# MuellerNico/DD2360-RayTracing

Hardware: AMD Instinct MI355X
Metric: Msamples/s (W*H*spp/render_time) at 1200x800, 10000 spheres (higher is better)
Workload: dtype f32

## Files before the change

### dd2360-raytracing_amd/csrc/rt_api.hip

```cpp
#include <hip/hip_runtime.h>
#include <atomic>
#include <vector>
#include <string>
#include <cstdio>
#include <cstring>
#include <new>
#include <limits>
#include <cmath>
#include <algorithm>
#include <mutex>
#include <cstdlib>
#include "rt_handles.h"
#include "rt_octgeom.h"
#include "../host/rt_image.hpp"

namespace rt {
hipError_t launch_render_init(rt_rand_state* rs, int max_x, int max_y, int part, int nparts, long long begin, long long end, hipStream_t st);
hipError_t launch_zero_counters(unsigned int* p, int n, hipStream_t st);
hipError_t launch_keep_counters(const unsigned int* queue, unsigned int* kept, hipStream_t st);
hipError_t launch_restore_counters(unsigned int* queue, const unsigned int* kept, hipStream_t st);
hipError_t launch_pilot(const RenderArgs& A, bool tree, int* cost, unsigned char* pilot, int* work, hipStream_t st);
hipError_t launch_pilot_h(const RenderArgs& A, bool tree, int* cost, hipStream_t st);
hipError_t launch_assemble_split(void* full, const void* parts, int max_x, int max_y, int nparts, const long long* starts, long long part_stride_px, bool half, hipStream_t st);
hipError_t launch_render(const RenderArgs& A, bool tree, int mode, hipStream_t st);
namespace fmac { hipError_t launch_render(const RenderArgs& A, bool tree, int mode, hipStream_t st); }
hipError_t launch_tile_order(const RenderArgs& A, bool tree, int* cost, unsigned int* order, unsigned char* flags, unsigned int* long_list, hipStream_t st);
hipError_t launch_render_h(const RenderArgs& A, bool tree, int mode, hipStream_t st);
hipError_t launch_tile_order_h(const RenderArgs& A, bool tree, int* cost, unsigned int* order, unsigned char* flags, unsigned int* long_list, hipStream_t st);
hipError_t launch_trace_h(const DevScene& S, const DevTree& T, bool tree, const float* rays, long long n, rt_hit_record* out, hipStream_t st);
hipError_t launch_assemble_h(void* full, const void* parts, int max_x, int max_y, int nparts, hipStream_t st);
hipError_t launch_trace(const DevScene& S, const DevTree& T, bool tree, const float* rays, long long n, rt_hit_record* out, hipStream_t st);
hipError_t launch_guides(const DevScene& S, const DevTree& T, bool tree, int max_x, int max_y, rt_hit_record* out, hipStream_t st);
hipError_t launch_denoise(float* fb_out, const float* fb_in, int max_x, int max_y, const rt_hit_record* hits, const rt_denoise_params& P,
                          float4* work, hipStream_t st);
hipError_t launch_denoise_var(float* fb_out, const float* fb_in, int max_x, int max_y, const rt_hit_record* hits, const void* state,
                              const rt_denoise_var_params& P, float4* work, hipStream_t st);
hipError_t launch_temporal_accumulate(void* hist_out, const void* hist_in, const rt_hit_record* hits, const rt_hit_record* hits_prev,
                                      const rt_camera* cam_prev, const void* state, const int32_t* kind, int n_kind, int max_x, int max_y,
                                      const rt_temporal_params& P, hipStream_t st);
hipError_t launch_denoise_hist(float* fb_out, const float* fb_in, int max_x, int max_y, const rt_hit_record* hits, const void* hist,
                               const rt_denoise_var_params& P, float4* work, hipStream_t st);
hipError_t launch_world_set_geometry(float4* geom, float4* shade, float4* list_hot, const int32_t* list_id, const float4* src, int n, int n_list,
                                     bool half, hipStream_t st);
hipError_t launch_temporal_accumulate_moving(void* hist_out, const void* hist_in, const rt_hit_record* hits, const rt_hit_record* hits_prev,
                                             const rt_camera* cam_prev, const float4* geom, const float4* geom_prev, const void* state,
                                             const int32_t* kind, int n_kind, int max_x, int max_y, const rt_temporal_params& P,
                                             hipStream_t st);
hipError_t launch_assemble(float* full, const float* parts, int max_x, int max_y, int nparts, hipStream_t st);
hipError_t launch_render_adaptive(const RenderArgs& A, bool tree, hipStream_t st);
hipError_t launch_adapt_check(float* fb, const float* sl, const float* q, const unsigned int* list_in, const unsigned int* count_in, long long n_all,
                              unsigned int* list_out, unsigned int* count_out, int32_t* spp, int k, bool last, float rel_error, float floor_lum,
                              const AdaptFrame& fr, hipStream_t st);
hipError_t launch_adapt_zero(unsigned int* p, int n, hipStream_t st);
hipError_t launch_adapt_check_keep(float* fb, const AdaptState& s, const unsigned int* list_in, const unsigned int* count_in, long long n_all,
                                   unsigned int* list_out, unsigned int* count_out, int32_t* spp, int k, bool last, float rel_error, float floor_lum,
                                   const AdaptFrame& fr, hipStream_t st);
hipError_t launch_adapt_refine_seed(float* fb, const AdaptState& s, long long n_all, unsigned int* list_out, unsigned int* count_out, int32_t* spp,
                                    int max_spp, float rel_error, float floor_lum, const AdaptFrame& fr, hipStream_t st);
hipError_t launch_adapt_refine_check(float* fb, const AdaptState& s, const unsigned int* list_in, const unsigned int* count_in, long long n_all,
                                     unsigned int* list_out, unsigned int* count_out, int32_t* spp, int batch, int max_spp, float rel_error, float floor_lum,
                                     hipStream_t st);
size_t budget_ws_bytes(long long n, bool filtered);
hipError_t launch_budget_select_filtered(const AdaptState& s, const rt_hit_record* hits, int max_x, int max_y, const rt_denoise_var_params& P, int batch,
                                         int max_spp, float floor_lum, unsigned int K, unsigned int* keys, float* keys_out, unsigned int* ws,
                                         unsigned int* list, unsigned int* count, hipStream_t st);
hipError_t launch_budget_select_temporal(const void* state, const void* hist_in, const rt_hit_record* hits, const rt_hit_record* hits_prev,
                                         const rt_camera* cam_prev, const int32_t* kind, int n_kind, int max_x, int max_y, const rt_temporal_params& P,
                                         int batch, int max_spp, float floor_lum, unsigned int K, unsigned int* keys, float* keys_out, unsigned int* ws,
                                         unsigned int* list, unsigned int* count, hipStream_t st);
hipError_t launch_budget_select(const AdaptState& s, long long n, const AdaptFrame& fr, int batch, int max_spp, float floor_lum, unsigned int K,
                                unsigned int* keys, unsigned int* ws, unsigned int* list, unsigned int* count, hipStream_t st);
hipError_t launch_budget_seed(float* fb, const AdaptState& s, const unsigned int* list, const unsigned int* count, unsigned int cap, hipStream_t st);
hipError_t launch_budget_final(float* fb, const AdaptState& s, const unsigned int* list, const unsigned int* count, unsigned int cap, int32_t* spp, int batch,
                               uint32_t* picked, hipStream_t st);
const char* render_kernel_name(bool tree, int mode, const DevAccel& acc);
namespace gpubuild { int build(rt_octree* O, const float4* d_geom, const int32_t* d_kind, int n, int spl, hipStream_t st); }
const char* render_kernel_name_h(bool tree, int mode);
#ifdef RT_H16_STATS
hipError_t read_h16_stats(unsigned long long* out, int reset);
#endif
#ifdef RT_STATS
hipError_t read_stats(unsigned long long* out, int reset);
hipError_t read_wp_classes(unsigned long long* out, int reset);
hipError_t read_wave_dbg(unsigned long long* out);
hipError_t read_pilot_dbg(int* out, int n);
#endif
}

using namespace rt;

#define RT_TRY(expr) do { const int e_ = (int)(expr); if (e_) return e_; } while (0)

static int world_host_geometry(const rt_world* W) {
    rt_world::Lazy& Z = *W->z;
    if (!Z.host_stale) return 0;
    rt_world* M = const_cast<rt_world*>(W);
    RT_TRY(hipDeviceSynchronize());
    RT_TRY(hipMemcpy(M->h_geom.data(), Z.d_geom, M->h_geom.size() * sizeof(float4), hipMemcpyDeviceToHost));
    if (!M->h_hot.empty()) RT_TRY(hipMemcpy(M->h_hot.data(), Z.d_list_hot, M->h_hot.size() * sizeof(float4), hipMemcpyDeviceToHost));
    Z.host_stale = false;
    return 0;
}

static rt_octree* build_list_tree(const rt_world* W) {
    rt_octree* O = new rt_octree();
    O->z = new rt_octree::Lazy();
    O->precision = RT_PRECISION_FP32;
    DevNode d; memset(&d, 0, sizeof(d));
    const float inf = std::numeric_limits<float>::infinity();
    d.lo[0] = d.lo[1] = d.lo[2] = -inf; d.hix = d.hiy = d.hiz = inf;
    d.skip = 1; d.first = 0; d.ref_index = 0;
    for (int i = 1; i < W->n; ++i) {
        if (W->h_kind[i] == RT_MAT_NONE) continue;
        const float4 g = W->h_geom[i];
        O->h_ent_hot.push_back(make_float4(g.x, g.y, g.z, g.w * g.w));
        O->h_ent_id.push_back(i);
    }
    d.count = (int32_t)O->h_ent_id.size();
    O->h_nodes.push_back(d);
    O->n_nodes = 1; O->n_entries = d.count;
    if (d.count > 0) build_accel(O->accel, O->h_nodes, O->h_ent_id, O->h_ent_hot, W->n, true);
    if (d.count < 64 || !O->accel.p.enabled || O->accel.p.n_large > 64) { delete O->z; delete O; return nullptr; }
    return O;
}
static rt_octree* ensure_list_tree(const rt_world* W) {
    rt_world::Lazy& Z = *W->z;
    if (!Z.list_tree_tried && W->precision == RT_PRECISION_FP32) {
        if (world_host_geometry(W)) return nullptr;
        Z.list_tree_tried = true;
        try { Z.list_tree = build_list_tree(W); } catch (const std::bad_alloc&) { Z.list_tree = nullptr; }
    }
    return Z.list_tree;
}

static bool valid_partition(rt_partition p) {
    if (!(p.nparts >= 1 && p.part >= 0 && p.part < p.nparts)) return false;
    if (p.tile_begin == 0 && p.tile_end == 0) return true;
    return p.tile_begin >= 0 && p.tile_end > p.tile_begin;
}
bool adaptive_params_ok(const rt_adaptive* P) {
    if (!P || P->min_spp < 2 || P->batch < 1 || P->max_spp < P->min_spp || (P->max_spp - P->min_spp) % P->batch != 0) return false;
    return P->rel_error >= 0.f && P->floor >= 0.f;
}
static bool adaptive_refines(const rt_adaptive* from, const rt_adaptive* to) {
    if (!adaptive_params_ok(from) || !adaptive_params_ok(to)) return false;
    if (to->min_spp != from->min_spp || to->batch != from->batch || to->max_spp < from->max_spp || !(to->floor <= from->floor)) return false;
    if (!(to->rel_error == 0.f || (to->rel_error > 0.f && to->rel_error <= from->rel_error))) return false;
    const float t = from->rel_error * from->rel_error;
    const float tn = t * ((float)from->max_spp - 1.f);
    if (!std::isfinite(tn)) return false;
    if (from->rel_error > 0.f && t == 0.f && to->rel_error > 0.f && to->floor != from->floor) return false;
    return true;
}
static const rt_partition kWhole = {0, 1, 0, 0};
static bool range_in_frame(rt_partition p, int64_t tiles) { return p.tile_end <= p.tile_begin || p.tile_end <= tiles; }
static int64_t local_tiles_of(int64_t tiles, rt_partition p) { return part_local_tiles(tiles, p.part, p.nparts, p.tile_begin, p.tile_end); }
static bool hittable(const rt_sphere& s) { return s.material != RT_MAT_NONE; }
static float radius_squared(const rt_sphere& s, int precision) {
    if (precision == RT_PRECISION_FP16) { const half_t r(s.radius); return (r * r).f(); }
    return s.radius * s.radius;
}

template <class R> static int create_world_impl(rt_sphere* list, int num_spheres, float sphere_radius, rt_camera* cam, int nx, int ny, rt_rand_state* st, int* num_created) {
    const int created = create_world_pods<R>(list, num_spheres, sphere_radius, cam, nx, ny, st);
    if (num_created) *num_created = created;
    return 0;
}

// ... 22 lines not shown
    switch (code) {
        case 0: return "ok";
        case RT_EINVAL: return "invalid argument";
        case RT_ENOMEM: return "out of host memory";
        case RT_EIO: return "i/o error";
        case RT_ENOTSUP: return "not supported";
        case RT_ECOMM: return "multi-GPU exchange failed";
        default: return code > 0 ? hipGetErrorString((hipError_t)code) : "unknown error";
    }
}

int rt_rand_init(rt_rand_state* rand_state) {
    if (!rand_state) return RT_EINVAL;
    xorwow::init(*rand_state, 1984ull);
    return 0;
}

int rt_create_world(rt_sphere* list, int num_spheres, float sphere_radius, rt_camera* cam, int nx, int ny, rt_rand_state* rand_state, int precision, int* num_created) {
    if (!list || !cam || !rand_state || num_spheres < 5 || nx <= 0 || ny <= 0) return RT_EINVAL;
    try {
        if (precision == RT_PRECISION_FP16) return create_world_impl<half_t>(list, num_spheres, sphere_radius, cam, nx, ny, rand_state, num_created);
        if (precision == RT_PRECISION_FP32) return create_world_impl<float>(list, num_spheres, sphere_radius, cam, nx, ny, rand_state, num_created);
    } catch (const std::bad_alloc&) { return RT_ENOMEM; }
    return RT_EINVAL;
}

int rt_camera_init(rt_camera* cam, const float lookfrom[3], const float lookat[3], const float vup[3], float vfov, float aspect, float aperture, float focus_dist, int precision) {
    if (!cam || !lookfrom || !lookat || !vup) return RT_EINVAL;
    if (precision == RT_PRECISION_FP16) camera_impl<half_t>(cam, lookfrom, lookat, vup, vfov, aspect, aperture, focus_dist);
    else if (precision == RT_PRECISION_FP32) camera_impl<float>(cam, lookfrom, lookat, vup, vfov, aspect, aperture, focus_dist);
    else return RT_EINVAL;
    return 0;
}

int rt_world_create(const rt_sphere* list, int num_spheres, const rt_camera* cam, int precision, rt_world** out) {
    if (!list || !cam || !out || num_spheres <= 0) return RT_EINVAL;
    if (precision != RT_PRECISION_FP32 && precision != RT_PRECISION_FP16) return RT_EINVAL;
    *out = nullptr;
    rt_world* W = new (std::nothrow) rt_world();
    if (!W) return RT_ENOMEM;
    W->z = new (std::nothrow) rt_world::Lazy();
    if (!W->z) { delete W; return RT_ENOMEM; }
    W->precision = precision; W->n = num_spheres;
    std::vector<float4>& hot = W->h_hot; std::vector<float4>& geom = W->h_geom; std::vector<float4>& mat = W->h_mat;
    std::vector<int32_t>& ids = W->h_ids; std::vector<int32_t>& kind = W->h_kind;
    geom.resize(num_spheres); mat.resize(num_spheres); kind.resize(num_spheres);
    for (int i = 0; i < num_spheres; ++i) {
        const rt_sphere& s = list[i];
        geom[i] = make_float4(s.center[0], s.center[1], s.center[2], s.radius);
        mat[i] = make_float4(s.albedo[0], s.albedo[1], s.albedo[2], s.param);
        kind[i] = s.material;
        if (hittable(s)) { hot.push_back(make_float4(s.center[0], s.center[1], s.center[2], radius_squared(s, precision))); ids.push_back(i); }
    }
    W->z->dev.n = num_spheres; W->z->dev.n_list = (int)hot.size();
    W->z->dev.ground_valid = hittable(list[0]) ? 1 : 0;
    W->z->dev.cam = *cam;
    *out = W;
    return 0;
}

int rt_world_set_list_traversal(rt_world* W, int mode) {
    if (!W || (mode != RT_TRAVERSAL_REFERENCE && mode != RT_TRAVERSAL_FAST)) return RT_EINVAL;
    W->list_traversal = mode;
    return 0;
}

int rt_world_set_arith(rt_world* W, int mode) {
    if (!W || (mode != RT_ARITH_IEEE && mode != RT_ARITH_CONTRACT)) return RT_EINVAL;
    if (mode == RT_ARITH_CONTRACT && W->precision == RT_PRECISION_FP16) return RT_ENOTSUP;
    W->arith = mode;
    return 0;
}
int rt_world_list_accel_info(const rt_world* W, int* enabled, int* grid_dim, float* cell_size, int* grid_entries, int* large_spheres) {
    if (!W) return RT_EINVAL;
    rt_octree* LT = ensure_list_tree(W);
    if (enabled) *enabled = LT != nullptr;
    if (!LT) { if (grid_dim) *grid_dim = 0; if (cell_size) *cell_size = 0.f; if (grid_entries) *grid_entries = 0; if (large_spheres) *large_spheres = 0; return 0; }
    return rt_octree_accel_info(LT, grid_dim, cell_size, grid_entries, large_spheres);
}

static DevGroup queue_group(rt_render_ctx& C) { return DevGroup().add(&C.d_queue, (kQueueSlots + 1) * kQueueStride * sizeof(unsigned int)); }
static DevGroup sched_group(rt_render_ctx& C, size_t tiles) {
    return DevGroup().add(&C.d_cost, sizeof(int) * tiles).add(&C.d_order, sizeof(unsigned int) * tiles).add(&C.d_flags, tiles * 96)
                     .add(&C.d_long, sizeof(unsigned int) * (tiles * 128 + 512)).add(&C.d_work, sizeof(int) * tiles * 2);
}
static DevGroup progressive_group(rt_render_ctx& C, size_t tiles) { return DevGroup().add(&C.p_cost, sizeof(int) * tiles).add(&C.p_order, sizeof(unsigned int) * tiles); }
static DevGroup adaptive_group(rt_render_ctx& C, size_t pixels) {
    return DevGroup().add(&C.a_sl, sizeof(float) * pixels).add(&C.a_q, sizeof(float) * pixels).add(&C.a_list, sizeof(unsigned int) * pixels * 2);
}
static DevGroup rounds_group(rt_render_ctx& C, size_t rounds) { return DevGroup().add(&C.a_count, sizeof(unsigned int) * rounds); }
static DevGroup budget_group(rt_render_ctx& C, size_t bytes) { return DevGroup().add(&C.b_ws, bytes); }

static int ctx_prepare(rt_render_ctx& C) {
    if (!C.d_queue) {
        RT_TRY(group_regrow(queue_group(C)));
        const hipError_t e = hipMemset(C.d_queue, 0, (kQueueSlots + 1) * kQueueStride * sizeof(unsigned int));
        if (e != hipSuccess) { (void)group_free(queue_group(C)); return (int)e; }
        C.d_kept = C.d_queue + (size_t)kQueueSlots * kQueueStride;
        sched_keep_drop(C.keep);
    }
    if (!C.ev_ready) {
        for (int k = 0; k < 64; ++k) {
            if (!C.ev0[k]) RT_TRY(hipEventCreate(&C.ev0[k]));
            if (!C.ev1[k]) RT_TRY(hipEventCreate(&C.ev1[k]));
        }
        if (!C.done) RT_TRY(hipEventCreateWithFlags(&C.done, hipEventDisableTiming));
        C.ev_ready = true;
    }
    return 0;
}
static int ctx_reserve(rt_render_ctx& C, int64_t tiles) {
    if (C.sched_tiles < tiles) sched_keep_drop(C.keep);
    return group_reserve(C.sched_tiles, tiles, sched_group(C, tiles));
}
static int ctx_reserve_progressive(rt_render_ctx& C, int64_t tiles) {
    if (C.p_tiles >= tiles) return 0;
    if (C.p_pinned) return RT_EINVAL;
    C.p_valid = false;
    return group_reserve(C.p_tiles, tiles, progressive_group(C, tiles));
}
static int ctx_reserve_adaptive(rt_render_ctx& C, int64_t pixels, int rounds) {
    RT_TRY(group_reserve(C.a_pixels, pixels, adaptive_group(C, pixels)));
    return group_reserve(C.a_rounds, rounds, rounds_group(C, rounds));
}
static int ctx_reserve_budget(rt_render_ctx& C, int64_t pixels, bool filtered = false) {
    const size_t bytes = budget_ws_bytes(pixels, filtered);
    return group_reserve(C.b_bytes, (int64_t)bytes, budget_group(C, bytes));
}
static int ctx_release(rt_render_ctx& C) {
    sched_keep_drop(C.keep); C.d_kept = nullptr;
    C.a_pixels = 0; C.a_rounds = 0; C.b_bytes = 0; C.sched_tiles = 0; C.p_tiles = 0; C.p_valid = false;
    int rc = 0;
    for (const DevGroup& g : {adaptive_group(C, 0), rounds_group(C, 0), budget_group(C, 0), queue_group(C), sched_group(C, 0), progressive_group(C, 0)}) {
        const int r = group_free(g);
        if (!rc) rc = r;
    }
    for (int k = 0; k < 64; ++k) { if (C.ev0[k]) (void)hipEventDestroy(C.ev0[k]); if (C.ev1[k]) (void)hipEventDestroy(C.ev1[k]); C.ev0[k] = nullptr; C.ev1[k] = nullptr; }
    if (C.done) (void)hipEventDestroy(C.done);
    C.done = nullptr; C.ev_ready = false; C.has_done = false; C.ev_count = 0;
    return rc;
}

int rt_render_ctx_create(rt_render_ctx** out) {
    if (!out) return RT_EINVAL;
    *out = nullptr;
    rt_render_ctx* C = new (std::nothrow) rt_render_ctx();
    if (!C) return RT_ENOMEM;
    const int rc = ctx_prepare(*C);
    if (rc) { (void)ctx_release(*C); delete C; return rc; }
    *out = C;
    return 0;
}
int rt_render_ctx_reserve(rt_render_ctx* C, int max_x, int max_y, rt_partition part) {
    if (!C || max_x <= 0 || max_y <= 0 || !valid_partition(part)) return RT_EINVAL;
    const int64_t tiles = (int64_t)((max_x + 7) / 8) * ((max_y + 7) / 8);
    const int rc = ctx_prepare(*C);
    if (!range_in_frame(part, tiles)) return RT_EINVAL;
    return rc ? rc : ctx_reserve(*C, local_tiles_of(tiles, part));
}
int rt_render_ctx_destroy(rt_render_ctx* C) {
    if (!C) return 0;
    const int rc = ctx_release(*C);
    delete C;
    return rc;
}

static DevGroup world_group(const rt_world* W, const std::vector<float4>* shade = nullptr, const std::vector<uint8_t>* kind8 = nullptr) {
// ... 352 lines not shown
        if (rc != RT_ENOTSUP) return rc;
    }
    RT_TRY(world_host_geometry(world));
    std::vector<rt_sphere> list;
    try {
        list.resize((size_t)world->n);
        for (int i = 0; i < world->n; ++i) {
            rt_sphere& s = list[i];
            const float4 g = world->h_geom[i], m = world->h_mat[i];
            s.center[0] = g.x; s.center[1] = g.y; s.center[2] = g.z; s.radius = g.w;
            s.material = world->h_kind[i]; s.albedo[0] = m.x; s.albedo[1] = m.y; s.albedo[2] = m.z; s.param = m.w;
        }
    } catch (const std::bad_alloc&) { return RT_ENOMEM; }
    return rt_build_octree(list.data(), world->n, spheres_per_leaf, world->precision, out);
}

int64_t rt_part_pixels(int max_x, int max_y, rt_partition part) {
    if (max_x <= 0 || max_y <= 0 || !valid_partition(part)) return RT_EINVAL;
    if (part_whole(part.nparts, part.tile_begin, part.tile_end)) return (int64_t)max_x * max_y;
    const int64_t tiles = (int64_t)((max_x + 7) / 8) * ((max_y + 7) / 8);
    if (!range_in_frame(part, tiles)) return RT_EINVAL;
    return local_tiles_of(tiles, part) * 64;
}

int rt_render_init(int max_x, int max_y, rt_rand_state* d_rand_state, rt_partition part, void* stream) {
    if (max_x <= 0 || max_y <= 0 || !valid_partition(part)) return RT_EINVAL;
    const int64_t npx = rt_part_pixels(max_x, max_y, part);
    if (npx < 0) return RT_EINVAL;
    if (npx == 0) return 0;
    if (!d_rand_state) return RT_EINVAL;
    return (int)launch_render_init(d_rand_state, max_x, max_y, part.part, part.nparts, part.tile_begin, part.tile_end, (hipStream_t)stream);
}

static const rt_octree* list_tree_of(const rt_world* world) {
    if (world->list_traversal != RT_TRAVERSAL_FAST) return nullptr;
    return ensure_list_tree(world);
}

static int ensure_on_device(const rt_world* world, const rt_octree*& d_octree) {
    if (!d_octree) d_octree = list_tree_of(world);
    int rc = world_upload(world);
    if (!rc && d_octree) rc = octree_upload(d_octree);
    return rc;
}
static DevTree tree_args(const rt_octree* d_octree) {
    DevTree T;
    if (d_octree) { T = d_octree->z->dev; T.acc.enabled = T.acc.enabled && d_octree->traversal == RT_TRAVERSAL_FAST; }
    else memset(&T, 0, sizeof(T));
    return T;
}
static float tune_value(const char* env, float dflt) {
    static std::mutex mu;
    static std::vector<std::pair<std::string, float>> seen;
    std::lock_guard<std::mutex> lock(mu);
    for (const auto& kv : seen) if (kv.first == env) return kv.second;
    float v = dflt;
    if (const char* e = getenv(env)) { char* end = nullptr; const float x = strtof(e, &end); if (end != e) v = x; }
    seen.emplace_back(env, v);
    return v;
}
static bool capturing(hipStream_t st) {
    hipStreamCaptureStatus cs = hipStreamCaptureStatusNone;
    if (hipStreamIsCapturing(st, &cs) != hipSuccess) { (void)hipGetLastError(); return false; }
    return cs != hipStreamCaptureStatusNone;
}

static void clear_schedule(RenderArgs& A) {
    A.order = nullptr; A.long_flag = nullptr; A.long_list = nullptr;
    A.tail_list = nullptr; A.tail_ws = nullptr; A.f_tail = 0.f; A.head_sum = 0; A.head_sum_dense = 0; A.head_min_load = 0.f;
    A.n_lanes = 0;
}
static RenderArgs frame_args(void* fb, int max_x, int max_y, int ns, const rt_world* world, rt_rand_state* d_rand_state, const rt_octree* d_octree, rt_partition part) {
    RenderArgs A;
    A.fb = fb; A.rand_state = d_rand_state; A.max_x = max_x; A.max_y = max_y; A.ns = ns;
    A.tiles_x = (max_x + 7) / 8; A.tiles_y = (max_y + 7) / 8;
    A.part = part.part; A.nparts = part.nparts; A.tile_begin = part.tile_begin; A.tile_end = part.tile_end;
    const int64_t tiles = (int64_t)A.tiles_x * A.tiles_y;
    A.n_local_tiles = local_tiles_of(tiles, part);
    A.scene = world->z->dev;
    A.tree = tree_args(d_octree);
    clear_schedule(A);
    A.f_inflight = tune_value("RT_F_INFLIGHT", RT_F_INFLIGHT); A.f_inflight_dense = tune_value("RT_F_INFLIGHT_DENSE", RT_F_INFLIGHT_DENSE); A.f_static = tune_value("RT_F_STATIC", RT_F_STATIC);
    A.ad_list = nullptr; A.ad_count = nullptr; A.ad_sl = nullptr; A.ad_q = nullptr;
    return A;
}

static int ctx_wait_previous(rt_render_ctx& C, hipStream_t st) {
    if (C.has_done && C.last_stream != st) RT_TRY(hipStreamWaitEvent(st, C.done, 0));
    return 0;
}
static int ctx_mark_done(rt_render_ctx& C, hipStream_t st) {
    RT_TRY(hipEventRecord(C.done, st));
    C.has_done = true; C.last_stream = st;
    return 0;
}
static unsigned int* next_slot(rt_render_ctx& C) { return C.d_queue + (size_t)(C.launches++ % kQueueSlots) * kQueueStride; }
static int ctx_timed_begin(rt_render_ctx& C, hipStream_t st) { return (int)hipEventRecord(C.ev0[C.ev_head % 64u], st); }
static int ctx_timed_end(rt_render_ctx& C, hipStream_t st) {
    RT_TRY(hipEventRecord(C.ev1[C.ev_head % 64u], st));
    C.ev_head++; if (C.ev_count < 64) C.ev_count++;
    return 0;
}
static int resumed_round(rt_render_ctx& C, RenderArgs& A, bool tree, hipStream_t st) {
    A.queue = next_slot(C);
    RT_TRY(launch_zero_counters(A.queue, (int)kQueueStride, st));
    return (int)launch_render_adaptive(A, tree, st);
}

static SchedKey frame_key(const rt_world* world, const rt_octree* d_octree, int max_x, int max_y, rt_partition part) {
    SchedKey key;
    key.world = world->serial; key.tree = d_octree ? d_octree->serial : 0;
    key.max_x = max_x; key.max_y = max_y;
    key.part = part.part; key.nparts = part.nparts; key.tile_begin = part.tile_begin; key.tile_end = part.tile_end;
    key.traversal = d_octree ? d_octree->traversal : 0;
    key.half = world->precision == RT_PRECISION_FP16 ? 1 : 0;
    return key;
}
static int schedule_decide(rt_render_ctx& C, const RenderArgs& A, const rt_world* world, const rt_octree* d_octree, int ns, bool cap, SchedKey& key, SchedAction& act) {
    int dev = 0;
    RT_TRY(hipGetDevice(&dev));
    key = frame_key(world, d_octree, A.max_x, A.max_y, rt_partition{A.part, A.nparts, A.tile_begin, A.tile_end});
    key.ns = ns; key.device = dev;
    act = sched_keep_decide(C.keep, key, tune_value("RT_SCHED_CACHE", (float)RT_SCHED_CACHE) != 0.f, cap);
    return 0;
}
static int begin_counters(rt_render_ctx& C, const RenderArgs& A, SchedAction act, hipStream_t st) {
    if (act == kSchedReuse) RT_TRY(launch_restore_counters(A.queue, C.d_kept, st));
    else RT_TRY(launch_zero_counters(A.queue, (int)kQueueStride, st));
    return 0;
}
static int schedule_frame(rt_render_ctx& C, RenderArgs& A, const rt_world* world, const rt_octree* d_octree, int ns, hipStream_t st, SchedAction act, const SchedKey& key) {
    const bool classify = ns >= 16;
    if (classify && world->precision != RT_PRECISION_FP16) { A.tail_list = C.d_long + (size_t)A.n_local_tiles * 64; A.tail_ws = C.d_long + (size_t)C.sched_tiles * 128; A.f_tail = tune_value("RT_F_TAIL", RT_F_TAIL); A.head_sum = (int)tune_value("RT_HEAD_SUM_SPARSE", (float)RT_HEAD_SUM_SPARSE); A.head_sum_dense = (int)tune_value("RT_HEAD_SUM_DENSE", (float)RT_HEAD_SUM_DENSE); A.head_min_load = tune_value("RT_HEAD_LOAD_DENSE", (float)RT_HEAD_LOAD_DENSE); }
    if (act != kSchedReuse) {
        if (world->precision == RT_PRECISION_FP16) RT_TRY(launch_tile_order_h(A, d_octree != nullptr, C.d_cost, C.d_order, classify ? C.d_flags : nullptr, classify ? C.d_long : nullptr, st));
        else RT_TRY(launch_tile_order(A, d_octree != nullptr, C.d_cost, C.d_order, classify ? C.d_flags : nullptr, classify ? C.d_long : nullptr, st));
        if (act == kSchedCompute) {
            RT_TRY(launch_keep_counters(A.queue, C.d_kept, st));
            sched_keep_commit(C.keep, key);
        }
    }
    A.order = C.d_order;
    if (classify) { A.long_flag = C.d_flags; A.long_list = C.d_long; }
    return 0;
}
static int scheduled_round(rt_render_ctx& C, RenderArgs& A, const rt_world* world, const rt_octree* d_octree, int ns, bool sched, bool cap, hipStream_t st) {
    A.queue = next_slot(C);
    SchedKey key; SchedAction act = kSchedBypass;
    if (sched) RT_TRY(schedule_decide(C, A, world, d_octree, ns, cap, key, act));
    RT_TRY(begin_counters(C, A, act, st));
    if (sched) RT_TRY(schedule_frame(C, A, world, d_octree, ns, st, act, key));
    return 0;
}

static int render_common(rt_render_ctx* ctx, void* fb, int max_x, int max_y, int ns, const rt_world* world, rt_rand_state* d_rand_state, const rt_octree* d_octree, rt_partition part, void* stream, int mode) {
    if (!world || max_x <= 0 || max_y <= 0 || ns <= 0 || !valid_partition(part)) return RT_EINVAL;
    if (d_octree && d_octree->precision != world->precision) return RT_EINVAL;
    { const int64_t npx = rt_part_pixels(max_x, max_y, part); if (npx < 0) return RT_EINVAL; if (npx == 0) return 0; }
    if (!fb || !d_rand_state) return RT_EINVAL;
    const hipStream_t st = (hipStream_t)stream;
    const bool cap = capturing(st);
    int rc = ensure_on_device(world, d_octree);
    rt_render_ctx& C = ctx ? *ctx : world->z->ctx;
    if (!rc && !cap) rc = ctx_prepare(C);
    if (rc) return rc;
    if (!C.d_queue) return RT_EINVAL;
    const SchedKey pkey = frame_key(world, d_octree, max_x, max_y, part);
    if (mode == 1 && ns == 1 && !cap && C.p_pinned && !sched_key_equal(C.p_key, pkey)) return RT_EINVAL;
    RenderArgs A = frame_args(fb, max_x, max_y, ns, world, d_rand_state, d_octree, part);
    const bool sched = mode == 0 && ns >= 4, tree = d_octree != nullptr;
    if (sched && C.sched_tiles < A.n_local_tiles) {
        if (cap) return RT_EINVAL;
        RT_TRY(ctx_reserve(C, A.n_local_tiles));
    }
    if (!cap) RT_TRY(ctx_wait_previous(C, st));
    RT_TRY(scheduled_round(C, A, world, d_octree, ns, sched, cap, st));
    C.last_queue = A.queue;
    if (mode == 1) {
        if (ns == 1 && !cap) {
            C.p_valid = false;
            RT_TRY(ctx_reserve_progressive(C, A.n_local_tiles));
            if (world->precision == RT_PRECISION_FP16) RT_TRY(launch_tile_order_h(A, tree, C.p_cost, C.p_order, nullptr, nullptr, st));
            else RT_TRY(launch_tile_order(A, tree, C.p_cost, C.p_order, nullptr, nullptr, st));
            C.p_key = pkey; C.p_valid = true;
        }
        if (C.p_valid && sched_key_equal(C.p_key, pkey) && C.p_tiles >= A.n_local_tiles) { A.order = C.p_order; if (cap) C.p_pinned = true; }
    }
    if (!cap) RT_TRY(ctx_timed_begin(C, st));
    if (world->precision == RT_PRECISION_FP16) RT_TRY(launch_render_h(A, tree, mode, st));
    else if (world->arith == RT_ARITH_CONTRACT) RT_TRY(fmac::launch_render(A, tree, mode, st));
    else RT_TRY(launch_render(A, tree, mode, st));
    if (cap) return 0;
    RT_TRY(ctx_timed_end(C, st));
    return ctx_mark_done(C, st);
}

static int ctx_times(rt_render_ctx& C, float* ms_out, int max, int* count) {
    int n = 0;
    const unsigned have = C.ev_count;
    for (unsigned k = 0; k < have && n < max; ++k) {
        const unsigned slot = (C.ev_head - have + k) % 64u;
        RT_TRY(hipEventSynchronize(C.ev1[slot]));
        float ms = 0.f;
        RT_TRY(hipEventElapsedTime(&ms, C.ev0[slot], C.ev1[slot]));
        ms_out[n++] = ms;
    }
    *count = n;
    C.ev_count = 0;
    return 0;
}
static int ctx_counters(rt_render_ctx& C, uint32_t* out4) {
    if (!C.last_queue) { out4[0] = out4[1] = out4[2] = out4[3] = 0u; return 0; }
    if (C.has_done) RT_TRY(hipEventSynchronize(C.done));
    uint32_t q[6];
    RT_TRY(hipMemcpy(q, C.last_queue, sizeof(q), hipMemcpyDeviceToHost));
    out4[0] = q[0]; out4[1] = q[1]; out4[2] = q[2] + q[4]; out4[3] = q[3] + q[5];
    return 0;
}
int rt_world_render_counters(rt_world* W, uint32_t* out4) {
    if (!W || !out4) return RT_EINVAL;
    return ctx_counters(W->z->ctx, out4);
}
int rt_render_ctx_counters(rt_render_ctx* C, uint32_t* out4) {
    if (!C || !out4) return RT_EINVAL;
    return ctx_counters(*C, out4);
}
static int ctx_schedule(rt_render_ctx& C, uint32_t* out, int n) {
    if (n > RT_SCHEDULE_WORDS) n = RT_SCHEDULE_WORDS;
    uint32_t w[RT_SCHEDULE_WORDS] = {0, 0, 0, 0, 0, 0, 0, 0};
    if (C.last_queue) {
        if (C.has_done) RT_TRY(hipEventSynchronize(C.done));
        uint32_t q[kQueueThr + 6];
        RT_TRY(hipMemcpy(q, C.last_queue, sizeof(q), hipMemcpyDeviceToHost));
        for (int k = 0; k < 6; ++k) w[k] = q[kQueueThr + k];
        w[6] = q[2]; w[7] = q[4];
    }
    for (int k = 0; k < n; ++k) out[k] = w[k];
    return 0;
}
int rt_world_render_schedule(rt_world* W, uint32_t* out, int n) {
    if (!W || n < 0 || (n > 0 && !out)) return RT_EINVAL;
    return ctx_schedule(W->z->ctx, out, n);
}
int rt_render_ctx_schedule(rt_render_ctx* C, uint32_t* out, int n) {
    if (!C || n < 0 || (n > 0 && !out)) return RT_EINVAL;
    return ctx_schedule(*C, out, n);
}
int rt_render_ctx_schedule_reuse(rt_render_ctx* C, uint64_t* reused, uint64_t* computed) {
    if (!C || !reused || !computed) return RT_EINVAL;
    *reused = C->keep.reused; *computed = C->keep.computed;
    return 0;
}
int rt_world_render_schedule_reuse(rt_world* W, uint64_t* reused, uint64_t* computed) {
    if (!W) return RT_EINVAL;
    return rt_render_ctx_schedule_reuse(&W->z->ctx, reused, computed);
}
int rt_world_render_times(rt_world* W, float* ms_out, int max, int* count) {
    if (!W || !ms_out || !count || max < 0) return RT_EINVAL;
    return ctx_times(W->z->ctx, ms_out, max, count);
}
int rt_render_ctx_times(rt_render_ctx* C, float* ms_out, int max, int* count) {
    if (!C || !ms_out || !count || max < 0) return RT_EINVAL;
    return ctx_times(*C, ms_out, max, count);
}

int rt_render(void* fb, int max_x, int max_y, int ns, const rt_world* world, rt_rand_state* d_rand_state, const rt_octree* d_octree, rt_partition part, void* stream) {
    return render_common(nullptr, fb, max_x, max_y, ns, world, d_rand_state, d_octree, part, stream, 0);
}
int rt_render_progressive(void* fb, int max_x, int max_y, int current_sample, const rt_world* world, rt_rand_state* d_rand_state, const rt_octree* d_octree, rt_partition part, void* stream) {
    return render_common(nullptr, fb, max_x, max_y, current_sample, world, d_rand_state, d_octree, part, stream, 1);
}
int rt_render_on(rt_render_ctx* ctx, void* fb, int max_x, int max_y, int ns, const rt_world* world, rt_rand_state* d_rand_state, const rt_octree* d_octree, rt_partition part, void* stream) {
    if (!ctx) return RT_EINVAL;
    return render_common(ctx, fb, max_x, max_y, ns, world, d_rand_state, d_octree, part, stream, 0);
}
int rt_render_progressive_on(rt_render_ctx* ctx, void* fb, int max_x, int max_y, int current_sample, const rt_world* world, rt_rand_state* d_rand_state, const rt_octree* d_octree, rt_partition part, void* stream) {
    if (!ctx) return RT_EINVAL;
    return render_common(ctx, fb, max_x, max_y, current_sample, world, d_rand_state, d_octree, part, stream, 1);
}

struct FrameCall {
    hipStream_t st = nullptr; rt_render_ctx* C = nullptr;
    int64_t npx = 0;
    bool tree = false;
    AdaptFrame fr{};
};
static int frame_begin(FrameCall& F, rt_render_ctx* ctx, bool params_ok, bool pointers_ok, int max_x, int max_y, rt_partition part,
                       const rt_world* world, const rt_octree*& d_octree, void* stream, const rt_world* kinds = nullptr) {
    if (!params_ok || max_x <= 0 || max_y <= 0 || !valid_partition(part)) return RT_EINVAL;
    const int64_t npx = rt_part_pixels(max_x, max_y, part);
    if (npx < 0 || npx > (int64_t)0xffffffffll) return RT_EINVAL;
    if (npx == 0) return 0;
    if (!pointers_ok) return RT_EINVAL;
    if (world && d_octree && d_octree->precision != world->precision) return RT_EINVAL;
    if (world && (world->precision == RT_PRECISION_FP16 || world->arith == RT_ARITH_CONTRACT)) return RT_ENOTSUP;
    if (kinds && kinds->precision == RT_PRECISION_FP16) return RT_ENOTSUP;
    F.st = (hipStream_t)stream;
    if (capturing(F.st)) return RT_EINVAL;
    int rc = world ? ensure_on_device(world, d_octree) : 0;
    if (!rc && kinds) rc = world_upload(kinds);
    F.C = ctx ? ctx : &world->z->ctx;
    if (!rc) rc = ctx_prepare(*F.C);
    if (rc) return rc;
    F.npx = npx; F.tree = d_octree != nullptr;
    F.fr = AdaptFrame{max_x, max_y, (max_x + 7) / 8, part.part, part.nparts, part.tile_begin, part.tile_end};
    return 0;
}

static int render_adaptive_common(rt_render_ctx* ctx, void* fb, int max_x, int max_y, const rt_adaptive* P, const rt_world* world,
                                  rt_rand_state* d_rand_state, const rt_octree* d_octree, int32_t* d_spp, rt_partition part, void* stream,
                                  void* d_state = nullptr, bool need_state = false) {
    FrameCall F;
    const int rc = frame_begin(F, ctx, adaptive_params_ok(P) && world, fb && d_rand_state && (d_state || !need_state), max_x, max_y, part, world, d_octree, stream);
    if (rc || !F.npx) return rc;
    rt_render_ctx& C = *F.C; const hipStream_t st = F.st; const int64_t npx = F.npx;
    const AdaptState keep = adapt_state(d_state, npx);
    const int rounds = (P->max_spp - P->min_spp) / P->batch;
    RenderArgs A = frame_args(fb, max_x, max_y, P->min_spp, world, d_rand_state, d_octree, part);
    const bool sched = P->min_spp >= 4;
    if (sched) RT_TRY(ctx_reserve(C, A.n_local_tiles));
    RT_TRY(ctx_reserve_adaptive(C, npx, rounds + 1));
    RT_TRY(ctx_wait_previous(C, st));
    unsigned int* lists[2] = {C.a_list, C.a_list + npx};
    A.ad_sl = d_state ? keep.sl : C.a_sl; A.ad_q = d_state ? keep.q : C.a_q;
    RT_TRY(launch_adapt_zero(C.a_count, rounds + 1, st));
    RT_TRY(scheduled_round(C, A, world, d_octree, P->min_spp, sched, false, st));
    RT_TRY(ctx_timed_begin(C, st));
    RT_TRY(launch_render_adaptive(A, F.tree, st));
    auto check = [&](const unsigned int* list_in, const unsigned int* count_in, unsigned int* list_out, unsigned int* count_out, int k, bool last) {
        return d_state ? launch_adapt_check_keep((float*)fb, keep, list_in, count_in, npx, list_out, count_out, d_spp, k, last, P->rel_error, P->floor, F.fr, st)
                       : launch_adapt_check((float*)fb, C.a_sl, C.a_q, list_in, count_in, npx, list_out, count_out, d_spp, k, last, P->rel_error, P->floor, F.fr, st);
    };
    RT_TRY(check(nullptr, nullptr, lists[0], C.a_count, P->min_spp, rounds == 0));
    A.ns = P->batch;
    clear_schedule(A);
    for (int r = 1; r <= rounds; ++r) {
        A.ad_list = lists[(r - 1) & 1]; A.ad_count = C.a_count + (r - 1);
        RT_TRY(resumed_round(C, A, F.tree, st));
// ... 348 lines not shown
    if (P.normal_pow_log2 < -1 || P.normal_pow_log2 > 10) return RT_EINVAL;
    if (P.prefilter != 0 && P.prefilter != 1) return RT_EINVAL;
    if (!denoise_sigma_ok(P.sigma_position, 1.0f)) return RT_EINVAL;
    if (!(P.sigma_variance >= 0.0f) || !std::isfinite(P.sigma_variance * P.sigma_variance)) return RT_EINVAL;
    return 0;
}

int rt_denoise_adaptive(void* fb_out, const void* fb_in, int max_x, int max_y, const rt_hit_record* d_hits, const void* d_state,
                        const rt_denoise_var_params* params, void* d_work, void* stream) {
    if (!fb_out || !fb_in || !d_hits || !d_state || !d_work) return RT_EINVAL;
    if (((uintptr_t)d_hits & 15) || ((uintptr_t)d_work & 15)) return RT_EINVAL;
    const int rc = rt_denoise_adaptive_check(max_x, max_y, params);
    if (rc) return rc;
    return (int)launch_denoise_var((float*)fb_out, (const float*)fb_in, max_x, max_y, d_hits, d_state, *params, (float4*)d_work, (hipStream_t)stream);
}

int rt_temporal_check(int max_x, int max_y, const rt_temporal_params* params) {
    if (!params || max_x <= 0 || max_y <= 0 || (long long)max_x * max_y > RT_DENOISE_MAX_PIXELS) return RT_EINVAL;
    const rt_temporal_params& P = *params;
    if (P.max_history < 0) return RT_EINVAL;
    if (P.reuse_specular != 0 && P.reuse_specular != 1) return RT_EINVAL;
    if (!(P.position_tolerance > 0.0f) || !std::isfinite(P.position_tolerance) || !std::isfinite(P.position_tolerance * P.position_tolerance)) return RT_EINVAL;
    if (!(P.normal_min_dot >= -1.0f && P.normal_min_dot <= 1.0f)) return RT_EINVAL;
    return 0;
}

int rt_temporal_accumulate(void* d_hist_out, const void* d_hist_in, const rt_hit_record* d_hits, const rt_hit_record* d_hits_prev,
                           const rt_camera* cam_prev, const void* d_state, const rt_world* world, int max_x, int max_y,
                           const rt_temporal_params* params, void* stream) {
    if (!d_hist_out || !d_hits || !d_state || !world) return RT_EINVAL;
    if (d_hist_in && (!d_hits_prev || !cam_prev)) return RT_EINVAL;
    if (((uintptr_t)d_hist_out & 15) || ((uintptr_t)d_hist_in & 15) || ((uintptr_t)d_hits & 15) || (d_hist_in && ((uintptr_t)d_hits_prev & 15))) return RT_EINVAL;
    const int rc = rt_temporal_check(max_x, max_y, params);
    if (rc) return rc;
    if (d_hist_in) {
        const uintptr_t a = (uintptr_t)d_hist_out, b = (uintptr_t)d_hist_in, bytes = (uintptr_t)RT_TEMPORAL_HISTORY_BYTES * (uintptr_t)max_x * (uintptr_t)max_y;
        if ((a > b ? a - b : b - a) < bytes) return RT_EINVAL;
    }
    if (world->precision == RT_PRECISION_FP16) return RT_ENOTSUP;
    const int up = world_upload(world);
    if (up) return up;
    return (int)launch_temporal_accumulate(d_hist_out, d_hist_in, d_hits, d_hits_prev, cam_prev, d_state, world->z->dev.kind, world->n, max_x, max_y,
                                           *params, (hipStream_t)stream);
}

int rt_temporal_accumulate_moving(void* d_hist_out, const void* d_hist_in, const rt_hit_record* d_hits, const rt_hit_record* d_hits_prev,
                                  const rt_camera* cam_prev, const float* d_geom_prev, const void* d_state, const rt_world* world,
                                  int max_x, int max_y, const rt_temporal_params* params, void* stream) {
    if (!d_hist_out || !d_hits || !d_state || !world) return RT_EINVAL;
    if (d_hist_in && (!d_hits_prev || !cam_prev || !d_geom_prev)) return RT_EINVAL;
    if (((uintptr_t)d_hist_out & 15) || ((uintptr_t)d_hist_in & 15) || ((uintptr_t)d_hits & 15) || (d_hist_in && ((uintptr_t)d_hits_prev & 15))) return RT_EINVAL;
    if (d_hist_in && ((uintptr_t)d_geom_prev & 15)) return RT_EINVAL;
    const int rc = rt_temporal_check(max_x, max_y, params);
    if (rc) return rc;
    if (d_hist_in) {
        const uintptr_t a = (uintptr_t)d_hist_out, b = (uintptr_t)d_hist_in, bytes = (uintptr_t)RT_TEMPORAL_HISTORY_BYTES * (uintptr_t)max_x * (uintptr_t)max_y;
        if ((a > b ? a - b : b - a) < bytes) return RT_EINVAL;
    }
    if (world->precision == RT_PRECISION_FP16) return RT_ENOTSUP;
    const int up = world_upload(world);
    if (up) return up;
    return (int)launch_temporal_accumulate_moving(d_hist_out, d_hist_in, d_hits, d_hits_prev, cam_prev, world->z->dev.geom,
                                                  d_hist_in ? (const float4*)d_geom_prev : nullptr, d_state, world->z->dev.kind, world->n,
                                                  max_x, max_y, *params, (hipStream_t)stream);
}

int rt_denoise_history(void* fb_out, const void* fb_in, int max_x, int max_y, const rt_hit_record* d_hits, const void* d_hist,
                       const rt_denoise_var_params* params, void* d_work, void* stream) {
    if (!fb_out || !fb_in || !d_hits || !d_hist || !d_work) return RT_EINVAL;
    if (((uintptr_t)d_hits & 15) || ((uintptr_t)d_hist & 15) || ((uintptr_t)d_work & 15)) return RT_EINVAL;
    const int rc = rt_denoise_adaptive_check(max_x, max_y, params);
    if (rc) return rc;
    return (int)launch_denoise_hist((float*)fb_out, (const float*)fb_in, max_x, max_y, d_hits, d_hist, *params, (float4*)d_work, (hipStream_t)stream);
}

#ifdef RT_H16_STATS
int rt_debug_h16(unsigned long long* out8, int reset) { return (int)rt::read_h16_stats(out8, reset); }
#endif
#ifdef RT_STATS
int rt_debug_stats(unsigned long long* out16, int reset) { return (int)read_stats(out16, reset); }
int rt_debug_wp_classes(unsigned long long* out96, int reset) { return (int)read_wp_classes(out96, reset); }
int rt_debug_waves(unsigned long long* out) { return (int)read_wave_dbg(out); }
int rt_debug_pilot(int* out, int n) { return (int)read_pilot_dbg(out, n); }
#endif

using rt::ppm_text;

int64_t rt_format_ppm(int nx, int ny, const void* fb, int precision, char* out, int64_t cap) {
    if (nx <= 0 || ny <= 0 || !fb) return RT_EINVAL;
    std::string s;
    try { ppm_text(nx, ny, fb, precision, s); } catch (const std::bad_alloc&) { return RT_ENOMEM; }
    if (out && (int64_t)s.size() <= cap) memcpy(out, s.data(), s.size());
    return (int64_t)s.size();
}

int rt_write_ppm(const char* path, int nx, int ny, const void* fb, int precision) {
    if (nx <= 0 || ny <= 0 || !fb) return RT_EINVAL;
    std::string s;
    try { ppm_text(nx, ny, fb, precision, s); } catch (const std::bad_alloc&) { return RT_ENOMEM; }
    FILE* f = path ? fopen(path, "wb") : stdout;
    if (!f) return RT_EIO;
    const size_t w = fwrite(s.data(), 1, s.size(), f);
    if (path) { if (fclose(f) != 0) return RT_EIO; } else fflush(f);
    return w == s.size() ? 0 : RT_EIO;
}

int rt_write_image(const char* path, int nx, int ny, const void* fb, int precision, int format) {
    if (!path || nx <= 0 || ny <= 0 || !fb) return RT_EINVAL;
    if (precision != RT_PRECISION_FP32 && precision != RT_PRECISION_FP16) return RT_EINVAL;
    if (format == RT_IMAGE_P3) return rt_write_ppm(path, nx, ny, fb, precision);
    if (format != RT_IMAGE_P6 && format != RT_IMAGE_PFM) return RT_EINVAL;
    FILE* f = fopen(path, "wb");
    if (!f) return RT_EIO;
    bool ok = true;
    try {
        ok = rt::write_binary_image(f, nx, ny, fb, precision, format);
    } catch (const std::bad_alloc&) { fclose(f); return RT_ENOMEM; }
    if (fclose(f) != 0) ok = false;
    return ok ? 0 : RT_EIO;
}

}
```

### dd2360-raytracing_amd/csrc/rt_device.h

```cpp
#pragma once
#include <hip/hip_runtime.h>
#include <stdint.h>
#include "../../include/rt_amd.h"

namespace rt {

constexpr double kRootHalfXZ = 11.0;
constexpr double kCellXZ = 2.0 * kRootHalfXZ / 8.0, kCellY = 0.25;
constexpr float kRootHalfXZf = (float)kRootHalfXZ, kInvCellXZf = 1.0f / 2.75f, kInvCellYf = 4.0f;
static_assert(kCellXZ == 2.75 && 1.0 / kCellY == 4.0, "level-3 cells of the reference's root box");


#ifndef RT_PART_RUN_BUILD
#define RT_PART_RUN_BUILD RT_PART_RUN
#endif
constexpr long long kPartRun = RT_PART_RUN_BUILD;
__host__ __device__ inline bool part_whole(int nparts, long long begin, long long end) { return nparts == 1 && end <= begin; }
__host__ __device__ inline long long part_tile(long long local_tile, int part, int nparts, long long begin = 0, long long end = 0) {
    if (end > begin) return begin + local_tile;
    if (nparts == 1) return local_tile;
    return ((local_tile / kPartRun) * nparts + part) * kPartRun + local_tile % kPartRun;
}
__host__ __device__ inline long long part_local_tiles(long long tiles, int part, int nparts, long long begin = 0, long long end = 0) {
    if (end > begin) return end - begin;
// ... 59 lines not shown
    float hiy, hiz;
    int32_t skip;
    int32_t first;
    int32_t count;
    int32_t ref_index;
    int32_t pad[2];
};
static_assert(sizeof(DevNode) == 48, "DevNode is 3 x float4");

struct DevScene {
    const float4* list_hot;
    const int32_t* list_id;
    const float4* geom;
    const float4* mat;
    const int32_t* kind;
    const float4* shade;
    const uint8_t* kind8;
    int32_t n, n_list;
    int32_t ground_valid;
    rt_camera cam;
};

struct DevAccel {
    const float4* large_hot;
    const float4* large_brick;
    const int32_t* cs;
    const float4* hot;
    const float4* brick;
    int32_t zoff;
    const int32_t* memb_start;
    const int32_t* memb_cell;
    const int32_t* bits_index;
    const uint32_t* cellbits;
    const int32_t* cellnode;
    int32_t n_large, G;
    int32_t F, Gf;
    float rq_c;
    float g0, h, inv_h;
    float ylo, yhi;
    float rmax;
    float zone2;
    int32_t enabled;
    int32_t coop_groups;
    int32_t solo_chains;
};

struct DevTree {
    const float4* nodes4;
    const float4* ent_hot;
    const int32_t* ent_id;
    int32_t n_nodes, n_entries;
    const float* h16_planes;
    int32_t h16_np[3];
    DevAccel acc;
};

constexpr int kQueueThr = 32;
struct RenderArgs {
    void* fb;
    rt_rand_state* rand_state;
    int32_t max_x, max_y, ns;
    int32_t tiles_x, tiles_y;
    int32_t part, nparts;
    int64_t tile_begin, tile_end;
    int64_t n_local_tiles;
    unsigned int* queue;
    int32_t n_lanes;
    const unsigned int* tail_list;
    unsigned int* tail_ws;
    float head_min_load;
    int32_t head_sum, head_sum_dense;
    float f_tail;
    float f_inflight_dense;
    float f_inflight, f_static;
    const unsigned int* order;
    const unsigned char* long_flag;
    const unsigned int* long_list;
    DevScene scene;
    DevTree tree;
    const unsigned int* ad_list;
    const unsigned int* ad_count;
    float* ad_sl;
    float* ad_q;
};

}
```

### dd2360-raytracing_amd/csrc/rt_handles.h

```cpp
#pragma once
#include <hip/hip_runtime.h>
#include <cassert>
#include <vector>
#include "rt_device.h"
#include "../host/rt_scene.hpp"
#include "rt_accel.h"
#include "rt_sched_keep.h"

using rt::DevScene; using rt::DevTree; using rt::DevNode; using rt::DevAccel; using rt::AccelHost; using rt::Octree;

struct rt_octree;

struct DevBuf { void** at; size_t bytes; const void* src; size_t src_bytes; };
struct DevGroup {
    int n = 0; DevBuf b[16];
    DevGroup& add(void* at, size_t bytes) { assert(n < 16); b[n++] = DevBuf{(void**)at, bytes, nullptr, 0}; return *this; }
    template <class V> DevGroup& add_copy(void* at, const V& v) {
        const size_t sz = sizeof(typename V::value_type);
        assert(n < 16);
        b[n++] = DevBuf{(void**)at, (v.empty() ? 1 : v.size()) * sz, v.empty() ? nullptr : v.data(), v.size() * sz};
        return *this;
    }
};
inline int group_free(const DevGroup& g) {
    int rc = 0;
    for (int k = 0; k < g.n; ++k) {
        void*& p = *g.b[k].at;
        if (p) { const hipError_t e = hipFree(p); if (e != hipSuccess && !rc) rc = (int)e; p = nullptr; }
    }
    return rc;
}
inline int group_regrow(const DevGroup& g) {
    int rc = group_free(g);
    for (int k = 0; k < g.n && !rc; ++k) {
        const DevBuf& b = g.b[k];
        if (!b.bytes) continue;
        rc = (int)hipMalloc(b.at, b.bytes);
        if (!rc && b.src) rc = (int)hipMemcpy(*b.at, b.src, b.src_bytes, hipMemcpyHostToDevice);
        if (rc) (void)group_free(g);
    }
    return rc;
}
inline int group_reserve(int64_t& have, int64_t need, const DevGroup& g) {
    if (have >= need) return 0;
    have = 0;
    const int rc = group_regrow(g);
    if (!rc) have = need;
    return rc;
}

struct rt_render_ctx {
    unsigned int* d_queue = nullptr; unsigned launches = 0;
    int* d_cost = nullptr; unsigned int* d_order = nullptr; unsigned char* d_flags = nullptr; unsigned int* d_long = nullptr; int* d_work = nullptr; int64_t sched_tiles = 0;
    unsigned int* last_queue = nullptr;
    rt::SchedKeep keep; unsigned int* d_kept = nullptr;
    int* p_cost = nullptr; unsigned int* p_order = nullptr; int64_t p_tiles = 0; bool p_valid = false; rt::SchedKey p_key;
    bool p_pinned = false;
    float* a_sl = nullptr; float* a_q = nullptr; unsigned int* a_list = nullptr; int64_t a_pixels = 0; unsigned int* a_count = nullptr; int64_t a_rounds = 0;
    unsigned int* b_ws = nullptr; int64_t b_bytes = 0;
    hipEvent_t ev0[64] = {}, ev1[64] = {}; unsigned ev_head = 0, ev_count = 0; bool ev_ready = false;
    hipEvent_t done = nullptr; hipStream_t last_stream = nullptr; bool has_done = false;
};
static const unsigned kQueueSlots = 64, kQueueStride = 64;

uint64_t rt_next_serial();

struct rt_world {
    uint64_t serial = rt_next_serial();
    int precision = RT_PRECISION_FP32;
    int n = 0;
    std::vector<float4> h_hot, h_geom, h_mat;
    std::vector<int32_t> h_ids, h_kind;
    int list_traversal = RT_TRAVERSAL_FAST;
    int arith = RT_ARITH_IEEE;
    struct Lazy {
        bool uploaded = false;
        DevScene dev{};
        void* d_list_hot = nullptr; void* d_list_id = nullptr; void* d_geom = nullptr; void* d_mat = nullptr; void* d_kind = nullptr;
        void* d_shade = nullptr; void* d_kind8 = nullptr;
        rt_octree* list_tree = nullptr; bool list_tree_tried = false;
        rt_render_ctx ctx;
        bool host_stale = false;
    };
    Lazy* z = nullptr;
};

struct rt_octree {
    uint64_t serial = rt_next_serial();
    int precision = RT_PRECISION_FP32;
    Octree* host = nullptr;
    std::vector<DevNode> h_nodes; std::vector<float4> h_ent_hot; std::vector<int32_t> h_ent_id;
    AccelHost accel;
    int traversal = RT_TRAVERSAL_FAST;
    struct Lazy {
        bool uploaded = false;
        DevTree dev{};
        void* d_nodes = nullptr; void* d_ent_hot = nullptr; void* d_ent_id = nullptr;
        void* d_acc[12] = {nullptr, nullptr, nullptr, nullptr, nullptr, nullptr, nullptr, nullptr, nullptr, nullptr, nullptr, nullptr};
        void* d_arena = nullptr;
        const rt_octnode* d_ref_nodes = nullptr; const int32_t* d_leaf_count = nullptr; const int32_t* d_leaf_indices = nullptr;
        int ref_node_count = 0, ref_leaf_count = 0, ref_dropped_full = 0, ref_dropped_outside = 0, ref_spl = 0;
        Octree* host_view = nullptr;
    };
    Lazy* z = nullptr;
    int n_nodes = 0, n_entries = 0;
    int n_world = 0, bit_rows = 1;
};


bool adaptive_params_ok(const rt_adaptive* P);
```

### dd2360-raytracing_amd/csrc/rt_kernels.hip

```cpp
#include <hip/hip_runtime.h>
#include <float.h>
#include "rt_device.h"
#include "rt_tuning.h"
#include "rt_sampling.h"
#include "rt_sched_keep.h"

#ifdef RT_TU_CONTRACT
#pragma clang fp contract(fast)
#else
#pragma clang fp contract(off)
#endif

namespace rt {
#ifdef RT_TU_CONTRACT
namespace fmac {
#endif

#define RT_DEV static __device__ __forceinline__

#include "rt_stats.h"

struct Rng { uint32_t d, v0, v1, v2, v3, v4; };

RT_DEV float rng_uniform(Rng& s) {
// ... 1009 lines not shown
    const float dt = dot3(uv, on);
    const float disc = 1.0f - ni * ni * (1.0f - dt * dt);
    float fx = 0.0f, fy = 0.0f, fz = 0.0f, reflect_prob;
    if (disc > 0.0f) {
        const float sq = sqrtf(disc);
        fx = ni * (uv.x - dt * on.x) - sq * on.x;
        fy = ni * (uv.y - dt * on.y) - sq * on.y;
        fz = ni * (uv.z - dt * on.z) - sq * on.z;
        const float r0 = r0sq;
        reflect_prob = r0 + (1.0f - r0) * pow5(1.0f - cosine);
    } else {
        reflect_prob = 1.0f;
    }
    r.o = p;
    if (rng_uniform(s) < reflect_prob) { r.d.x = rx; r.d.y = ry; r.d.z = rz; }
    else { r.d.x = fx; r.d.y = fy; r.d.z = fz; }
    return true;
}

RT_DEV V3 sky(const RayF& r, const V3& att) {
    WPASS(WP_SKY);
    const float len = sqrtf(r.d.x * r.d.x + r.d.y * r.d.y + r.d.z * r.d.z);
    const float uy = r.d.y / len;
    const float t = 0.5f * (uy + 1.0f);
    const float omt = 1.0f - t;
    V3 c;
    c.x = att.x * (omt + t * 0.5f);
    c.y = att.y * (omt + t * 0.7f);
    c.z = att.z * (omt + t * 1.0f);
    return c;
}

#ifndef RT_TU_LIST
__global__ __launch_bounds__(256) void k_render_init(rt_rand_state* rand_state, int max_x, int max_y, int tiles_x, int part, int nparts, long long begin, long long end, long long n_local_tiles) {
    const int lane = threadIdx.x & 63;
    const long long local_tile = (long long)blockIdx.x * 4 + (threadIdx.x >> 6);
    if (local_tile >= n_local_tiles) return;
    const long long tile = part_tile(local_tile, part, nparts, begin, end);
    const int tx = (int)(tile % tiles_x), ty = (int)(tile / tiles_x);
    const int i = tx * 8 + (lane & 7), j = ty * 8 + (lane >> 3);
    const bool inside = (i < max_x) && (j < max_y);
    const bool whole = part_whole(nparts, begin, end);
    if (whole && !inside) return;
    const long long idx = whole ? (long long)j * max_x + i : local_tile * 64 + lane;
    const int pixel_index = j * max_x + i;
    Rng s; rng_seed(s, 1984ull + (unsigned long long)(long long)pixel_index);
    rt_rand_state out;
    out.d = s.d; out.v[0] = s.v0; out.v[1] = s.v1; out.v[2] = s.v2; out.v[3] = s.v3; out.v[4] = s.v4;
    out.boxmuller_flag = 0; out.boxmuller_flag_double = 0; out.boxmuller_extra = 0.f; out.pad_ = 0; out.boxmuller_extra_double = 0.0;
    rand_state[idx] = out;
}
#endif

template <bool TREE, int MODE, int COOPG>
__global__ __launch_bounds__(256, RT_RENDER_WAVES) void k_render(RenderArgs A) {
    extern __shared__ float4 s_nodes[];
    if (TREE) stage_tree_fp32<COOPG != 1>(A.scene, A.tree, s_nodes);
    const int lane = threadIdx.x & 63;
    const long long n_slots = (MODE == 2 && A.ad_list) ? (long long)*A.ad_count : A.n_local_tiles * 64;
    const int ns = (MODE != 1) ? A.ns : 1;

    const long long n_waves = (long long)gridDim.x * 4;
    long long slot = 0;
    int i = 0, j = 0; long long idx = 0;
    unsigned int iters = 0;
    bool is_long = false;
    bool is_med = false;
    bool retired = false;
    bool thin = false;
    bool thin_counted = false;
    bool long_done = false;
    const unsigned int n_long_raw = A.long_list ? A.queue[2] : 0u, n_solo_raw = A.long_list ? A.queue[4] : 0u;
    const bool use_long = (n_long_raw + n_solo_raw) != 0u && (long long)(n_long_raw + n_solo_raw) * 64 <= n_slots;
    const unsigned int n_long = use_long ? n_long_raw : 0u, n_solo = use_long ? n_solo_raw : 0u;
    bool solo = false, solo_done = false;
    Rng s = {0, 0, 0, 0, 0, 0};
    V3 col = {0.0f, 0.0f, 0.0f};
    V3 att = {1.0f, 1.0f, 1.0f};
    float sum_l = 0.0f, sum_q = 0.0f;
    RayF r; r.o = {0.f, 0.f, 0.f}; r.d = {0.f, 1.f, 0.f};
    int sample = 0, depth = 0;
    bool live = false;
    RT_STATS_ONLY(
    unsigned int pix_iters = 0;
    unsigned long long pix_t0 = 0;
    )

    constexpr bool kChunked = MODE == 1;
    constexpr long long kProgOwn = RT_PROG_OWN;
    const long long first_free = (kChunked && kProgOwn > 0 && n_waves * kProgOwn <= n_slots) ? n_waves * kProgOwn : 0;
    long long pool_next = 0, pool_end = 0;
    if (kChunked && first_free > 0) { pool_next = ((long long)blockIdx.x * 4 + (threadIdx.x >> 6)) * kProgOwn; pool_end = pool_next + kProgOwn; }
    auto take_slot = [&]() -> long long {
        return first_free + (long long)atomicAdd(cold_args()->queue, 1u);
    };
    auto begin_pixel = [&]() {
        live = false;
        const RenderArgs& A = *cold_args();
#ifdef RT_ONLY_LANE
        if (lane != RT_ONLY_LANE) return;
#endif
        iters = 0; is_long = false; is_med = false;
        while (slot < n_slots) {
            if constexpr (MODE == 2) {
                if (A.ad_list) {
                    const unsigned int pid = A.ad_list[slot];
                    idx = (long long)pid;
                    if (part_whole(A.nparts, A.tile_begin, A.tile_end)) { i = (int)(pid % (unsigned int)A.max_x); j = (int)(pid / (unsigned int)A.max_x); }
                    else {
                        const long long tile = part_tile((long long)(pid >> 6), A.part, A.nparts, A.tile_begin, A.tile_end);
                        const int tx = (int)(tile % A.tiles_x), ty = (int)(tile / A.tiles_x);
                        i = tx * 8 + (int)(pid & 7u); j = ty * 8 + (int)((pid >> 3) & 7u);
                    }
                    live = true;
                    break;
                }
            }
            long long local_tile; int l;
            const long long tail0 = (MODE != 1 && A.tail_list) ? (long long)A.queue[kQueueThr + 2] : 0;
            const long long head = tail0 > 0 ? (long long)A.queue[kQueueThr + 3] : 0;
            if (tail0 > 0 && (slot < head || slot >= tail0 - 1 + head)) {
                const bool from_end = A.queue[kQueueThr + 5] != 0u;
                const long long n_tail = n_slots - (tail0 - 1);
                const long long k = slot < head ? (from_end ? n_tail - head + slot : slot) : (from_end ? slot - (tail0 - 1) - head : slot - (tail0 - 1));
                const unsigned int pid = A.tail_list[k];
                local_tile = (long long)(pid >> 6); l = (int)(pid & 63u);
            } else {
                constexpr int kIl = COOPG == 2 ? RT_INTERLEAVE_DENSE : (COOPG == 5 ? RT_INTERLEAVE_SOLO : RT_INTERLEAVE);
                static_assert(kIl > 0 && 64 % kIl == 0, "RT_INTERLEAVE, RT_INTERLEAVE_DENSE and RT_INTERLEAVE_SOLO must divide 64 (the tail starts on a multiple of 64 tiles)");
                const long long ms = slot - head;
                const long long blk = ms / (64 * kIl);
                const long long tiles_in_blk = (A.n_local_tiles - blk * kIl) < kIl ? (A.n_local_tiles - blk * kIl) : kIl;
                const long long within = ms % (64 * kIl);
                const long long rank = blk * kIl + within % tiles_in_blk;
                l = (int)(within / tiles_in_blk);
                local_tile = A.order ? (long long)A.order[rank] : rank;
            }
            const long long tile = part_tile(local_tile, A.part, A.nparts, A.tile_begin, A.tile_end);
            const int tx = (int)(tile % A.tiles_x), ty = (int)(tile / A.tiles_x);
            i = tx * 8 + (l & 7); j = ty * 8 + (l >> 3);
            const bool taken = use_long && A.long_flag[local_tile * 64 + l];
            if (i < A.max_x && j < A.max_y && !taken) {
                idx = part_whole(A.nparts, A.tile_begin, A.tile_end) ? (long long)j * A.max_x + i : local_tile * 64 + l;
                live = true;
                RT_STATS_ONLY(
                pix_t0 = __builtin_amdgcn_s_memrealtime();
                )
                break;
            }
            slot = take_slot();
        }
        if (!live) retired = true;
        if (live) {
            const rt_rand_state* st = A.rand_state + idx;
            s.d = st->d; s.v0 = st->v[0]; s.v1 = st->v[1]; s.v2 = st->v[2]; s.v3 = st->v[3]; s.v4 = st->v[4];
            col = {0.0f, 0.0f, 0.0f}; att = {1.0f, 1.0f, 1.0f}; sample = 0; depth = 0;
            if constexpr (MODE == 2) {
                sum_l = 0.0f; sum_q = 0.0f;
                if (A.ad_list) {
                    const float* f = (const float*)A.fb + idx * 3;
                    col.x = f[0]; col.y = f[1]; col.z = f[2]; sum_l = A.ad_sl[idx]; sum_q = A.ad_q[idx];
                }
            }
            r = primary_ray(A.scene.cam, i, j, A.max_x, A.max_y, s);
        }
    };
    auto begin_long_pixel = [&](bool from_solo) -> bool {
        if (!use_long || (from_solo ? solo_done : long_done)) return false;
        const RenderArgs& A = *cold_args();
        long long pid;
        if (from_solo) {
            const unsigned int h = atomicAdd(A.queue + 5, 1u);
            if (h >= n_solo) { solo_done = true; return false; }
            pid = (long long)A.long_list[n_slots - 1 - (long long)h];
        } else {
            const unsigned int h = atomicAdd(A.queue + 3, 1u);
            if (h >= n_long) { long_done = true; return false; }
            const unsigned int stride = n_long % 257u ? 257u : (n_long % 263u ? 263u : 269u);
            pid = (long long)A.long_list[(unsigned int)(((unsigned long long)h * stride) % n_long)];
        }
        const long long local_tile = pid >> 6;
        const int l = (int)(pid & 63);
        const long long tile = part_tile(local_tile, A.part, A.nparts, A.tile_begin, A.tile_end);
        const int tx = (int)(tile % A.tiles_x), ty = (int)(tile / A.tiles_x);
        i = tx * 8 + (l & 7); j = ty * 8 + (l >> 3);
        idx = part_whole(A.nparts, A.tile_begin, A.tile_end) ? (long long)j * A.max_x + i : pid;
        live = true; iters = 0; is_long = true;
        RT_STATS_ONLY(
        pix_t0 = __builtin_amdgcn_s_memrealtime();
        )
        const rt_rand_state* st = A.rand_state + idx;
        s.d = st->d; s.v0 = st->v[0]; s.v1 = st->v[1]; s.v2 = st->v[2]; s.v3 = st->v[3]; s.v4 = st->v[4];
        col = {0.0f, 0.0f, 0.0f}; att = {1.0f, 1.0f, 1.0f}; sample = 0; depth = 0;
        if constexpr (MODE == 2) { sum_l = 0.0f; sum_q = 0.0f; }
        r = primary_ray(A.scene.cam, i, j, A.max_x, A.max_y, s);
        return true;
    };
    auto end_pixel = [&]() {
        const RenderArgs& A = *cold_args();
        rt_rand_state* st_out = A.rand_state + idx;
        st_out->d = s.d; st_out->v[0] = s.v0; st_out->v[1] = s.v1; st_out->v[2] = s.v2; st_out->v[3] = s.v3; st_out->v[4] = s.v4;
        float* fb = (float*)A.fb + idx * 3;
        if constexpr (MODE == 2) {
            fb[0] = col.x; fb[1] = col.y; fb[2] = col.z;
            A.ad_sl[idx] = sum_l; A.ad_q[idx] = sum_q;
        } else if (MODE == 0) {
            const float k = (float)(1.0 / (double)(float)A.ns);
            col.x *= k; col.y *= k; col.z *= k;
            fb[0] = sqrtf(col.x); fb[1] = sqrtf(col.y); fb[2] = sqrtf(col.z);
            RT_STATS_ONLY(
            fb[0] = (float)pix_iters; fb[1] = (float)((__builtin_amdgcn_s_memrealtime() >> 4) & 0xffffffull); fb[2] = (float)((pix_t0 >> 4) & 0xffffffull);
            )
        } else {
            if (A.ns == 1) { fb[0] = col.x; fb[1] = col.y; fb[2] = col.z; }
            else { fb[0] += col.x; fb[1] += col.y; fb[2] += col.z; }
        }
    };
    RT_STATS_ONLY(
    Stats st; for (int q = 0; q < ST_N; ++q) st.c[q] = 0;
    for (int q = 0; q < 8; ++q) st.cyc[q] = 0;
    const unsigned long long tK0 = TICK(), rK0 = __builtin_amdgcn_s_memrealtime();
    unsigned int dbg_thin_iters = 0, dbg_long = 0;
    unsigned long long th[4] = {0, 0, 0, 0};
    unsigned long long dbg_thin_cyc = 0, dbg_thin_closest = 0, dbg_thin1_cyc = 0; unsigned int dbg_thin1_iters = 0; unsigned long long dbg_t_prev = TICK();
    )
    constexpr bool kSolo = TREE && COOPG == 5;
    if (kSolo && lane == 0 && begin_long_pixel(true)) solo = true;
    if (__ballot(live) == 0ull && lane < RT_LONG_PER_WAVE) begin_long_pixel(false);
    if (__ballot(live) != 0ull) { thin = true; __builtin_amdgcn_s_setprio(3); }

    const unsigned int thin_cap = (unsigned int)(n_waves / RT_THIN_CAP_DEN);
    float closest = FLT_MAX; int best = -1;
    TreeState ts; tree_state_init(ts);
    while (true) {
        const unsigned long long m_live = __ballot(live);
        const unsigned long long m_long = __ballot(live && is_long);
        if (!thin && m_long != 0ull) {
            unsigned int prev = 0;
            if (lane == 0) prev = atomicAdd(cold_args()->queue + 1, 1u);
            prev = __builtin_amdgcn_readfirstlane(prev);
            if (prev < thin_cap) { thin = true; thin_counted = true; __builtin_amdgcn_s_setprio(3); }
            else { if (lane == 0) atomicSub(cold_args()->queue + 1, 1u); is_long = false; }
        } else if (thin && m_long == 0ull) {
            thin = false; __builtin_amdgcn_s_setprio(0);
            if (thin_counted && lane == 0) atomicSub(A.queue + 1, 1u);
            thin_counted = false;
        }
        if (RT_MED_RATE > 0 && !thin) { if (__ballot(live && is_med) != 0ull) __builtin_amdgcn_s_setprio(1); else __builtin_amdgcn_s_setprio(0); }
        if (!thin) {
            if (kChunked) {
                const bool need = !live && !retired;
                const unsigned long long mneed = __ballot(need);
                if (mneed != 0ull) {
                    const long long n = (long long)__popcll(mneed);
                    const long long left = pool_end - pool_next;
                    const long long rank = (long long)__builtin_amdgcn_mbcnt_hi((unsigned)(mneed >> 32), __builtin_amdgcn_mbcnt_lo((unsigned)mneed, 0u));
                    long long fresh = 0;
                    if (n > left) {
                        unsigned int b = 0;
                        if (lane == 0) b = atomicAdd(cold_args()->queue, 64u);
                        fresh = first_free + (long long)__builtin_amdgcn_readfirstlane(b);
                    }
                    if (need) slot = rank < left ? pool_next + rank : fresh + (rank - left);
                    if (n > left) { pool_next = fresh + (n - left); pool_end = fresh + 64; } else pool_next += n;
                    if (need) begin_pixel();
                }
            } else if (!live && !retired) { slot = take_slot(); begin_pixel(); }
        }
        if (__ballot(live) == 0ull) break;
        (void)m_live;
        STAT(st, ST_LOOP_ITERS_WAVE, 1);
        RT_STATS_ONLY(
        { const unsigned long long now = TICK(); const int nl2 = __popcll(__ballot(live));
          if (thin) { ++dbg_thin_iters; dbg_thin_cyc += now - dbg_t_prev; if (nl2 <= 2) { ++dbg_thin1_iters; dbg_thin1_cyc += now - dbg_t_prev; } }
          dbg_t_prev = now; }
        )
        RT_STATS_ONLY(
        { const int nl = __popcll(__ballot(live)); STAT(st, nl >= 56 ? ST_LIVE_GE56 : nl >= 32 ? ST_LIVE_32 : nl >= 8 ? ST_LIVE_8 : ST_LIVE_LT8, 1);
          WPASS_CLASS(nl >= 56 ? 0 : nl >= 32 ? 1 : nl >= 8 ? 2 : 3); }
        )
        const float a = dot3(r.d, r.d);
        if (!TREE) { closest = FLT_MAX; best = -1; }
        RT_STATS_ONLY(
        const unsigned long long tC0 = TICK();
        const unsigned long long c4_ = st.cyc[4], c5_ = st.cyc[5], c1_ = st.cyc[1], c3_ = st.cyc[3];
        const bool thin12 = thin && __popcll(__ballot(live)) <= 2;
        )
        if (TREE) closest_tree<COOPG>(A.scene, A.tree, s_nodes, r, a, live, closest, best, ts STAT_PASS);
        else closest_list(A.scene, r, a, live, closest, best);
        RT_STATS_ONLY(
        const unsigned long long tC1 = TICK(); st.cyc[0] += tC1 - tC0; st.cyc[2] += tC0; if (thin) dbg_thin_closest += tC1 - tC0;
        if (TREE && thin12) { th[0] += (st.cyc[4] - c4_) - tC0; th[1] += st.cyc[5] - c5_; th[2] += (st.cyc[1] - c1_) - (st.cyc[5] - c5_); th[3] += st.cyc[3] - c3_; }
        if (live) { ++pix_iters; }
        )
        if (live && !(TREE && ts.pending)) {
            ++iters;
            bool done;
            float lum = 0.0f;
            if (best >= 0) {
                const bool cont = scatter(cold_args()->scene, best, closest, r, att, s);
                ++depth;
                done = !cont || depth >= 50;
            } else {
                const V3 c = sky(r, att);
                col.x += c.x; col.y += c.y; col.z += c.z;
                if constexpr (MODE == 2) lum = (c.x + c.y) + c.z;
                done = true;
            }
            if (done) {
                if constexpr (MODE == 2) { sum_l += lum; sum_q += lum * lum; }
                (void)lum;
                ++sample; depth = 0; att = {1.0f, 1.0f, 1.0f};
                if (sample < ns) {
                    { const RenderArgs& C = *cold_args(); r = primary_ray(C.scene.cam, i, j, C.max_x, C.max_y, s); }
                    bool now_long = false;
                    if ((sample & (RT_LONG_CHECK - 1)) == 0 && sample + 8 <= ns) {
                        const unsigned int long_thr = MODE != 1 ? cold_args()->queue[kQueueThr] : 0u;
                        now_long = iters >= (unsigned int)((COOPG == 2 ? RT_LONG_RATE_DENSE : RT_LONG_RATE) * sample) ||
                                   (long_thr != 0u && (unsigned long long)iters * (unsigned int)ns >= (unsigned long long)long_thr * (unsigned int)sample);
                    }
                    if (now_long) {
                        RT_STATS_ONLY(
                        if (!is_long) ++dbg_long;
                        )
                        is_long = true;
                    }
                    else if (RT_MED_RATE > 0 && (sample & 7) == 0 && iters >= (unsigned int)(RT_MED_RATE * sample)) is_med = true;
                } else {
                    WPASS(WP_ENDPIX);
                    end_pixel();
                    RT_STATS_ONLY(
                    pix_iters = 0;
                    )
                    STAT(st, ST_SWITCHES, 1);
                    live = false; is_long = false; is_med = false;
                    if (kSolo && solo && begin_long_pixel(true)) {  }
                    else if (lane < RT_LONG_PER_WAVE && begin_long_pixel(false)) { solo = false;  }
                }
            }
        }
    }

    RT_STATS_ONLY(
    for (int q = 0; q < ST_N; ++q) {
        const bool wave_level = (q == ST_LOOP_ITERS_WAVE || (q >= ST_LIVE_GE56 && q <= ST_LIVE_LT8));
        const bool lane_max = (q == ST_A_ITERS_WAVE || q == ST_B_ROUNDS_WAVE);
        if (lane_max) { int m = (int)st.c[q]; for (int off = 32; off > 0; off >>= 1) m = max(m, __shfl_xor(m, off)); if (lane == 0) atomicAdd(&g_stats[q], (unsigned long long)m); }
        else if (st.c[q] && (!wave_level || lane == 0)) atomicAdd(&g_stats[q], (unsigned long long)st.c[q]);
    }
    { int nl = (int)dbg_long; for (int off = 32; off > 0; off >>= 1) nl += __shfl_xor(nl, off); dbg_long = (unsigned int)nl; }
    if (lane == 0) {
        const long long wv = (long long)blockIdx.x * 4 + (threadIdx.x >> 6);
        if (wv < 8192) {
            g_wave_dbg[wv * 4 + 0] = __builtin_amdgcn_s_memrealtime();
            g_wave_dbg[wv * 4 + 1] = st.c[ST_LOOP_ITERS_WAVE]; g_wave_dbg[wv * 4 + 2] = dbg_thin_iters; g_wave_dbg[wv * 4 + 3] = dbg_long;
            atomicAdd(&g_stats[TH_GROUND], th[0]); atomicAdd(&g_stats[TH_LARGE_SETUP], th[1]); atomicAdd(&g_stats[TH_WALK], th[2]); atomicAdd(&g_stats[TH_SCAN], th[3]);
            atomicAdd(&g_stats[ST_SPARE0], dbg_thin_cyc); atomicAdd(&g_stats[ST_SPARE1], dbg_thin_closest); atomicAdd(&g_stats[ST_SPARE2], dbg_thin1_cyc); atomicAdd(&g_stats[ST_SPARE3], (unsigned long long)dbg_thin1_iters); atomicAdd(&g_stats[ST_SPARE4], (unsigned long long)dbg_thin_iters);
        }
        atomicAdd(&g_stats[ST_SAMPLES], 1ull);
        const unsigned long long tot = TICK() - tK0;
        atomicAdd(&g_stats[ST_CYC_TOTAL], tot);
        atomicAdd(&g_stats[ST_CYC_CLOSEST], st.cyc[0]); atomicAdd(&g_stats[ST_CYC_WALK_A], st.cyc[1]); atomicAdd(&g_stats[ST_CYC_WALK_B], st.cyc[4] - st.cyc[2]);
        atomicAdd(&g_stats[ST_CYC_SCAN], st.cyc[3]); atomicAdd(&g_stats[ST_CYC_SHADE], tot - st.cyc[0]); atomicAdd(&g_stats[ST_SPARE4 + 1], st.cyc[5]); atomicAdd(&g_stats[ST_SPARE4 + 2], st.cyc[6]);
        atomicAdd(&g_stats[ST_REALTIME], __builtin_amdgcn_s_memrealtime() - rK0);
    }
    )
}

#if !defined(RT_TU_LIST) && !defined(RT_TU_CONTRACT)
__device__ __forceinline__ bool adapt_rule(float S, float Q, int k, float rel_error, float floor_lum) {
    const float nk = (float)k;
    const float d = nk * Q - S * S;
    const float nf = nk * floor_lum;
    const float m = S > nf ? S : nf;
    const float tt = rel_error * rel_error;
    return rel_error > 0.f && d <= (tt * (nk - 1.f)) * (m * m);
}
__device__ __forceinline__ bool adapt_in_frame(long long t, const AdaptFrame& fr) {
    const long long tile = part_tile(t >> 6, fr.part, fr.nparts, fr.tile_begin, fr.tile_end);
    const int tx = (int)(tile % fr.tiles_x), ty = (int)(tile / fr.tiles_x);
    return tx * 8 + (int)(t & 7) < fr.max_x && ty * 8 + (int)((t >> 3) & 7) < fr.max_y;
}
__device__ __forceinline__ void adapt_append(bool active, unsigned int pid, unsigned int* list_out, unsigned int* count_out) {
    const unsigned long long mask = __ballot(active);
    if (mask != 0ull) {
        unsigned int base = 0;
        if ((threadIdx.x & 63) == 0) base = atomicAdd(count_out, (unsigned int)__popcll(mask));
        base = __shfl(base, 0);
        const unsigned int rank = __builtin_amdgcn_mbcnt_hi((unsigned)(mask >> 32), __builtin_amdgcn_mbcnt_lo((unsigned)mask, 0u));
        if (active) list_out[base + rank] = pid;
    }
}
template <bool KEEP>
__device__ __forceinline__ void adapt_check(float* __restrict__ fb, const float* __restrict__ sl, const float* __restrict__ q,
                                            const unsigned int* __restrict__ list_in, const unsigned int* __restrict__ count_in, long long n_all,
                                            unsigned int* __restrict__ list_out, unsigned int* __restrict__ count_out, int32_t* __restrict__ spp,
                                            int k, int last, float rel_error, float floor_lum, const AdaptFrame& fr, const AdaptState& keep) {
    const long long t = (long long)blockIdx.x * 256 + threadIdx.x;
    const long long n = count_in ? (long long)*count_in : n_all;
    bool active = false;
    unsigned int pid = 0;
    bool inside = true;
    if (!list_in && t < n && !part_whole(fr.nparts, fr.tile_begin, fr.tile_end)) {
        const long long tile = part_tile(t >> 6, fr.part, fr.nparts, fr.tile_begin, fr.tile_end);
        const int tx = (int)(tile % fr.tiles_x), ty = (int)(tile / fr.tiles_x);
        inside = tx * 8 + (int)(t & 7) < fr.max_x && ty * 8 + (int)((t >> 3) & 7) < fr.max_y;
    }
    if (t < n && inside) {
        pid = list_in ? list_in[t] : (unsigned int)t;
        bool stop = last != 0;
        if (!stop) stop = adapt_rule(sl[pid], q[pid], k, rel_error, floor_lum);
        if (stop) {
            float* f = fb + (size_t)pid * 3;
            const float kk = (float)(1.0 / (double)(float)k);
            if constexpr (KEEP) {
// ... 56 lines not shown
        s.k[pid] = k;
        if (k >= max_spp || adapt_rule(s.sl[pid], s.q[pid], k, rel_error, floor_lum)) {
            float* f = fb + (size_t)pid * 3;
            float* S = s.rgb + (size_t)pid * 3;
            const float kk = (float)(1.0 / (double)(float)k);
            S[0] = f[0]; S[1] = f[1]; S[2] = f[2];
            f[0] = sqrtf(f[0] * kk); f[1] = sqrtf(f[1] * kk); f[2] = sqrtf(f[2] * kk);
            if (spp) spp[pid] = k;
        } else {
            active = true;
        }
    }
    adapt_append(active, pid, list_out, count_out);
}
__global__ __launch_bounds__(256) void k_adapt_zero(unsigned int* p, int n) {
    const int t = blockIdx.x * 256 + threadIdx.x;
    if (t < n) p[t] = 0u;
}
#endif

template <bool TREE, int COOPG = 1>
__global__ __launch_bounds__(256) void k_tile_cost(RenderArgs A, int* __restrict__ cost, unsigned char* __restrict__ pilot, int* __restrict__ work) {
    extern __shared__ float4 s_nodes[];
    if (TREE) stage_tree_fp32<COOPG != 1>(A.scene, A.tree, s_nodes);
    const int lane = threadIdx.x & 63;
    constexpr int kPerTile = 16 * RT_PILOT_SAMPLES, kTilesPerWave = 64 / kPerTile;
    static_assert(RT_PILOT_SAMPLES == 1 || RT_PILOT_SAMPLES == 2 || RT_PILOT_SAMPLES == 4, "pilot samples per pixel");
    const long long local_tile = ((long long)blockIdx.x * 4 + (threadIdx.x >> 6)) * kTilesPerWave + lane / kPerTile;
    const bool tile_ok = local_tile < A.n_local_tiles;
    const long long tile = part_tile(tile_ok ? local_tile : 0, A.part, A.nparts, A.tile_begin, A.tile_end);
    const int tx = (int)(tile % A.tiles_x), ty = (int)(tile / A.tiles_x);
    const int sub = (lane % kPerTile) / RT_PILOT_SAMPLES, smp = lane % RT_PILOT_SAMPLES;
    const int lx = 2 * (sub & 3), ly = 2 * (sub >> 2);
    const int i = tx * 8 + lx, j = ty * 8 + ly;
    const bool inside = tile_ok && (i < A.max_x) && (j < A.max_y);
    Rng ps; rng_seed(ps, 0x5deece66dull + (unsigned long long)((long long)j * A.max_x + i) + (unsigned long long)smp * 0x9e3779b97f4a7c15ull);
    RayF r; r.o = {0.f, 0.f, 0.f}; r.d = {0.f, 1.f, 0.f};
    V3 att = {1.0f, 1.0f, 1.0f};
    bool live = inside;
    if (live) r = primary_ray(A.scene.cam, i, j, A.max_x, A.max_y, ps);
    int bounces = 0;
    RT_STATS_ONLY(
    Stats st; for (int q = 0; q < ST_N; ++q) st.c[q] = 0;
    for (int q = 0; q < 8; ++q) st.cyc[q] = 0;
    )
    float closest = FLT_MAX; int best = -1;
    TreeState ts; tree_state_init(ts);
    int lane_iters = 0;
    while (__ballot(live) != 0ull) {
        const float a = dot3(r.d, r.d);
        if (!TREE) { closest = FLT_MAX; best = -1; }
        if (TREE) closest_tree<COOPG>(A.scene, A.tree, s_nodes, r, a, live, closest, best, ts STAT_PASS);
        else closest_list(A.scene, r, a, live, closest, best);
        if (live) ++lane_iters;
        if (live && !(TREE && ts.pending)) {
            ++bounces;
            bool done = true;
            if (best >= 0) { const bool cont = scatter(A.scene, best, closest, r, att, ps); done = !cont || bounces >= RT_PILOT_CAP; }
            if (done) live = false;
        }
    }
    int pix = inside ? bounces : 0;
    for (int off = RT_PILOT_SAMPLES / 2; off > 0; off >>= 1) pix += __shfl_xor(pix, off);
    RT_STATS_ONLY(
    if (tile_ok && smp == 0 && local_tile * 16 + sub < (1 << 20)) g_pilot_dbg[local_tile * 16 + sub] = inside ? pix : -1;
    )
    if (pilot && tile_ok && smp == 0) pilot[local_tile * 16 + sub] = (unsigned char)(pix < 255 ? pix : 255);
    int w = inside ? bounces : 0;
    for (int off = kPerTile / 2; off > 0; off >>= 1) w += __shfl_xor(w, off);
    if (lane % kPerTile == 0 && tile_ok) cost[local_tile] = w * 4;
    if (work) {
        int tw = inside ? (int)ts.work : 0;
        for (int off = kPerTile / 2; off > 0; off >>= 1) tw += __shfl_xor(tw, off);
        int tc = inside ? lane_iters : 0;
        for (int off = kPerTile / 2; off > 0; off >>= 1) tc += __shfl_xor(tc, off);
        if (lane % kPerTile == 0 && tile_ok) { work[local_tile] = tw; work[A.n_local_tiles + local_tile] = tc; }
        (void)ts.cols;
    }
}

RT_DEV int cost_class(int w) { const int c = (w - 64) / 64; return c < 0 ? 0 : (c > 7 ? 7 : c); }

#ifndef RT_TU_LIST
__global__ __launch_bounds__(256) void k_long_select(RenderArgs A, const unsigned char* __restrict__ pilot, unsigned char* __restrict__ long_flag,
                                                    unsigned int* __restrict__ long_list, int long_sum, int solo_sum, unsigned char* __restrict__ sum8) {
    const long long g = (long long)blockIdx.x * 256 + threadIdx.x;
    if (g >= A.n_local_tiles * 16) return;
    const long long local_tile = g >> 4;
    const int sub = (int)(g & 15);
    const long long tile = part_tile(local_tile, A.part, A.nparts, A.tile_begin, A.tile_end);
    const int tx = (int)(tile % A.tiles_x), ty = (int)(tile / A.tiles_x);
    const int bx = tx * 4 + (sub & 3), by = ty * 4 + (sub >> 2);
    const int own = pilot[g];
    int sum = 0;
#pragma unroll
    for (int dy = -1; dy <= 1; ++dy)
#pragma unroll
        for (int dx = -1; dx <= 1; ++dx) {
            const int nx_ = bx + dx, ny_ = by + dy;
            int v = own;
            if (nx_ >= 0 && ny_ >= 0 && nx_ < A.tiles_x * 4 && ny_ < A.tiles_y * 4) {
                long long nl;
                if (part_has((long long)(ny_ >> 2) * A.tiles_x + (nx_ >> 2), A.part, A.nparts, A.tile_begin, A.tile_end, nl)) v = pilot[nl * 16 + (ny_ & 3) * 4 + (nx_ & 3)];
            }
            sum += v;
        }
    if (sum8) sum8[g] = (unsigned char)(sum < 255 ? sum : 255);
    const int abs_sum = (int)A.queue[kQueueThr + 1];
    const bool is_long = sum >= (abs_sum > 0 && abs_sum < long_sum ? abs_sum : long_sum);
    const int lx = 2 * (sub & 3), ly = 2 * (sub >> 2);
#pragma unroll
    for (int q = 0; q < 4; ++q) {
        const int px = lx + (q & 1), py = ly + (q >> 1);
        const bool in_img = (tx * 8 + px < A.max_x) && (ty * 8 + py < A.max_y);
        const long long pid = local_tile * 64 + py * 8 + px;
        long_flag[pid] = (is_long && in_img) ? 1 : 0;
        if (is_long && in_img) {
            if (sum >= solo_sum) { const unsigned int pos = atomicAdd(A.queue + 4, 1u); long_list[A.n_local_tiles * 64 - 1 - pos] = (unsigned int)pid; }
            else { const unsigned int pos = atomicAdd(A.queue + 2, 1u); long_list[pos] = (unsigned int)pid; }
        }
    }
}

__global__ __launch_bounds__(1024) void k_tile_order(const int* __restrict__ cost, unsigned int* __restrict__ order, long long n, unsigned int* __restrict__ queue,
                                                    int ns, int n_lanes, float f_inflight, float f_static, float f_tail, long long tail_cap_tiles, unsigned int* __restrict__ tail_ws, int head_sum, float head_min_load) {
    if (tail_ws && threadIdx.x < 512) tail_ws[threadIdx.x] = 0u;
    __shared__ int s_cnt[16][8];
    __shared__ long long s_sum[16];
    __shared__ long long s_ccost[16][8];
    const int lane = threadIdx.x & 63, wave = threadIdx.x >> 6;
    const long long per = ((n + 15) / 16 + 63) / 64 * 64;
    const long long lo = wave * per, hi = (lo + per < n) ? lo + per : n;
    int cnt[8] = {0, 0, 0, 0, 0, 0, 0, 0};
    long long csum = 0;
    long long ccost[8] = {0, 0, 0, 0, 0, 0, 0, 0};
    for (long long t0 = lo + lane; t0 < hi; t0 += 512) {
        int wv[8];
#pragma unroll
        for (int u = 0; u < 8; ++u) wv[u] = (t0 + 64 * u < hi) ? cost[t0 + 64 * u] : -1;
#pragma unroll
        for (int u = 0; u < 8; ++u) {
            const int w = wv[u] < 0 ? 0 : wv[u];
            const int c = wv[u] < 0 ? -1 : cost_class(w);
            csum += w;
#pragma unroll
            for (int k = 0; k < 8; ++k) { cnt[k] += (c == k) ? 1 : 0; ccost[k] += (c == k) ? w : 0; }
        }
    }
#pragma unroll
    for (int k = 0; k < 8; ++k) {
        for (int off = 32; off > 0; off >>= 1) ccost[k] += __shfl_xor(ccost[k], off);
        if (lane == 0) s_ccost[wave][k] = ccost[k];
    }
#pragma unroll
    for (int k = 0; k < 8; ++k) {
        for (int off = 32; off > 0; off >>= 1) cnt[k] += __shfl_xor(cnt[k], off);
        if (lane == 0) s_cnt[wave][k] = cnt[k];
    }
    for (int off = 32; off > 0; off >>= 1) csum += __shfl_xor(csum, off);
    if (lane == 0) s_sum[wave] = csum;
    __syncthreads();
    if (threadIdx.x == 0 && queue && n_lanes > 0 && ns > 0) {
        long long tot = 0;
        for (int w = 0; w < 16; ++w) tot += s_sum[w];
        const double load = (double)tot * 0.5 * (double)ns / (double)n_lanes;
        double ti = (double)f_inflight * load, tsum = 18.0 * (double)f_static * load / (double)ns;
        if (ti < (double)RT_LONG_RATE_MIN * ns) ti = (double)RT_LONG_RATE_MIN * ns;
        if (tsum < (double)RT_PILOT_LONG_SUM_MIN) tsum = (double)RT_PILOT_LONG_SUM_MIN;
        unsigned int tail_mark = 0u;
        if (f_tail > 0.f && tot > 0) {
            const double want = (1.0 - (double)f_tail) * (double)tot;
            double cum = 0.0; long long r0 = n;
            long long start = 0;
#pragma unroll 1
            for (int k = 7; k >= 0; --k) {
                long long nk = 0, ck = 0;
#pragma unroll 1
                for (int w = 0; w < 16; ++w) { nk += s_cnt[w][k]; ck += s_ccost[w][k]; }
                if (nk > 0 && cum + (double)ck >= want) { r0 = start + (long long)((want - cum) / ((double)ck / (double)nk)); break; }
                cum += (double)ck; start += nk;
            }
            r0 = (r0 / 64) * 64;
            if (r0 < n && (n - r0) <= tail_cap_tiles) tail_mark = (unsigned int)(r0 * 64 + 1);
        }
        queue[kQueueThr + 2] = tail_mark;
        if (load < (double)head_min_load) head_sum = 0;
        queue[kQueueThr + 4] = (tail_mark != 0u && head_sum > 0) ? (unsigned int)(head_sum > 255 ? 255 : head_sum) : (tail_mark != 0u && head_sum < 0) ? (unsigned int)(-head_sum >= 254 ? 255 : -head_sum + 1) : 0u;
        queue[kQueueThr + 5] = (tail_mark != 0u && head_sum < 0) ? 1u : 0u;
        queue[kQueueThr] = f_inflight > 0.f ? (unsigned int)(ti < 1.0 ? 1.0 : (ti > 4.0e9 ? 4.0e9 : ti)) : 0u;
        queue[kQueueThr + 1] = f_static > 0.f ? (unsigned int)(tsum < 1.0 ? 1.0 : (tsum > 1.0e9 ? 1.0e9 : tsum)) : 0u;
    }
    __shared__ int s_tot[8];
    __shared__ int s_base[16][8];
    if (threadIdx.x < 8) {
        int all = 0;
#pragma unroll 1
        for (int w = 0; w < 16; ++w) all += s_cnt[w][threadIdx.x];
        s_tot[threadIdx.x] = all;
    }
    __syncthreads();
    if (threadIdx.x < 128) {
        const int w0 = threadIdx.x >> 3, k0 = threadIdx.x & 7;
// ... 232 lines not shown
    return hipGetLastError();
}

hipError_t launch_render_init(rt_rand_state* rs, int max_x, int max_y, int part, int nparts, long long begin, long long end, hipStream_t st) {
    const int tiles_x = (max_x + 7) / 8, tiles_y = (max_y + 7) / 8;
    const long long tiles = (long long)tiles_x * tiles_y;
    const long long local = part_local_tiles(tiles, part, nparts, begin, end);
    if (local <= 0) return hipSuccess;
    const unsigned blocks = (unsigned)((local + 3) / 4);
    hipLaunchKernelGGL(k_render_init, dim3(blocks), dim3(256), 0, st, rs, max_x, max_y, tiles_x, part, nparts, begin, end, local);
    return hipGetLastError();
}
#endif

static size_t tree_lds_bytes(int n_nodes, bool pool = false) { return (size_t)n_nodes * sizeof(DevNode) + (pool ? 4 * sizeof(WalkLds) + kHotSlots * sizeof(float4) : 0); }

template <class K> static unsigned resident_blocks(K kernel, size_t lds) {
    int dev = 0, cus = 0, per_cu = 0;
    if (hipGetDevice(&dev) != hipSuccess) return 1024u;
    if (hipDeviceGetAttribute(&cus, hipDeviceAttributeMultiprocessorCount, dev) != hipSuccess || cus <= 0) return 1024u;
    if (hipOccupancyMaxActiveBlocksPerMultiprocessor(&per_cu, kernel, 256, lds) != hipSuccess || per_cu <= 0) per_cu = 4;
    return (unsigned)(cus * per_cu);
}

#if defined(RT_TU_LIST) || !defined(RT_SPLIT_LIST)
#ifdef RT_TU_LIST
#define RT_LIST_FN(name) name##_list
#else
#define RT_LIST_FN(name) static name##_list
#endif
hipError_t RT_LIST_FN(launch_tile_cost)(const RenderArgs& A, unsigned blocks, int* cost, unsigned char* pilot, hipStream_t st) {
    hipLaunchKernelGGL((k_tile_cost<false>), dim3(blocks), dim3(256), 0, st, A, cost, pilot, (int*)nullptr);
    return hipGetLastError();
}
hipError_t RT_LIST_FN(launch_render)(const RenderArgs& A, int mode, hipStream_t st) {
    const unsigned need = (unsigned)((A.n_local_tiles + 3) / 4);
    const unsigned cap = mode == 0 ? resident_blocks(k_render<false, 0, 1>, 0) : resident_blocks(k_render<false, 1, 1>, 0);
    const unsigned blocks = need < cap ? need : cap;
    if (mode == 0) hipLaunchKernelGGL((k_render<false, 0, 1>), dim3(blocks), dim3(256), 0, st, A);
    else hipLaunchKernelGGL((k_render<false, 1, 1>), dim3(blocks), dim3(256), 0, st, A);
    return hipGetLastError();
}
hipError_t RT_LIST_FN(launch_trace)(const RenderArgs& A, unsigned blocks, const float* rays, long long n, rt_hit_record* out, hipStream_t st) {
    hipLaunchKernelGGL((k_trace<false>), dim3(blocks), dim3(256), 0, st, A, rays, n, out);
    return hipGetLastError();
}
#ifndef RT_TU_CONTRACT
hipError_t RT_LIST_FN(launch_guides)(const RenderArgs& A, unsigned blocks, long long n, rt_hit_record* out, hipStream_t st) {
    hipLaunchKernelGGL((k_guides<false>), dim3(blocks), dim3(256), 0, st, A, n, out);
    return hipGetLastError();
}
hipError_t RT_LIST_FN(launch_render_adaptive)(const RenderArgs& A, hipStream_t st) {
    const unsigned need = (unsigned)((A.n_local_tiles + 3) / 4);
    const unsigned cap = resident_blocks(k_render<false, 2, 1>, 0);
    hipLaunchKernelGGL((k_render<false, 2, 1>), dim3(need < cap ? need : cap), dim3(256), 0, st, A);
    return hipGetLastError();
}
#endif
#else
hipError_t launch_tile_cost_list(const RenderArgs& A, unsigned blocks, int* cost, unsigned char* pilot, hipStream_t st);
hipError_t launch_render_list(const RenderArgs& A, int mode, hipStream_t st);
hipError_t launch_trace_list(const RenderArgs& A, unsigned blocks, const float* rays, long long n, rt_hit_record* out, hipStream_t st);
hipError_t launch_guides_list(const RenderArgs& A, unsigned blocks, long long n, rt_hit_record* out, hipStream_t st);
hipError_t launch_render_adaptive_list(const RenderArgs& A, hipStream_t st);
#endif

#ifndef RT_TU_LIST
static int render_variant(bool tree, int mode, const DevAccel& acc) {
    (void)mode;
    if (!tree) return 0;
    if (acc.enabled) return acc.coop_groups >= 4 ? (acc.solo_chains ? 5 : 4) : 2;
    return 1;
}
const char* render_kernel_name(bool tree, int mode, const DevAccel& acc) {
    switch (render_variant(tree, mode, acc)) {
        case 0: return mode == 0 ? "k_render<false,0,1>" : "k_render<false,1,1>";
        case 4: return mode == 0 ? "k_render<true,0,4>" : "k_render<true,1,4>";
        case 5: return mode == 0 ? "k_render<true,0,5>" : "k_render<true,1,5>";
        case 2: return mode == 0 ? "k_render<true,0,2>" : "k_render<true,1,2>";
        default: return mode == 0 ? "k_render<true,0,1>" : "k_render<true,1,1>";
    }
}

hipError_t launch_select_and_order(const RenderArgs& A, int* cost, unsigned int* order, unsigned char* flags, unsigned int* long_list, hipStream_t st, int long_sum, int solo_sum) {
    const bool tail = flags && A.tail_list && A.tail_ws && A.f_tail > 0.f;
    hipLaunchKernelGGL(k_tile_order, dim3(1), dim3(1024), 0, st, (const int*)cost, order, (long long)A.n_local_tiles, A.queue, (int)A.ns, (int)A.n_lanes, A.f_inflight, A.f_static,
                       tail ? A.f_tail : 0.f, (long long)A.n_local_tiles, tail ? A.tail_ws : (unsigned int*)nullptr, tail ? A.head_sum : 0, A.head_min_load);
    if (flags) {
        const unsigned char* pilot = flags + (size_t)A.n_local_tiles * 64;
        unsigned char* sum8 = flags + (size_t)A.n_local_tiles * 80;
        hipLaunchKernelGGL(k_long_select, dim3((unsigned)((A.n_local_tiles * 16 + 255) / 256)), dim3(256), 0, st, A, pilot, flags, long_list, long_sum > 0 ? long_sum : RT_PILOT_LONG_SUM, solo_sum, sum8);
        if (tail) {
            const unsigned nb = (unsigned)((A.n_local_tiles * 16 + kTailChunk - 1) / kTailChunk);
            hipLaunchKernelGGL(k_tail_hist, dim3(nb), dim3(256), 0, st, (const unsigned int*)order, (const unsigned char*)sum8, (long long)A.n_local_tiles, (const unsigned int*)A.queue, A.tail_ws);
            hipLaunchKernelGGL(k_tail_scatter, dim3(nb), dim3(256), 0, st, (const unsigned int*)order, (const unsigned char*)sum8, (unsigned int*)A.tail_list, (long long)A.n_local_tiles, A.queue, A.tail_ws);
        }
    }
    return hipGetLastError();
}

static unsigned render_grid_blocks(const RenderArgs& A, int variant, int mode);
hipError_t launch_pilot(const RenderArgs& A, bool tree, int* cost, unsigned char* pilot, int* work, hipStream_t st) {
    if (A.n_local_tiles <= 0) return hipSuccess;
    const long long per_block = 4 * (64 / (16 * RT_PILOT_SAMPLES));
    const unsigned blocks = (unsigned)((A.n_local_tiles + per_block - 1) / per_block);
    const int variant = render_variant(tree, 0, A.tree.acc);
    if (variant == 5) hipLaunchKernelGGL((k_tile_cost<true, 5>), dim3(blocks), dim3(256), tree_lds_bytes(A.tree.n_nodes, true), st, A, cost, pilot, work);
    else if (variant == 4) hipLaunchKernelGGL((k_tile_cost<true, 4>), dim3(blocks), dim3(256), tree_lds_bytes(A.tree.n_nodes, true), st, A, cost, pilot, work);
    else if (variant == 2) hipLaunchKernelGGL((k_tile_cost<true, 2>), dim3(blocks), dim3(256), tree_lds_bytes(A.tree.n_nodes, true), st, A, cost, pilot, work);
    else if (tree) hipLaunchKernelGGL((k_tile_cost<true, 1>), dim3(blocks), dim3(256), tree_lds_bytes(A.tree.n_nodes), st, A, cost, pilot, work);
    else return launch_tile_cost_list(A, blocks, cost, pilot, st);
    return hipGetLastError();
}

hipError_t launch_tile_order(const RenderArgs& A, bool tree, int* cost, unsigned int* order, unsigned char* flags, unsigned int* long_list, hipStream_t st) {
    if (A.n_local_tiles <= 0) return hipSuccess;
    unsigned char* pilot = flags ? flags + (size_t)A.n_local_tiles * 64 : nullptr;
    const int variant = render_variant(tree, 0, A.tree.acc);
    RenderArgs B = A;
    B.n_lanes = tree ? (int)render_grid_blocks(A, variant, 0) * 256 : 0;
    if (variant == 2 && A.f_inflight_dense > 0.f) B.f_inflight = A.f_inflight_dense;
    B.head_sum = variant == 2 ? A.head_sum_dense : A.head_sum;
    B.head_min_load = variant == 2 ? A.head_min_load : 0.f;
    { const hipError_t e = launch_pilot(A, tree, cost, pilot, nullptr, st); if (e != hipSuccess) return e; }
    return launch_select_and_order(B, cost, order, flags, long_list, st, 0, variant == 5 ? RT_PILOT_SOLO_SUM : 0x7fffffff);
}

template <int MODE, int COOPG>
static unsigned tree_grid_blocks(const RenderArgs& A, size_t lds) {
    const unsigned need = (unsigned)((A.n_local_tiles + 3) / 4);
    thread_local int c_dev = -1; thread_local size_t c_lds = 0; thread_local unsigned c_cap = 0;
    int dev = 0;
    if (hipGetDevice(&dev) != hipSuccess) dev = -2;
    if (dev != c_dev || lds != c_lds || c_cap == 0) { c_cap = resident_blocks(k_render<true, MODE, COOPG>, lds); c_dev = dev; c_lds = lds; }
    const unsigned cap = c_cap;
    return need < cap ? need : cap;
}
template <int MODE, int COOPG>
static hipError_t launch_render_tree(const RenderArgs& A, size_t lds, hipStream_t st) {
    hipLaunchKernelGGL((k_render<true, MODE, COOPG>), dim3(tree_grid_blocks<MODE, COOPG>(A, lds)), dim3(256), lds, st, A);
    return hipGetLastError();
}
static unsigned render_grid_blocks(const RenderArgs& A, int variant, int mode) {
    const size_t lds = tree_lds_bytes(A.tree.n_nodes, variant != 1);
    if (variant == 5) return mode == 0 ? tree_grid_blocks<0, 5>(A, lds) : tree_grid_blocks<1, 5>(A, lds);
    if (variant == 4) return mode == 0 ? tree_grid_blocks<0, 4>(A, lds) : tree_grid_blocks<1, 4>(A, lds);
    if (variant == 2) return mode == 0 ? tree_grid_blocks<0, 2>(A, lds) : tree_grid_blocks<1, 2>(A, lds);
    return mode == 0 ? tree_grid_blocks<0, 1>(A, lds) : tree_grid_blocks<1, 1>(A, lds);
}

hipError_t launch_render(const RenderArgs& A, bool tree, int mode, hipStream_t st) {
    if (A.n_local_tiles <= 0) return hipSuccess;
    const int variant = render_variant(tree, mode, A.tree.acc);
    if (variant == 0) return launch_render_list(A, mode, st);
    const size_t lds = tree_lds_bytes(A.tree.n_nodes, variant != 1);
    if (variant == 5) return mode == 0 ? launch_render_tree<0, 5>(A, lds, st) : launch_render_tree<1, 5>(A, lds, st);
    if (variant == 4) return mode == 0 ? launch_render_tree<0, 4>(A, lds, st) : launch_render_tree<1, 4>(A, lds, st);
    if (variant == 2) return mode == 0 ? launch_render_tree<0, 2>(A, lds, st) : launch_render_tree<1, 2>(A, lds, st);
    return mode == 0 ? launch_render_tree<0, 1>(A, lds, st) : launch_render_tree<1, 1>(A, lds, st);
}

#ifndef RT_TU_CONTRACT
hipError_t launch_render_adaptive(const RenderArgs& A, bool tree, hipStream_t st) {
    if (A.n_local_tiles <= 0) return hipSuccess;
    const int variant = render_variant(tree, 0, A.tree.acc);
    if (variant == 0) return launch_render_adaptive_list(A, st);
    const size_t lds = tree_lds_bytes(A.tree.n_nodes, variant != 1);
    if (variant == 5) return launch_render_tree<2, 5>(A, lds, st);
    if (variant == 4) return launch_render_tree<2, 4>(A, lds, st);
    if (variant == 2) return launch_render_tree<2, 2>(A, lds, st);
    return launch_render_tree<2, 1>(A, lds, st);
}
hipError_t launch_adapt_check(float* fb, const float* sl, const float* q, const unsigned int* list_in, const unsigned int* count_in, long long n_all,
                              unsigned int* list_out, unsigned int* count_out, int32_t* spp, int k, bool last, float rel_error, float floor_lum,
                              const AdaptFrame& fr, hipStream_t st) {
    if (n_all <= 0) return hipSuccess;
    hipLaunchKernelGGL(k_adapt_check, dim3((unsigned)((n_all + 255) / 256)), dim3(256), 0, st, fb, sl, q, list_in, count_in, n_all, list_out, count_out, spp,
                       k, last ? 1 : 0, rel_error, floor_lum, fr);
    return hipGetLastError();
}
hipError_t launch_adapt_check_keep(float* fb, const AdaptState& s, const unsigned int* list_in, const unsigned int* count_in, long long n_all,
                                   unsigned int* list_out, unsigned int* count_out, int32_t* spp, int k, bool last, float rel_error, float floor_lum,
                                   const AdaptFrame& fr, hipStream_t st) {
    if (n_all <= 0) return hipSuccess;
    hipLaunchKernelGGL(k_adapt_check_keep, dim3((unsigned)((n_all + 255) / 256)), dim3(256), 0, st, fb, s, list_in, count_in, n_all, list_out, count_out, spp,
                       k, last ? 1 : 0, rel_error, floor_lum, fr);
    return hipGetLastError();
}
hipError_t launch_adapt_refine_seed(float* fb, const AdaptState& s, long long n_all, unsigned int* list_out, unsigned int* count_out, int32_t* spp,
                                    int max_spp, float rel_error, float floor_lum, const AdaptFrame& fr, hipStream_t st) {
    if (n_all <= 0) return hipSuccess;
    hipLaunchKernelGGL(k_adapt_refine_seed, dim3((unsigned)((n_all + 255) / 256)), dim3(256), 0, st, fb, s, n_all, list_out, count_out, spp,
                       max_spp, rel_error, floor_lum, fr);
    return hipGetLastError();
}
hipError_t launch_adapt_refine_check(float* fb, const AdaptState& s, const unsigned int* list_in, const unsigned int* count_in, long long n_all,
                                     unsigned int* list_out, unsigned int* count_out, int32_t* spp, int batch, int max_spp, float rel_error, float floor_lum,
                                     hipStream_t st) {
    if (n_all <= 0) return hipSuccess;
    hipLaunchKernelGGL(k_adapt_refine_check, dim3((unsigned)((n_all + 255) / 256)), dim3(256), 0, st, fb, s, list_in, count_in, list_out, count_out, spp,
                       batch, max_spp, rel_error, floor_lum);
    return hipGetLastError();
}
hipError_t launch_adapt_zero(unsigned int* p, int n, hipStream_t st) {
    if (n <= 0) return hipSuccess;
    hipLaunchKernelGGL(k_adapt_zero, dim3((unsigned)((n + 255) / 256)), dim3(256), 0, st, p, n);
    return hipGetLastError();
}
// ... 57 lines not shown
```

### dd2360-raytracing_amd/csrc/rt_sched_keep.h

```cpp
#pragma once
#include <cstdint>

namespace rt {

struct SchedKey {
    uint64_t world = 0, tree = 0;
    int32_t max_x = 0, max_y = 0;
    int32_t part = 0, nparts = 0;
    int64_t tile_begin = 0, tile_end = 0;
    int32_t traversal = 0;
    int32_t ns = 0;
    int32_t half = 0;
    int32_t device = 0;
};
inline bool sched_key_equal(const SchedKey& a, const SchedKey& b) {
    return a.world == b.world && a.tree == b.tree && a.max_x == b.max_x && a.max_y == b.max_y && a.part == b.part && a.nparts == b.nparts &&
           a.tile_begin == b.tile_begin && a.tile_end == b.tile_end && a.traversal == b.traversal && a.ns == b.ns && a.half == b.half &&
           a.device == b.device;
}

constexpr int kSchedKeptWords = 8;

enum SchedAction {
    kSchedBypass = 0,
    kSchedCompute = 1,
    kSchedReuse = 2,
};

struct SchedKeep {
    bool valid = false;
    bool captured = false;
    SchedKey key;
    uint64_t reused = 0, computed = 0;
};

inline SchedAction sched_keep_decide(SchedKeep& K, const SchedKey& key, bool enabled, bool capturing) {
    if (capturing) K.captured = true;
    if (capturing || K.captured || !enabled) { K.valid = false; ++K.computed; return kSchedBypass; }
    if (K.valid && sched_key_equal(K.key, key)) { ++K.reused; return kSchedReuse; }
    K.valid = false; ++K.computed;
    return kSchedCompute;
}
inline void sched_keep_commit(SchedKeep& K, const SchedKey& key) {
    if (K.captured) return;
    K.key = key; K.valid = true;
}
inline void sched_keep_drop(SchedKeep& K) { K.valid = false; }

}
```

### dd2360-raytracing_amd/csrc/rt_stats.h

```cpp
#pragma once
#ifdef RT_STATS
enum { ST_RAYS, ST_FAST, ST_SLOW, ST_TIE, ST_COLS, ST_TESTS, ST_DISCPOS, ST_OFFERS, ST_ELIG, ST_ELIG_NODES, ST_A_ITERS_WAVE, ST_B_ROUNDS_WAVE,
       ST_LOOP_ITERS_WAVE, ST_A_LANE_STEPS, ST_B_LANES, ST_SAMPLES, ST_LIVE_GE56, ST_LIVE_32, ST_LIVE_8, ST_LIVE_LT8, ST_SWITCHES,
       ST_CYC_TOTAL, ST_CYC_CLOSEST, ST_CYC_WALK_A, ST_CYC_WALK_B, ST_CYC_SCAN, ST_CYC_SHADE, ST_REALTIME,
       ST_SPARE0, ST_SPARE1, ST_SPARE2, ST_SPARE3, ST_SPARE4, ST_SPARE5, ST_SPARE6,
       WP_GROUND, WP_LARGE_K, WP_LARGE_EXACT, WP_OFFER_NODE, WP_OFFER_RAYBOX, WP_ELIG_FN, WP_ELIG_LIST, WP_SETUP, WP_A_COL, WP_A_BATCH, WP_A_HOLD,
       WP_B_OFFER, WP_B_CLIP, WP_COOP_CHUNK, WP_SCAN, WP_SC_ANY, WP_SC_LAMB, WP_SC_METAL, WP_SC_DIEL, WP_REJ_ITER, WP_PRIMARY, WP_DISK_ITER, WP_SKY, WP_ENDPIX,
       TH_GROUND, TH_LARGE_SETUP, TH_WALK, TH_SCAN,
       TR_ROUNDS, TR_SEG0, TR_SEG1, TR_SEG4, TR_SEG16, TR_SEGMORE, TR_LE64, ST_N };
#ifdef RT_STATS_LIGHT
#define TICK() 0ull
#else
#define TICK() ((unsigned long long)__builtin_amdgcn_s_memtime())
#endif
__device__ unsigned long long g_stats[ST_N];
__device__ int g_pilot_dbg[1 << 20];
__device__ unsigned long long g_wave_dbg[8192 * 4];
struct Stats { unsigned int c[ST_N]; unsigned long long cyc[8]; };
#ifdef RT_STATS_LIGHT
#define STAT(st, k, v) ((void)0)
#define TRSTAT_ROUND(lane, n_seg, total) ((void)0)
#else
#define STAT(st, k, v) ((st).c[k] += (v))
#define TRSTAT_ROUND(lane, n_seg, total) do { if ((lane) == 0) { atomicAdd(&g_stats[TR_ROUNDS], 1ull); \
    atomicAdd(&g_stats[(n_seg) == 0u ? TR_SEG0 : (n_seg) == 1u ? TR_SEG1 : (n_seg) <= 4u ? TR_SEG4 : (n_seg) <= 16u ? TR_SEG16 : TR_SEGMORE], 1ull); \
    if ((total) <= 64u) atomicAdd(&g_stats[TR_LE64], 1ull); } } while (0)
#endif
constexpr int kWpBlocks = WP_ENDPIX - WP_GROUND + 1;
__device__ unsigned long long g_wp_cls[4 * kWpBlocks];
#ifdef RT_STATS_WPASS
__shared__ int s_wp_cls[4];
#define WPASS(k) do { const int l_ = (int)(threadIdx.x & 63); if (__builtin_amdgcn_readfirstlane(l_) == l_) { atomicAdd(&g_stats[k], 1ull); \
    atomicAdd(&g_wp_cls[(s_wp_cls[(threadIdx.x >> 6) & 3] & 3) * kWpBlocks + ((k) - WP_GROUND)], 1ull); } } while (0)
#define WPASS_CLASS(c) do { const int l_ = (int)(threadIdx.x & 63); if (__builtin_amdgcn_readfirstlane(l_) == l_) s_wp_cls[(threadIdx.x >> 6) & 3] = (c); } while (0)
#else
#define WPASS(k) ((void)0)
#define WPASS_CLASS(c) ((void)0)
#endif
#define STAT_ARG , Stats& st
#define STAT_PASS , st
#define RT_STATS_ONLY(...) __VA_ARGS__
#define RT_STATS_READERS \
hipError_t read_pilot_dbg(int* out, int n) { return hipMemcpyFromSymbol(out, HIP_SYMBOL(g_pilot_dbg), sizeof(int) * (size_t)(n < (1 << 20) ? n : (1 << 20))); } \
hipError_t read_wave_dbg(unsigned long long* out) { return hipMemcpyFromSymbol(out, HIP_SYMBOL(g_wave_dbg), sizeof(unsigned long long) * 8192 * 4); } \
hipError_t read_wp_classes(unsigned long long* out, int reset) { \
    hipError_t e = hipMemcpyFromSymbol(out, HIP_SYMBOL(g_wp_cls), sizeof(unsigned long long) * 4 * kWpBlocks); \
    if (e != hipSuccess) return e; \
    if (reset) { unsigned long long z[4 * kWpBlocks] = {0}; e = hipMemcpyToSymbol(HIP_SYMBOL(g_wp_cls), z, sizeof(z)); } \
    return e; \
} \
hipError_t read_stats(unsigned long long* out, int reset) { \
    hipError_t e = hipMemcpyFromSymbol(out, HIP_SYMBOL(g_stats), sizeof(unsigned long long) * ST_N); \
    if (e != hipSuccess) return e; \
    if (reset) { unsigned long long z[ST_N] = {0}; e = hipMemcpyToSymbol(HIP_SYMBOL(g_stats), z, sizeof(z)); } \
    return e; \
}
#else
#define STAT(st, k, v) ((void)0)
#define WPASS(k) ((void)0)
#define WPASS_CLASS(c) ((void)0)
#define STAT_ARG
#define STAT_PASS
#define RT_STATS_ONLY(...)
#define RT_STATS_READERS
#endif
```

### dd2360-raytracing_amd/csrc/rt_tuning.h

```cpp
#pragma once

#ifndef RT_RENDER_WAVES
#define RT_RENDER_WAVES 4
#endif

#ifndef RT_LONG_RATE
#define RT_LONG_RATE 14
#endif
#ifndef RT_LONG_RATE_DENSE
#define RT_LONG_RATE_DENSE 20
#endif
#ifndef RT_LONG_CHECK
#define RT_LONG_CHECK 4
#endif
#ifndef RT_F_INFLIGHT
#define RT_F_INFLIGHT 1.35f
#endif
#ifndef RT_F_INFLIGHT_DENSE
#define RT_F_INFLIGHT_DENSE 1.1f
#endif

#ifndef RT_F_STATIC
#define RT_F_STATIC 1.07f
#endif
#ifndef RT_HEAD_SUM_SPARSE
#define RT_HEAD_SUM_SPARSE 1
#endif
#ifndef RT_HEAD_SUM_DENSE
#define RT_HEAD_SUM_DENSE -21
#endif
#ifndef RT_HEAD_LOAD_DENSE
#define RT_HEAD_LOAD_DENSE 3500
#endif
#ifndef RT_F_TAIL
#define RT_F_TAIL 0.15f
#endif
#ifndef RT_INTERLEAVE
#define RT_INTERLEAVE 64
#endif
#ifndef RT_INTERLEAVE_DENSE
#define RT_INTERLEAVE_DENSE 16
#endif
#ifndef RT_INTERLEAVE_SOLO
#define RT_INTERLEAVE_SOLO 1
#endif
#ifndef RT_LONG_RATE_MIN
#define RT_LONG_RATE_MIN 8
#endif
#ifndef RT_PILOT_LONG_SUM_MIN
#define RT_PILOT_LONG_SUM_MIN 120
#endif
#ifndef RT_MED_RATE
#define RT_MED_RATE 12
#endif
#ifndef RT_THIN_CAP_DEN
#define RT_THIN_CAP_DEN 4
#endif
#ifndef RT_LONG_PER_WAVE
#define RT_LONG_PER_WAVE 16
#endif
#ifndef RT_PILOT_SAMPLES
#define RT_PILOT_SAMPLES 2
#endif
#ifndef RT_PILOT_LONG_SUM
#define RT_PILOT_LONG_SUM 200
#endif
#ifndef RT_SOLO_DENSITY
#define RT_SOLO_DENSITY 1.0
#endif
#ifndef RT_PILOT_SOLO_SUM
#define RT_PILOT_SOLO_SUM 200
#endif
#ifndef RT_PILOT_CAP
#define RT_PILOT_CAP 35
#endif
#ifndef RT_SCHED_CACHE
#define RT_SCHED_CACHE 1
#endif
#ifndef RT_PROG_OWN
#define RT_PROG_OWN 64
#endif

#ifndef RT_SPLIT_WB
#define RT_SPLIT_WB 1000
#endif
#ifndef RT_SPLIT_WT
#define RT_SPLIT_WT 17
#endif
#ifndef RT_SPLIT_WC
#define RT_SPLIT_WC 0
#endif

#ifndef RT_ACCEL_FINE
#define RT_ACCEL_FINE 8
#endif
#ifndef RT_DENSE_CELL
#define RT_DENSE_CELL 0.7
#endif
#ifndef RT_SPARSE_CELL
#define RT_SPARSE_CELL 1.0
#endif

#ifndef RT_QUORUM_SPARSE
#define RT_QUORUM_SPARSE 4
#endif
#ifndef RT_QUORUM_DENSE
#define RT_QUORUM_DENSE 2
#endif
#ifndef RT_QUORUM_MIN
#define RT_QUORUM_MIN 16
#endif
#ifndef RT_POOL_COLS
#define RT_POOL_COLS 2
#endif
#ifndef RT_POOL_COLS_THIN
#define RT_POOL_COLS_THIN 4
#endif
#ifndef RT_POOL_THIN_ROUND
#define RT_POOL_THIN_ROUND 1
#endif
#ifndef RT_POOL_SPANS
#define RT_POOL_SPANS 1
#endif
#ifndef RT_POOL_DIRECT
#define RT_POOL_DIRECT 1
#endif
#ifndef RT_DENSE_PB
#define RT_DENSE_PB 4
#endif
#ifndef RT_DENSE_DRAIN
#define RT_DENSE_DRAIN 32
#endif

#ifndef RT_LIST_BATCH
#define RT_LIST_BATCH 8
#endif
#ifndef RT_LIST_COOP_COST
#define RT_LIST_COOP_COST 16
#endif

#ifndef RT_H16_MINWAVES
#define RT_H16_MINWAVES 4
#endif
#ifndef RT_H16_BIG
#define RT_H16_BIG 128
#endif
#ifndef RT_H16_SMALL
#define RT_H16_SMALL 256
#endif
#ifndef RT_H16_INTERLEAVE
#define RT_H16_INTERLEAVE 64
#endif
#ifndef RT_H16_TASKS
#define RT_H16_TASKS 384
#endif
#ifndef RT_H16_PP
#define RT_H16_PP 10
#endif
#ifndef RT_H16_LONG_PER_WAVE
#define RT_H16_LONG_PER_WAVE 16
// ... 17 lines not shown
```

### dd2360-raytracing_amd/rt_amd.py

```python
import ctypes as C
import os
import numpy as np

_HERE = os.path.dirname(os.path.abspath(__file__))
LIB_PATH = os.environ.get("RT_AMD_LIB", os.path.join(_HERE, "librt_amd.so"))

FP32, FP16 = 0, 1
MAT_NONE, MAT_LAMBERTIAN, MAT_METAL, MAT_DIELECTRIC = -1, 0, 1, 2
OCTREE_MAX_NODES = 585
TRAVERSAL_REFERENCE, TRAVERSAL_FAST = 0, 1
ARITH_IEEE, ARITH_CONTRACT = 0, 1
IMAGE_P3, IMAGE_P6, IMAGE_PFM = 0, 1, 2

rand_state_dtype = np.dtype([("d", "<u4"), ("v", "<u4", 5), ("boxmuller_flag", "<i4"), ("boxmuller_flag_double", "<i4"),
                             ("boxmuller_extra", "<f4"), ("pad_", "<u4"), ("boxmuller_extra_double", "<f8")])
sphere_dtype = np.dtype([("center", "<f4", 3), ("radius", "<f4"), ("material", "<i4"), ("albedo", "<f4", 3), ("param", "<f4")])
camera_dtype = np.dtype([("origin", "<f4", 3), ("lower_left_corner", "<f4", 3), ("horizontal", "<f4", 3), ("vertical", "<f4", 3),
                         ("u", "<f4", 3), ("v", "<f4", 3), ("w", "<f4", 3), ("lens_radius", "<f4")])
octnode_dtype = np.dtype([("level", "<i4"), ("aabb", "<f4", 6), ("children", "<i4", 8)])
hit_record_dtype = np.dtype([("t", "<f4"), ("p", "<f4", 3), ("normal", "<f4", 3), ("sphere", "<i4")])
assert rand_state_dtype.itemsize == 48 and sphere_dtype.itemsize == 36 and camera_dtype.itemsize == 88
assert octnode_dtype.itemsize == 60 and hit_record_dtype.itemsize == 32


class RtError(RuntimeError):
    pass


class Partition(C.Structure):
    _fields_ = [("part", C.c_int32), ("nparts", C.c_int32), ("tile_begin", C.c_int64), ("tile_end", C.c_int64)]


WHOLE = Partition(0, 1)
PART_RUN = 64
SCHEDULE_FIELDS = ("inflight_thr", "static_thr", "tail_mark", "head", "head_thr", "from_end", "long_raw", "solo_raw")

class Adaptive(C.Structure):
    _fields_ = [("min_spp", C.c_int32), ("max_spp", C.c_int32), ("batch", C.c_int32), ("rel_error", C.c_float), ("floor", C.c_float)]

ADAPTIVE_STATE_BYTES = 24


class Budget(C.Structure):
    _fields_ = [("samples", C.c_int64), ("rounds", C.c_int32), ("batch", C.c_int32), ("max_spp", C.c_int32), ("floor", C.c_float)]


class DenoiseParams(C.Structure):
    _fields_ = [("input", C.c_int32), ("samples", C.c_int32), ("levels", C.c_int32), ("normal_pow_log2", C.c_int32),
                ("sigma_position", C.c_float), ("sigma_color", C.c_float)]

DENOISE_INPUT_GAMMA, DENOISE_INPUT_SUM = 0, 1
DENOISE_MAX_LEVELS = 8
DENOISE_MAX_PIXELS = 1 << 30
DENOISE_WORK_BYTES = 32
DENOISE_DEFAULTS = dict(levels=2, normal_pow_log2=4, sigma_position=0.01, sigma_color=0.3)


def denoise_params(input=DENOISE_INPUT_GAMMA, samples=1, **kw):
    p = dict(DENOISE_DEFAULTS)
    p.update(kw)
    return DenoiseParams(input, samples, p["levels"], p["normal_pow_log2"], p["sigma_position"], p["sigma_color"])


class DenoiseVarParams(C.Structure):
    _fields_ = [("levels", C.c_int32), ("normal_pow_log2", C.c_int32), ("prefilter", C.c_int32), ("sigma_position", C.c_float),
                ("sigma_variance", C.c_float)]

DENOISE_VAR_EPS = 1e-8
DENOISE_VAR_DEFAULTS = dict(levels=1, normal_pow_log2=4, prefilter=1, sigma_position=0.01, sigma_variance=4.0)


def denoise_var_params(**kw):
    p = dict(DENOISE_VAR_DEFAULTS)
    p.update(kw)
    return DenoiseVarParams(p["levels"], p["normal_pow_log2"], p["prefilter"], p["sigma_position"], p["sigma_variance"])


class TemporalParams(C.Structure):
    _fields_ = [("max_history", C.c_int32), ("reuse_specular", C.c_int32), ("position_tolerance", C.c_float), ("normal_min_dot", C.c_float)]

TEMPORAL_HISTORY_BYTES = 20
TEMPORAL_DEFAULTS = dict(max_history=32, reuse_specular=0, position_tolerance=0.03, normal_min_dot=0.9)


def temporal_params(**kw):
    p = dict(TEMPORAL_DEFAULTS)
    p.update(kw)
    return TemporalParams(p["max_history"], p["reuse_specular"], p["position_tolerance"], p["normal_min_dot"])


class TemporalInputs(C.Structure):
    _fields_ = [("d_hist_in", C.c_void_p), ("d_hits", C.c_void_p), ("d_hits_prev", C.c_void_p), ("cam_prev", C.c_void_p)]


def temporal_inputs(d_hits, d_hist_in=None, d_hits_prev=None, cam_prev=None):
    ptr = lambda t: None if t is None else (t if isinstance(t, int) else t.data_ptr())
    t = TemporalInputs(ptr(d_hist_in), ptr(d_hits), ptr(d_hits_prev), None)
    t._keep = (d_hits, d_hist_in, d_hits_prev)
    if cam_prev is not None:
        t._cam = np.ascontiguousarray(cam_prev, camera_dtype).reshape(1).copy()
        t.cam_prev = t._cam.ctypes.data
    return t


class LevelsParams(C.Structure):
    _fields_ = [("input", C.c_int32), ("samples", C.c_int32), ("format", C.c_int32), ("top_first", C.c_int32)]

LEVELS_RGB8, LEVELS_RGBA8, LEVELS_GRAY8 = 0, 1, 2


class FrameMetrics(C.Structure):
    _fields_ = [("pixels", C.c_int64), ("gray_sse", C.c_int64), ("gray_differ", C.c_int64), ("windows", C.c_int64), ("ssim_sum", C.c_double),
                ("finite_pixels", C.c_int64), ("sq_err", C.c_double), ("reserved", C.c_int64)]

    @property
    def psnr(self):
        return lib().rt_frame_psnr(C.byref(self))

    @property
    def ssim(self):
        return lib().rt_frame_ssim(C.byref(self))

    @property
    def rmse(self):
        return lib().rt_frame_rmse(C.byref(self))

assert C.sizeof(FrameMetrics) == 64 and C.sizeof(LevelsParams) == 16

_vp, _i, _i64, _f = C.c_void_p, C.c_int, C.c_int64, C.c_float
SYMBOLS = {
    "rt_abi_version": (_i, []),
    "rt_device_check": (_i, [_vp]),
    "rt_error_string": (C.c_char_p, [_i]),
    "rt_rand_init": (_i, [_vp]),
    "rt_create_world": (_i, [_vp, _i, _f, _vp, _i, _i, _vp, _i, _vp]),
    "rt_camera_init": (_i, [_vp, _vp, _vp, _vp, _f, _f, _f, _f, _i]),
    "rt_world_create": (_i, [_vp, _i, _vp, _i, _vp]),
    "rt_world_upload": (_i, [_vp]),
    "rt_world_set_camera": (_i, [_vp, _vp]),
    "rt_world_camera": (_i, [_vp, _vp]),
    "rt_world_set_geometry": (_i, [_vp, _vp, _vp]),
    "rt_world_get_geometry": (_i, [_vp, _vp, _vp]),
    "rt_free_world": (_i, [_vp]),
    "rt_build_octree": (_i, [_vp, _i, _i, _i, _vp]),
    "rt_octree_upload": (_i, [_vp]),
    "rt_build_octree_gpu": (_i, [_vp, _i, _vp, _vp]),
    "rt_octree_debug_array": (_i, [_vp, _i, _vp, C.c_size_t, _vp]),
    "rt_free_octree": (_i, [_vp]),
    "rt_octree_info": (_i, [_vp, _vp, _vp, _vp, _vp, _vp]),
    "rt_octree_flat_info": (_i, [_vp, _vp, _vp]),
    "rt_octree_set_traversal": (_i, [_vp, _i]),
    "rt_world_set_list_traversal": (_i, [_vp, _i]),
    "rt_world_set_arith": (_i, [_vp, _i]),
    "rt_world_list_accel_info": (_i, [_vp, _vp, _vp, _vp, _vp, _vp]),
    "rt_octree_accel_info": (_i, [_vp, _vp, _vp, _vp, _vp]),
    "rt_octree_nodes": (_i, [_vp, _vp]),
    "rt_octree_leaves": (_i, [_vp, _vp, _vp]),
    "rt_part_pixels": (_i64, [_i, _i, Partition]),
    "rt_render_init": (_i, [_i, _i, _vp, Partition, _vp]),
    "rt_render": (_i, [_vp, _i, _i, _i, _vp, _vp, _vp, Partition, _vp]),
    "rt_render_progressive": (_i, [_vp, _i, _i, _i, _vp, _vp, _vp, Partition, _vp]),
    "rt_world_render_times": (_i, [_vp, _vp, _i, _vp]),
    "rt_render_ctx_create": (_i, [_vp]),
    "rt_render_ctx_reserve": (_i, [_vp, _i, _i, Partition]),
    "rt_render_ctx_destroy": (_i, [_vp]),
    "rt_render_on": (_i, [_vp, _vp, _i, _i, _i, _vp, _vp, _vp, Partition, _vp]),
    "rt_render_progressive_on": (_i, [_vp, _vp, _i, _i, _i, _vp, _vp, _vp, Partition, _vp]),
    "rt_render_adaptive": (_i, [_vp, _i, _i, C.POINTER(Adaptive), _vp, _vp, _vp, _vp, _vp]),
    "rt_render_adaptive_on": (_i, [_vp, _vp, _i, _i, C.POINTER(Adaptive), _vp, _vp, _vp, _vp, _vp]),
    "rt_render_adaptive_part": (_i, [_vp, _i, _i, C.POINTER(Adaptive), _vp, _vp, _vp, _vp, Partition, _vp]),
    "rt_render_adaptive_part_on": (_i, [_vp, _vp, _i, _i, C.POINTER(Adaptive), _vp, _vp, _vp, _vp, Partition, _vp]),
    "rt_render_adaptive_begin": (_i, [_vp, _i, _i, C.POINTER(Adaptive), _vp, _vp, _vp, _vp, _vp, Partition, _vp]),
    "rt_render_adaptive_begin_on": (_i, [_vp, _vp, _i, _i, C.POINTER(Adaptive), _vp, _vp, _vp, _vp, _vp, Partition, _vp]),
    "rt_render_adaptive_refine": (_i, [_vp, _i, _i, C.POINTER(Adaptive), C.POINTER(Adaptive), _vp, _vp, _vp, _vp, _vp, Partition, _vp]),
    "rt_render_adaptive_refine_on": (_i, [_vp, _vp, _i, _i, C.POINTER(Adaptive), C.POINTER(Adaptive), _vp, _vp, _vp, _vp, _vp, Partition, _vp]),
    "rt_adaptive_priority": (_f, [_f, _f, _i, _f]),
    "rt_adaptive_budget_check": (_i, [C.POINTER(Budget)]),
    "rt_adaptive_budget_picks": (_i, [C.POINTER(Budget), _i, _vp]),
    "rt_adaptive_budget_select": (_i, [_vp, _vp, _i, _i, Partition, C.POINTER(Budget), _i64, _vp, _vp, _vp]),
    "rt_render_adaptive_spend": (_i, [_vp, _i, _i, C.POINTER(Budget), _vp, _vp, _vp, _vp, _vp, Partition, _vp, _vp]),
    "rt_render_adaptive_spend_on": (_i, [_vp, _vp, _i, _i, C.POINTER(Budget), _vp, _vp, _vp, _vp, _vp, Partition, _vp, _vp]),
    "rt_render_ctx_times": (_i, [_vp, _vp, _i, _vp]),
    "rt_render_ctx_counters": (_i, [_vp, _vp]),
    "rt_world_render_counters": (_i, [_vp, _vp]),
    "rt_render_ctx_schedule": (_i, [_vp, _vp, _i]),
    "rt_world_render_schedule": (_i, [_vp, _vp, _i]),
    "rt_render_ctx_schedule_reuse": (_i, [_vp, _vp, _vp]),
    "rt_world_render_schedule_reuse": (_i, [_vp, _vp, _vp]),
    "rt_render_kernel_name": (_i, [_vp, _vp, _i, _vp, _i]),
    "rt_multi_unique_id": (_i, [_vp]),
    "rt_multi_init": (_i, [_vp, _i, _i, _vp]),
    "rt_multi_probe": (_i, []),
    "rt_multi_init_custom": (_i, [_vp, _i, _i, _vp, _vp]),
    "rt_multi_destroy": (_i, [_vp]),
    "rt_multi_reserve": (_i, [_vp, _i, _i, _i, _i]),
    "rt_multi_render": (_i, [_vp, _vp, _i, _i, _i, _vp, _vp, _i, _i, _vp]),
    "rt_multi_render_adaptive": (_i, [_vp, _vp, _i, _i, C.POINTER(Adaptive), _vp, _vp, _i, _i, _vp, _vp]),
    "rt_multi_last_render_ms": (_i, [_vp, _vp, _vp]),
    "rt_multi_selftest": (_i, [_vp, _vp, _vp, C.c_size_t, _vp]),
    "rt_assemble": (_i, [_vp, _vp, _i, _i, _i, _i, _vp]),
    "rt_assemble_split": (_i, [_vp, _vp, _i, _i, _i, _vp, _i64, _i, _vp]),
    "rt_split_balanced": (_i, [_vp, _vp, _vp, _i, _i, _i, _vp, _vp, _vp, _vp, _vp]),
    "rt_multi_set_split": (_i, [_vp, _i]),
    "rt_multi_last_split": (_i, [_vp, _vp]),
    "rt_trace_rays": (_i, [_vp, _vp, _vp, _i64, _vp, _vp]),
    "rt_render_guides": (_i, [_vp, _vp, _i, _i, _vp, _vp]),
    "rt_denoise": (_i, [_vp, _vp, _i, _i, _vp, C.POINTER(DenoiseParams), _vp, _vp]),
    "rt_denoise_check": (_i, [_i, _i, C.POINTER(DenoiseParams)]),
    "rt_denoise_adaptive": (_i, [_vp, _vp, _i, _i, _vp, _vp, C.POINTER(DenoiseVarParams), _vp, _vp]),
    "rt_denoise_adaptive_check": (_i, [_i, _i, C.POINTER(DenoiseVarParams)]),
    "rt_temporal_check": (_i, [_i, _i, C.POINTER(TemporalParams)]),
    "rt_temporal_accumulate": (_i, [_vp, _vp, _vp, _vp, _vp, _vp, _vp, _i, _i, C.POINTER(TemporalParams), _vp]),
    "rt_temporal_accumulate_moving": (_i, [_vp, _vp, _vp, _vp, _vp, _vp, _vp, _vp, _i, _i, C.POINTER(TemporalParams), _vp]),
    "rt_denoise_history": (_i, [_vp, _vp, _i, _i, _vp, _vp, C.POINTER(DenoiseVarParams), _vp, _vp]),
    "rt_adaptive_priority_filtered": (_f, [_f, _f, _f]),
    "rt_adaptive_budget_select_filtered": (_i, [_vp, _vp, _vp, _i, _i, C.POINTER(Budget), C.POINTER(DenoiseVarParams), _i64, _vp, _vp, _vp, _vp]),
    "rt_render_adaptive_spend_filtered": (_i, [_vp, _i, _i, C.POINTER(Budget), C.POINTER(DenoiseVarParams), _vp, _vp, _vp, _vp, _vp, _vp, _vp, _vp]),
    "rt_render_adaptive_spend_filtered_on": (_i, [_vp, _vp, _i, _i, C.POINTER(Budget), C.POINTER(DenoiseVarParams), _vp, _vp, _vp, _vp, _vp, _vp, _vp, _vp]),
    "rt_adaptive_budget_select_temporal": (_i, [_vp, _vp, _vp, _i, _i, C.POINTER(Budget), C.POINTER(TemporalInputs), C.POINTER(TemporalParams), _i64,
                                                _vp, _vp, _vp, _vp]),
    "rt_render_adaptive_spend_temporal": (_i, [_vp, _i, _i, C.POINTER(Budget), C.POINTER(TemporalInputs), C.POINTER(TemporalParams), _vp, _vp, _vp, _vp,
                                               _vp, _vp, _vp]),
    "rt_render_adaptive_spend_temporal_on": (_i, [_vp, _vp, _i, _i, C.POINTER(Budget), C.POINTER(TemporalInputs), C.POINTER(TemporalParams), _vp, _vp, _vp,
                                                  _vp, _vp, _vp, _vp]),
    "rt_frame_levels": (_i, [_vp, _vp, _i, _i, _i, C.POINTER(LevelsParams), _vp]),
    "rt_frame_levels_check": (_i, [_i, _i, _i, C.POINTER(LevelsParams)]),
    "rt_frame_levels_bytes": (_i64, [_i, _i, _i]),
    "rt_frame_compare_work_bytes": (_i64, [_i, _i]),
    "rt_frame_compare": (_i, [_vp, _i, _vp, _i, _i, _i, _vp, _vp, _vp, _vp]),
    "rt_frame_psnr": (C.c_double, [C.POINTER(FrameMetrics)]),
    "rt_frame_ssim": (C.c_double, [C.POINTER(FrameMetrics)]),
    "rt_frame_rmse": (C.c_double, [C.POINTER(FrameMetrics)]),
    "rt_write_ppm": (_i, [C.c_char_p, _i, _i, _vp, _i]),
    "rt_format_ppm": (_i64, [_i, _i, _vp, _i, _vp, _i64]),
    "rt_write_image": (_i, [C.c_char_p, _i, _i, _vp, _i, _i]),
}

_LIB = None


def lib():
    global _LIB
    if _LIB is None:
        if not os.path.exists(LIB_PATH):
            raise RtError("librt_amd.so is not built (%s): run __graft_entry__.build() / make -C dd2360-raytracing_amd" % LIB_PATH)
        try:
            import torch
        except ImportError:
            pass
        try:
            L = C.CDLL(LIB_PATH)
        except OSError as e:
            raise RtError("cannot load %s: %s" % (LIB_PATH, e))
        for name, (res, args) in SYMBOLS.items():
            try:
                fn = getattr(L, name)
            except AttributeError:
                raise RtError("librt_amd.so does not export %s" % name)
            fn.restype, fn.argtypes = res, args
        _LIB = L
    return _LIB


def check(rc, what):
    if rc != 0:
        msg = lib().rt_error_string(int(rc))
        raise RtError("%s failed: %d (%s)" % (what, rc, msg.decode() if msg else "?"))


def _np(a):
    return a.ctypes.data_as(C.c_void_p)
# ... 29 lines not shown
        check(lib().rt_render_on(self.h, _dev(fb), max_x, max_y, ns, world.h, _dev(d_rand_state), octree.h if octree is not None else None,
                                 part or WHOLE, C.c_void_p(stream) if stream is not None else _stream()), "rt_render_on")

    def render_adaptive(self, fb, max_x, max_y, params, world, d_rand_state, octree=None, d_spp=None, stream=None):
        check(lib().rt_render_adaptive_on(self.h, _dev(fb), max_x, max_y, C.byref(params), world.h, _dev(d_rand_state),
                                          octree.h if octree is not None else None, _dev(d_spp) if d_spp is not None else None,
                                          C.c_void_p(stream) if stream is not None else _stream()), "rt_render_adaptive_on")

    def render_adaptive_part(self, fb, max_x, max_y, params, world, d_rand_state, octree=None, d_spp=None, part=None, stream=None):
        check(lib().rt_render_adaptive_part_on(self.h, _dev(fb), max_x, max_y, C.byref(params), world.h, _dev(d_rand_state),
                                               octree.h if octree is not None else None, _dev(d_spp) if d_spp is not None else None,
                                               part or WHOLE, C.c_void_p(stream) if stream is not None else _stream()), "rt_render_adaptive_part_on")

    def render_adaptive_begin(self, fb, max_x, max_y, params, world, d_rand_state, d_state, octree=None, d_spp=None, part=None, stream=None):
        check(lib().rt_render_adaptive_begin_on(self.h, _dev(fb), max_x, max_y, C.byref(params), world.h, _dev(d_rand_state),
                                                octree.h if octree is not None else None, _dev(d_spp) if d_spp is not None else None, _dev(d_state),
                                                part or WHOLE, C.c_void_p(stream) if stream is not None else _stream()), "rt_render_adaptive_begin_on")

    def render_adaptive_refine(self, fb, max_x, max_y, frm, to, world, d_rand_state, d_state, octree=None, d_spp=None, part=None, stream=None):
        check(lib().rt_render_adaptive_refine_on(self.h, _dev(fb), max_x, max_y, C.byref(frm), C.byref(to), world.h, _dev(d_rand_state),
                                                 octree.h if octree is not None else None, _dev(d_spp) if d_spp is not None else None, _dev(d_state),
                                                 part or WHOLE, C.c_void_p(stream) if stream is not None else _stream()), "rt_render_adaptive_refine_on")

    def render_adaptive_spend(self, fb, max_x, max_y, params, world, d_rand_state, d_state, octree=None, d_spp=None, part=None, d_picked=None,
                              stream=None):
        check(lib().rt_render_adaptive_spend_on(self.h, _dev(fb), max_x, max_y, C.byref(params), world.h, _dev(d_rand_state),
                                                octree.h if octree is not None else None, _dev(d_spp) if d_spp is not None else None, _dev(d_state),
                                                part or WHOLE, _dev(d_picked) if d_picked is not None else None,
                                                C.c_void_p(stream) if stream is not None else _stream()), "rt_render_adaptive_spend_on")

    def adaptive_budget_select(self, d_state, max_x, max_y, params, picks, d_list, d_count, part=None, stream=None):
        check(lib().rt_adaptive_budget_select(self.h, _dev(d_state), max_x, max_y, part or WHOLE, C.byref(params), picks, _dev(d_list), _dev(d_count),
                                              C.c_void_p(stream) if stream is not None else _stream()), "rt_adaptive_budget_select")

    def render_adaptive_spend_filtered(self, fb, max_x, max_y, params, filter, d_hits, world, d_rand_state, d_state, octree=None, d_spp=None,
                                       d_picked=None, stream=None):
        check(lib().rt_render_adaptive_spend_filtered_on(self.h, _dev(fb), max_x, max_y, C.byref(params), C.byref(filter), _dev(d_hits), world.h,
                                                         _dev(d_rand_state), octree.h if octree is not None else None,
                                                         _dev(d_spp) if d_spp is not None else None, _dev(d_state),
                                                         _dev(d_picked) if d_picked is not None else None,
                                                         C.c_void_p(stream) if stream is not None else _stream()), "rt_render_adaptive_spend_filtered_on")

    def adaptive_budget_select_filtered(self, d_state, d_hits, max_x, max_y, params, filter, picks, d_list, d_count, d_keys=None, stream=None):
        check(lib().rt_adaptive_budget_select_filtered(self.h, _dev(d_state), _dev(d_hits), max_x, max_y, C.byref(params), C.byref(filter), picks,
                                                       _dev(d_list), _dev(d_count), _dev(d_keys) if d_keys is not None else None,
                                                       C.c_void_p(stream) if stream is not None else _stream()), "rt_adaptive_budget_select_filtered")

    def render_adaptive_spend_temporal(self, fb, max_x, max_y, params, inputs, temporal, world, d_rand_state, d_state, octree=None, d_spp=None,
                                       d_picked=None, stream=None):
        check(lib().rt_render_adaptive_spend_temporal_on(self.h, _dev(fb), max_x, max_y, C.byref(params), C.byref(inputs), C.byref(temporal), world.h,
                                                         _dev(d_rand_state), octree.h if octree is not None else None,
                                                         _dev(d_spp) if d_spp is not None else None, _dev(d_state),
                                                         _dev(d_picked) if d_picked is not None else None,
                                                         C.c_void_p(stream) if stream is not None else _stream()), "rt_render_adaptive_spend_temporal_on")

    def adaptive_budget_select_temporal(self, d_state, world, max_x, max_y, params, inputs, temporal, picks, d_list, d_count, d_keys=None,
                                        stream=None):
        check(lib().rt_adaptive_budget_select_temporal(self.h, _dev(d_state), world.h, max_x, max_y, C.byref(params), C.byref(inputs),
                                                       C.byref(temporal), picks, _dev(d_list), _dev(d_count),
                                                       _dev(d_keys) if d_keys is not None else None,
                                                       C.c_void_p(stream) if stream is not None else _stream()), "rt_adaptive_budget_select_temporal")

    def times(self):
        out = np.zeros(64, np.float32)
        n = C.c_int(0)
        check(lib().rt_render_ctx_times(self.h, _np(out), 64, C.byref(n)), "rt_render_ctx_times")
        return out[: n.value].tolist()

    def counters(self):
        out = np.zeros(4, np.uint32)
        check(lib().rt_render_ctx_counters(self.h, _np(out)), "rt_render_ctx_counters")
        return dict(zip(("slots", "thin_waves", "long_chains", "long_handles"), (int(v) for v in out)))

    def schedule(self):
        out = np.zeros(len(SCHEDULE_FIELDS), np.uint32)
        check(lib().rt_render_ctx_schedule(self.h, _np(out), len(out)), "rt_render_ctx_schedule")
        return dict(zip(SCHEDULE_FIELDS, (int(v) for v in out)))

    def schedule_reuse(self):
        a, b = C.c_uint64(0), C.c_uint64(0)
        check(lib().rt_render_ctx_schedule_reuse(self.h, C.byref(a), C.byref(b)), "rt_render_ctx_schedule_reuse")
        return a.value, b.value

    def close(self):
        if getattr(self, "h", None):
            lib().rt_render_ctx_destroy(self.h)
            self.h = None

    def __del__(self):
        try:
            self.close()
        except Exception:
            pass


SPLIT_RUNS, SPLIT_BALANCED, SPLIT_BALANCED_CACHED = 0, 1, 2
GATHER_FN = C.CFUNCTYPE(C.c_int, C.c_void_p, C.c_void_p, C.c_size_t, C.c_void_p, C.c_size_t, C.c_int, C.c_void_p)
MULTI_ID_BYTES = 128


def multi_unique_id():
    buf = C.create_string_buffer(MULTI_ID_BYTES)
    check(lib().rt_multi_unique_id(buf), "rt_multi_unique_id")
    return buf.raw


def multi_probe():
    return int(lib().rt_multi_probe())


class Multi:

    def __init__(self, rank, nranks, unique_id=None, gather=None):
        h = C.c_void_p()
        if gather is not None:
            self._cb = GATHER_FN(gather)
            check(lib().rt_multi_init_custom(C.byref(h), rank, nranks, C.cast(self._cb, C.c_void_p), None), "rt_multi_init_custom")
        else:
            assert unique_id is not None and len(unique_id) == MULTI_ID_BYTES
            self._id = C.create_string_buffer(unique_id, MULTI_ID_BYTES)
            check(lib().rt_multi_init(C.byref(h), rank, nranks, self._id), "rt_multi_init")
        self.h, self.rank, self.nranks = h, rank, nranks
        self.split_mode = SPLIT_RUNS

    def reserve(self, max_x, max_y, precision=FP32, root=0):
        check(lib().rt_multi_reserve(self.h, max_x, max_y, precision, root), "rt_multi_reserve")
        return self

    def render(self, fb_full, max_x, max_y, ns, world, octree=None, root=0, precision=None):
        check(lib().rt_multi_render(self.h, _dev(fb_full) if fb_full is not None else None, max_x, max_y, ns, world.h,
                                    octree.h if octree is not None else None, world.precision if precision is None else precision,
                                    root, _stream()), "rt_multi_render")

    def render_adaptive(self, fb_full, max_x, max_y, params, world, octree=None, root=0, d_spp_full=None, precision=None):
        check(lib().rt_multi_render_adaptive(self.h, _dev(fb_full) if fb_full is not None else None, max_x, max_y, C.byref(params), world.h,
                                             octree.h if octree is not None else None, world.precision if precision is None else precision,
                                             root, _dev(d_spp_full) if d_spp_full is not None else None, _stream()), "rt_multi_render_adaptive")

    def set_split(self, mode):
        check(lib().rt_multi_set_split(self.h, mode), "rt_multi_set_split")
        self.split_mode = mode
        return self

    def last_split(self):
        st = (C.c_int64 * (self.nranks + 1))()
        check(lib().rt_multi_last_split(self.h, st), "rt_multi_last_split")
        return list(st)

    def last_render_ms(self):
        a, b = C.c_float(0), C.c_float(0)
        check(lib().rt_multi_last_render_ms(self.h, C.byref(a), C.byref(b)), "rt_multi_last_render_ms")
        return a.value, b.value

    def selftest(self, d_src, d_dst, nbytes):
        check(lib().rt_multi_selftest(self.h, _dev(d_src), _dev(d_dst), nbytes, _stream()), "rt_multi_selftest")

    def close(self):
        if getattr(self, "h", None):
            lib().rt_multi_destroy(self.h)
            self.h = None

    def __del__(self):
        try:
            self.close()
        except Exception:
            pass
# ... 47 lines not shown
            self.camera = np.zeros(1, camera_dtype)
            created = C.c_int(0)
            check(L.rt_rand_init(_np(self.rand_state)), "rt_rand_init")
            check(L.rt_create_world(_np(self.spheres), num_spheres, sphere_radius, _np(self.camera), nx, ny, _np(self.rand_state),
                                    precision, C.byref(created)), "rt_create_world")
            self.created = created.value
        else:
            self.spheres = np.ascontiguousarray(spheres, sphere_dtype)
            self.camera = np.ascontiguousarray(camera, camera_dtype).reshape(1)
            self.created = int((self.spheres["material"] != MAT_NONE).sum())
        h = C.c_void_p()
        check(L.rt_world_create(_np(self.spheres), num_spheres, _np(self.camera), precision, C.byref(h)), "rt_world_create")
        self.h = h

    def upload(self):
        check(lib().rt_world_upload(self.h), "rt_world_upload")
        return self

    def set_camera(self, cam):
        cam = np.ascontiguousarray(cam, camera_dtype).reshape(1).copy()
        check(lib().rt_world_set_camera(self.h, _np(cam)), "rt_world_set_camera")
        self.camera = cam
        return self

    def get_camera(self):
        cam = np.zeros(1, camera_dtype)
        check(lib().rt_world_camera(self.h, _np(cam)), "rt_world_camera")
        return cam

    def set_geometry(self, d_geom):
        check(lib().rt_world_set_geometry(self.h, _dev(d_geom), _stream()), "rt_world_set_geometry")
        self._spheres_stale = True
        return self

    def get_geometry(self, d_out=None):
        if d_out is None:
            import torch
            d_out = torch.empty((self.num_spheres, 4), dtype=torch.float32, device="cuda")
        check(lib().rt_world_get_geometry(self.h, _dev(d_out), _stream()), "rt_world_get_geometry")
        return d_out

    def host_spheres(self):
        if getattr(self, "_spheres_stale", False):
            g = self.get_geometry().cpu().numpy()
            self.spheres["center"] = g[:, :3]
            self.spheres["radius"] = g[:, 3]
            self._spheres_stale = False
        return self.spheres

    def set_list_traversal(self, mode):
        check(lib().rt_world_set_list_traversal(self.h, mode), "rt_world_set_list_traversal")
        return self

    def set_arith(self, mode):
        check(lib().rt_world_set_arith(self.h, mode), "rt_world_set_arith")
        return self

    def list_accel_info(self):
        e, g, h, n, l = C.c_int(0), C.c_int(0), C.c_float(0), C.c_int(0), C.c_int(0)
        check(lib().rt_world_list_accel_info(self.h, C.byref(e), C.byref(g), C.byref(h), C.byref(n), C.byref(l)), "rt_world_list_accel_info")
        return {"enabled": bool(e.value), "grid_dim": g.value, "cell_size": h.value, "grid_entries": n.value, "large_spheres": l.value}

    def render_times(self):
        out = np.zeros(64, np.float32)
        n = C.c_int(0)
        check(lib().rt_world_render_times(self.h, _np(out), 64, C.byref(n)), "rt_world_render_times")
        return out[: n.value].tolist()

    def render_counters(self):
        out = np.zeros(4, np.uint32)
        check(lib().rt_world_render_counters(self.h, _np(out)), "rt_world_render_counters")
        return dict(zip(("slots", "thin_waves", "long_chains", "long_handles"), (int(v) for v in out)))

    def render_schedule(self):
        out = np.zeros(len(SCHEDULE_FIELDS), np.uint32)
        check(lib().rt_world_render_schedule(self.h, _np(out), len(out)), "rt_world_render_schedule")
        return dict(zip(SCHEDULE_FIELDS, (int(v) for v in out)))

    def schedule_reuse(self):
        a, b = C.c_uint64(0), C.c_uint64(0)
        check(lib().rt_world_render_schedule_reuse(self.h, C.byref(a), C.byref(b)), "rt_world_render_schedule_reuse")
        return a.value, b.value

    def close(self):
        if getattr(self, "h", None):
            lib().rt_free_world(self.h)
            self.h = None

    def __del__(self):
        try:
            self.close()
        except Exception:
            pass


class Octree:

    def __init__(self, world, spheres_per_leaf=30, gpu=False):
        L = lib()
        self.world, self.spl = world, spheres_per_leaf
        h = C.c_void_p()
        if gpu:
            check(L.rt_build_octree_gpu(world.h, spheres_per_leaf, C.byref(h), _stream()), "rt_build_octree_gpu")
        else:
            check(L.rt_build_octree(_np(world.host_spheres()), world.num_spheres, spheres_per_leaf, world.precision, C.byref(h)), "rt_build_octree")
        self.h = h

    def upload(self):
        check(lib().rt_octree_upload(self.h), "rt_octree_upload")
        return self

    def set_traversal(self, mode):
        check(lib().rt_octree_set_traversal(self.h, mode), "rt_octree_set_traversal")
        return self

    def device_array(self, which):
        n = C.c_size_t(0)
        check(lib().rt_octree_debug_array(self.h, which, None, 0, C.byref(n)), "rt_octree_debug_array")
        buf = np.zeros(max(1, n.value), np.uint8)
        check(lib().rt_octree_debug_array(self.h, which, _np(buf), n.value, C.byref(n)), "rt_octree_debug_array")
        return buf[: n.value]

    def accel_info(self):
        g, n, l = C.c_int(0), C.c_int(0), C.c_int(0)
        h = C.c_float(0)
        check(lib().rt_octree_accel_info(self.h, C.byref(g), C.byref(h), C.byref(n), C.byref(l)), "rt_octree_accel_info")
        return dict(grid_dim=g.value, cell_size=h.value, grid_entries=n.value, large_spheres=l.value)

    def info(self):
        v = [C.c_int(0) for _ in range(5)]
        check(lib().rt_octree_info(self.h, *[C.byref(x) for x in v]), "rt_octree_info")
        fn, fe = C.c_int(0), C.c_int(0)
        check(lib().rt_octree_flat_info(self.h, C.byref(fn), C.byref(fe)), "rt_octree_flat_info")
        keys = ["node_count", "leaf_count", "spl", "dropped_full", "dropped_outside"]
        d = dict(zip(keys, [x.value for x in v]))
        d.update(flat_nodes=fn.value, flat_entries=fe.value)
        return d

    def nodes(self):
        out = np.zeros(OCTREE_MAX_NODES, octnode_dtype)
        check(lib().rt_octree_nodes(self.h, _np(out)), "rt_octree_nodes")
        return out

    def leaves(self):
        lc = self.info()["leaf_count"]
        counts = np.zeros(lc, np.int32)
        idx = np.zeros((lc, self.spl), np.int32)
        check(lib().rt_octree_leaves(self.h, _np(counts), _np(idx)), "rt_octree_leaves")
        return counts, idx

    def close(self):
        if getattr(self, "h", None):
            lib().rt_free_octree(self.h)
            self.h = None

    def __del__(self):
        try:
            self.close()
        except Exception:
            pass


def camera_init(lookfrom, lookat, vup, vfov, aspect, aperture, focus_dist, precision=FP32):
    cam = np.zeros(1, camera_dtype)
    a = [np.asarray(x, np.float32) for x in (lookfrom, lookat, vup)]
    check(lib().rt_camera_init(_np(cam), _np(a[0]), _np(a[1]), _np(a[2]), vfov, aspect, aperture, focus_dist, precision), "rt_camera_init")
# ... 219 lines not shown
```

### include/rt_amd.h

```cpp
#ifndef RT_AMD_H
#define RT_AMD_H
#include <stdint.h>
#include <stddef.h>

#ifdef __cplusplus
extern "C" {
#endif

#define RT_ABI_VERSION 6

#define RT_EINVAL (-1)
#define RT_ENOMEM (-2)
#define RT_EIO (-3)
#define RT_ENOTSUP (-4)
#define RT_ECOMM (-5)

#define RT_PRECISION_FP32 0
#define RT_PRECISION_FP16 1

#define RT_MAT_NONE (-1)
#define RT_MAT_LAMBERTIAN 0
#define RT_MAT_METAL 1
#define RT_MAT_DIELECTRIC 2

// ... 82 lines not shown
int rt_octree_accel_info(const rt_octree* octree, int* grid_dim, float* cell_size, int* grid_entries, int* large_spheres);
int rt_octree_info(const rt_octree* octree, int* node_count, int* leaf_count, int* spheres_per_leaf,
                   int* dropped_full, int* dropped_outside);
int rt_octree_nodes(const rt_octree* octree, rt_octnode* out_nodes );
int rt_octree_leaves(const rt_octree* octree, int32_t* counts, int32_t* indices);

int64_t rt_part_pixels(int max_x, int max_y, rt_partition part);

int rt_render_init(int max_x, int max_y, rt_rand_state* d_rand_state, rt_partition part, void* stream);

int rt_render(void* fb, int max_x, int max_y, int ns, const rt_world* world, rt_rand_state* d_rand_state,
              const rt_octree* d_octree, rt_partition part, void* stream);

int rt_render_progressive(void* fb, int max_x, int max_y, int current_sample, const rt_world* world,
                          rt_rand_state* d_rand_state, const rt_octree* d_octree, rt_partition part, void* stream);

int rt_render_ctx_create(rt_render_ctx** out);
int rt_render_ctx_reserve(rt_render_ctx* ctx, int max_x, int max_y, rt_partition part);
int rt_render_ctx_destroy(rt_render_ctx* ctx);
int rt_render_on(rt_render_ctx* ctx, void* fb, int max_x, int max_y, int ns, const rt_world* world, rt_rand_state* d_rand_state,
                 const rt_octree* d_octree, rt_partition part, void* stream);
int rt_render_progressive_on(rt_render_ctx* ctx, void* fb, int max_x, int max_y, int current_sample, const rt_world* world,
                             rt_rand_state* d_rand_state, const rt_octree* d_octree, rt_partition part, void* stream);
int rt_render_ctx_times(rt_render_ctx* ctx, float* ms_out, int max, int* count);

typedef struct rt_adaptive {
    int32_t min_spp;
    int32_t max_spp;
    int32_t batch;
    float rel_error;
    float floor;
} rt_adaptive;
int rt_render_adaptive(void* fb, int max_x, int max_y, const rt_adaptive* params, const rt_world* world, rt_rand_state* d_rand_state,
                       const rt_octree* d_octree, int32_t* d_spp, void* stream);
int rt_render_adaptive_on(rt_render_ctx* ctx, void* fb, int max_x, int max_y, const rt_adaptive* params, const rt_world* world,
                          rt_rand_state* d_rand_state, const rt_octree* d_octree, int32_t* d_spp, void* stream);
int rt_render_adaptive_part(void* fb, int max_x, int max_y, const rt_adaptive* params, const rt_world* world, rt_rand_state* d_rand_state,
                            const rt_octree* d_octree, int32_t* d_spp, rt_partition part, void* stream);
int rt_render_adaptive_part_on(rt_render_ctx* ctx, void* fb, int max_x, int max_y, const rt_adaptive* params, const rt_world* world,
                               rt_rand_state* d_rand_state, const rt_octree* d_octree, int32_t* d_spp, rt_partition part, void* stream);

#define RT_ADAPTIVE_STATE_BYTES 24
int rt_render_adaptive_begin(void* fb, int max_x, int max_y, const rt_adaptive* params, const rt_world* world, rt_rand_state* d_rand_state,
                             const rt_octree* d_octree, int32_t* d_spp, void* d_state, rt_partition part, void* stream);
int rt_render_adaptive_begin_on(rt_render_ctx* ctx, void* fb, int max_x, int max_y, const rt_adaptive* params, const rt_world* world,
                                rt_rand_state* d_rand_state, const rt_octree* d_octree, int32_t* d_spp, void* d_state, rt_partition part, void* stream);
int rt_render_adaptive_refine(void* fb, int max_x, int max_y, const rt_adaptive* from, const rt_adaptive* to, const rt_world* world,
                              rt_rand_state* d_rand_state, const rt_octree* d_octree, int32_t* d_spp, void* d_state, rt_partition part, void* stream);
int rt_render_adaptive_refine_on(rt_render_ctx* ctx, void* fb, int max_x, int max_y, const rt_adaptive* from, const rt_adaptive* to,
                                 const rt_world* world, rt_rand_state* d_rand_state, const rt_octree* d_octree, int32_t* d_spp, void* d_state,
                                 rt_partition part, void* stream);

float rt_adaptive_priority(float SL, float Q, int k, float floor);
typedef struct rt_budget {
    int64_t samples;
    int32_t rounds;
    int32_t batch;
    int32_t max_spp;
    float floor;
} rt_budget;
int rt_adaptive_budget_check(const rt_budget* params);
int rt_adaptive_budget_picks(const rt_budget* params, int round, int64_t* picks);
int rt_adaptive_budget_select(rt_render_ctx* ctx, const void* d_state, int max_x, int max_y, rt_partition part, const rt_budget* params,
                              int64_t picks, uint32_t* d_list, uint32_t* d_count, void* stream);
int rt_render_adaptive_spend(void* fb, int max_x, int max_y, const rt_budget* params, const rt_world* world, rt_rand_state* d_rand_state,
                             const rt_octree* d_octree, int32_t* d_spp, void* d_state, rt_partition part, uint32_t* d_picked, void* stream);
int rt_render_adaptive_spend_on(rt_render_ctx* ctx, void* fb, int max_x, int max_y, const rt_budget* params, const rt_world* world,
                                rt_rand_state* d_rand_state, const rt_octree* d_octree, int32_t* d_spp, void* d_state, rt_partition part,
                                uint32_t* d_picked, void* stream);

int rt_render_kernel_name(const rt_world* world, const rt_octree* d_octree, int mode, char* out, int cap);

int rt_world_render_times(rt_world* world, float* ms_out, int max, int* count);

int rt_world_render_counters(rt_world* world, uint32_t* out4);
int rt_render_ctx_counters(rt_render_ctx* ctx, uint32_t* out4);

#define RT_SCHEDULE_WORDS 8
int rt_world_render_schedule(rt_world* world, uint32_t* out, int n);
int rt_render_ctx_schedule(rt_render_ctx* ctx, uint32_t* out, int n);

int rt_render_ctx_schedule_reuse(rt_render_ctx* ctx, uint64_t* reused, uint64_t* computed);
int rt_world_render_schedule_reuse(rt_world* world, uint64_t* reused, uint64_t* computed);

int rt_assemble(void* fb_full, const void* fb_parts, int max_x, int max_y, int nparts, int precision, void* stream);

int rt_split_balanced(rt_render_ctx* ctx, const rt_world* world, const rt_octree* d_octree, int max_x, int max_y, int nparts,
                      int64_t* starts , int32_t* tile_bounces, int32_t* tile_tests, int32_t* tile_columns, void* stream);
int rt_assemble_split(void* fb_full, const void* fb_parts, int max_x, int max_y, int nparts, const int64_t* starts, int64_t part_stride_px,
                      int precision, void* stream);

#define RT_MULTI_ID_BYTES 128
int rt_multi_unique_id(void* id_out );
int rt_multi_init(rt_multi** out, int rank, int nranks, const void* unique_id);
int rt_multi_probe(void);
typedef int (*rt_gather_fn)(void* user, const void* d_send, size_t send_bytes, void* d_parts, size_t part_stride_bytes, int root, void* stream);
int rt_multi_init_custom(rt_multi** out, int rank, int nranks, rt_gather_fn gather, void* user);
int rt_multi_destroy(rt_multi* m);
#define RT_SPLIT_RUNS 0
#define RT_SPLIT_BALANCED 1
#define RT_SPLIT_BALANCED_CACHED 2
int rt_multi_set_split(rt_multi* m, int mode);
int rt_multi_last_split(rt_multi* m, int64_t* starts);
int rt_multi_reserve(rt_multi* m, int max_x, int max_y, int precision, int root);
int rt_multi_render(rt_multi* m, void* fb_full, int max_x, int max_y, int ns, const rt_world* world, const rt_octree* d_octree,
                    int precision, int root, void* stream);
int rt_multi_render_adaptive(rt_multi* m, void* fb_full, int max_x, int max_y, const rt_adaptive* params, const rt_world* world,
                             const rt_octree* d_octree, int precision, int root, int32_t* d_spp_full, void* stream);
int rt_multi_last_render_ms(rt_multi* m, float* call_ms, float* kernel_ms);
int rt_multi_selftest(rt_multi* m, const void* d_src, void* d_dst, size_t bytes, void* stream);

int rt_trace_rays(const rt_world* world, const rt_octree* d_octree, const float* d_rays, int64_t n,
                  rt_hit_record* d_out, void* stream);

#define RT_DENOISE_MAX_PIXELS 1073741824
int rt_render_guides(const rt_world* world, const rt_octree* d_octree, int max_x, int max_y, rt_hit_record* d_hits, void* stream);

#define RT_DENOISE_INPUT_GAMMA 0
#define RT_DENOISE_INPUT_SUM 1
#define RT_DENOISE_MAX_LEVELS 8
#define RT_DENOISE_WORK_BYTES 32
#define RT_DENOISE_DEFAULT_LEVELS 2
#define RT_DENOISE_DEFAULT_NORMAL_POW_LOG2 4
#define RT_DENOISE_DEFAULT_SIGMA_POSITION 0.01f
#define RT_DENOISE_DEFAULT_SIGMA_COLOR 0.3f
typedef struct rt_denoise_params {
    int32_t input;
    int32_t samples;
    int32_t levels;
    int32_t normal_pow_log2;
    float sigma_position;
    float sigma_color;
} rt_denoise_params;
int rt_denoise(void* fb_out, const void* fb_in, int max_x, int max_y, const rt_hit_record* d_hits, const rt_denoise_params* params,
               void* d_work, void* stream);
int rt_denoise_check(int max_x, int max_y, const rt_denoise_params* params);

#define RT_DENOISE_VAR_EPS 1e-8f
#define RT_DENOISE_VAR_DEFAULT_LEVELS 1
#define RT_DENOISE_VAR_DEFAULT_NORMAL_POW_LOG2 4
#define RT_DENOISE_VAR_DEFAULT_PREFILTER 1
#define RT_DENOISE_VAR_DEFAULT_SIGMA_POSITION 0.01f
#define RT_DENOISE_VAR_DEFAULT_SIGMA_VARIANCE 4.0f
typedef struct rt_denoise_var_params {
    int32_t levels;
    int32_t normal_pow_log2;
    int32_t prefilter;
    float sigma_position;
    float sigma_variance;
} rt_denoise_var_params;
int rt_denoise_adaptive(void* fb_out, const void* fb_in, int max_x, int max_y, const rt_hit_record* d_hits, const void* d_state,
                        const rt_denoise_var_params* params, void* d_work, void* stream);
int rt_denoise_adaptive_check(int max_x, int max_y, const rt_denoise_var_params* params);

#define RT_TEMPORAL_HISTORY_BYTES 20
#define RT_TEMPORAL_DEFAULT_MAX_HISTORY 32
#define RT_TEMPORAL_DEFAULT_REUSE_SPECULAR 0
#define RT_TEMPORAL_DEFAULT_POSITION_TOLERANCE 0.03f
#define RT_TEMPORAL_DEFAULT_NORMAL_MIN_DOT 0.9f
typedef struct rt_temporal_params {
    int32_t max_history;
    int32_t reuse_specular;
    float position_tolerance;
    float normal_min_dot;
} rt_temporal_params;
int rt_temporal_check(int max_x, int max_y, const rt_temporal_params* params);
// ... 81 lines not shown
```

Baseline: 4837.

## Refine cached tile schedule using measured per-pixel iteration counts from prior frame

```diff
diff --git a/dd2360-raytracing_amd/csrc/rt_api.hip b/dd2360-raytracing_amd/csrc/rt_api.hip
--- a/dd2360-raytracing_amd/csrc/rt_api.hip
+++ b/dd2360-raytracing_amd/csrc/rt_api.hip
@@ -25,6 +25,9 @@
 hipError_t launch_render(const RenderArgs& A, bool tree, int mode, hipStream_t st);
 namespace fmac { hipError_t launch_render(const RenderArgs& A, bool tree, int mode, hipStream_t st); }
 hipError_t launch_tile_order(const RenderArgs& A, bool tree, int* cost, unsigned int* order, unsigned char* flags, unsigned int* long_list, hipStream_t st);
+int render_variant_of(bool tree, const DevAccel& acc);
+hipError_t launch_count_order(const RenderArgs& A, const unsigned short* iters, int* cost, unsigned int* order, unsigned char* flags, unsigned int* long_list,
+                              float solo_frac, int solo_cap_den, unsigned int* extra, hipStream_t st);
 hipError_t launch_render_h(const RenderArgs& A, bool tree, int mode, hipStream_t st);
 hipError_t launch_tile_order_h(const RenderArgs& A, bool tree, int* cost, unsigned int* order, unsigned char* flags, unsigned int* long_list, hipStream_t st);
 hipError_t launch_trace_h(const DevScene& S, const DevTree& T, bool tree, const float* rays, long long n, rt_hit_record* out, hipStream_t st);
@@ -84,6 +87,7 @@
 hipError_t read_wp_classes(unsigned long long* out, int reset);
 hipError_t read_wave_dbg(unsigned long long* out);
 hipError_t read_pilot_dbg(int* out, int n);
+hipError_t read_chain_dbg(unsigned int* out, int n_pixels);
 #endif
 }
 
@@ -272,7 +276,8 @@
 static DevGroup queue_group(rt_render_ctx& C) { return DevGroup().add(&C.d_queue, (kQueueSlots + 1) * kQueueStride * sizeof(unsigned int)); }
 static DevGroup sched_group(rt_render_ctx& C, size_t tiles) {
     return DevGroup().add(&C.d_cost, sizeof(int) * tiles).add(&C.d_order, sizeof(unsigned int) * tiles).add(&C.d_flags, tiles * 96)
-                     .add(&C.d_long, sizeof(unsigned int) * (tiles * 128 + 512)).add(&C.d_work, sizeof(int) * tiles * 2);
+                     .add(&C.d_long, sizeof(unsigned int) * (tiles * 128 + 512)).add(&C.d_work, sizeof(int) * tiles * 2)
+                     .add(&C.d_iters, sizeof(unsigned short) * tiles * 64);
 }
 static DevGroup progressive_group(rt_render_ctx& C, size_t tiles) { return DevGroup().add(&C.p_cost, sizeof(int) * tiles).add(&C.p_order, sizeof(unsigned int) * tiles); }
 static DevGroup adaptive_group(rt_render_ctx& C, size_t pixels) {
@@ -791,6 +796,7 @@
     clear_schedule(A);
     A.f_inflight = tune_value("RT_F_INFLIGHT", RT_F_INFLIGHT); A.f_inflight_dense = tune_value("RT_F_INFLIGHT_DENSE", RT_F_INFLIGHT_DENSE); A.f_static = tune_value("RT_F_STATIC", RT_F_STATIC);
     A.ad_list = nullptr; A.ad_count = nullptr; A.ad_sl = nullptr; A.ad_q = nullptr;
+    A.iters_out = nullptr;
     return A;
 }
 
@@ -838,10 +844,21 @@
     else RT_TRY(launch_zero_counters(A.queue, (int)kQueueStride, st));
     return 0;
 }
-static int schedule_frame(rt_render_ctx& C, RenderArgs& A, const rt_world* world, const rt_octree* d_octree, int ns, hipStream_t st, SchedAction act, const SchedKey& key) {
+static bool feedback_gate(const RenderArgs& A, const rt_world* world, const rt_octree* d_octree, int ns) {
+    const int min_ns = (int)tune_value("RT_FEEDBACK_MIN_NS", (float)RT_FEEDBACK_MIN_NS);
+    const bool half = world->precision == RT_PRECISION_FP16;
+    return sched_feedback_gate(ns, min_ns < 16 ? 16 : min_ns, half ? 0 : render_variant_of(d_octree != nullptr, A.tree.acc), half);
+}
+static bool feedback_enabled() { return tune_value("RT_SCHED_FEEDBACK", (float)RT_SCHED_FEEDBACK) != 0.f; }
+static int schedule_frame(rt_render_ctx& C, RenderArgs& A, const rt_world* world, const rt_octree* d_octree, int ns, hipStream_t st, SchedAction act, const SchedKey& key, bool refine) {
     const bool classify = ns >= 16;
     if (classify && world->precision != RT_PRECISION_FP16) { A.tail_list = C.d_long + (size_t)A.n_local_tiles * 64; A.tail_ws = C.d_long + (size_t)C.sched_tiles * 128; A.f_tail = tune_value("RT_F_TAIL", RT_F_TAIL); A.head_sum = (int)tune_value("RT_HEAD_SUM_SPARSE", (float)RT_HEAD_SUM_SPARSE); A.head_sum_dense = (int)tune_value("RT_HEAD_SUM_DENSE", (float)RT_HEAD_SUM_DENSE); A.head_min_load = tune_value("RT_HEAD_LOAD_DENSE", (float)RT_HEAD_LOAD_DENSE); }
-    if (act != kSchedReuse) {
+    if (refine) {
+        RT_TRY(launch_count_order(A, C.d_iters, C.d_cost, C.d_order, C.d_flags, C.d_long, tune_value("RT_FB_SOLO_FRAC", RT_FB_SOLO_FRAC),
+                                  (int)tune_value("RT_FB_SOLO_CAP_DEN", (float)RT_FB_SOLO_CAP_DEN), C.d_kept + kSchedKeptWords, st));
+        RT_TRY(launch_keep_counters(A.queue, C.d_kept, st));
+        sched_keep_refine_commit(C.keep);
+    } else if (act != kSchedReuse) {
         if (world->precision == RT_PRECISION_FP16) RT_TRY(launch_tile_order_h(A, d_octree != nullptr, C.d_cost, C.d_order, classify ? C.d_flags : nullptr, classify ? C.d_long : nullptr, st));
         else RT_TRY(launch_tile_order(A, d_octree != nullptr, C.d_cost, C.d_order, classify ? C.d_flags : nullptr, classify ? C.d_long : nullptr, st));
         if (act == kSchedCompute) {
@@ -853,12 +870,21 @@
     if (classify) { A.long_flag = C.d_flags; A.long_list = C.d_long; }
     return 0;
 }
-static int scheduled_round(rt_render_ctx& C, RenderArgs& A, const rt_world* world, const rt_octree* d_octree, int ns, bool sched, bool cap, hipStream_t st) {
+static int scheduled_round(rt_render_ctx& C, RenderArgs& A, const rt_world* world, const rt_octree* d_octree, int ns, bool sched, bool cap, hipStream_t st, bool record = false) {
     A.queue = next_slot(C);
     SchedKey key; SchedAction act = kSchedBypass;
-    if (sched) RT_TRY(schedule_decide(C, A, world, d_octree, ns, cap, key, act));
-    RT_TRY(begin_counters(C, A, act, st));
-    if (sched) RT_TRY(schedule_frame(C, A, world, d_octree, ns, st, act, key));
+    bool refine = false;
+    if (sched) {
+        RT_TRY(schedule_decide(C, A, world, d_octree, ns, cap, key, act));
+        const bool take_part = act != kSchedBypass && feedback_enabled() && feedback_gate(A, world, d_octree, ns);
+        if (act == kSchedReuse && sched_keep_refine_due(C.keep, feedback_enabled(), take_part)) { refine = true; sched_keep_refine_begin(C.keep); }
+        if (act == kSchedCompute && record && take_part) {
+            RT_TRY(hipMemsetAsync(C.d_iters, 0, sizeof(unsigned short) * (size_t)A.n_local_tiles * 64, st));
+            A.iters_out = C.d_iters;
+        }
+    }
+    RT_TRY(begin_counters(C, A, refine ? kSchedCompute : act, st));
+    if (sched) RT_TRY(schedule_frame(C, A, world, d_octree, ns, st, act, key, refine));
     return 0;
 }
 
@@ -883,7 +909,7 @@
         RT_TRY(ctx_reserve(C, A.n_local_tiles));
     }
     if (!cap) RT_TRY(ctx_wait_previous(C, st));
-    RT_TRY(scheduled_round(C, A, world, d_octree, ns, sched, cap, st));
+    RT_TRY(scheduled_round(C, A, world, d_octree, ns, sched, cap, st, mode == 0));
     C.last_queue = A.queue;
     if (mode == 1) {
         if (ns == 1 && !cap) {
@@ -899,6 +925,7 @@
     if (world->precision == RT_PRECISION_FP16) RT_TRY(launch_render_h(A, tree, mode, st));
     else if (world->arith == RT_ARITH_CONTRACT) RT_TRY(fmac::launch_render(A, tree, mode, st));
     else RT_TRY(launch_render(A, tree, mode, st));
+    if (A.iters_out) { sched_keep_counts(C.keep); C.iters_n = rt_part_pixels(max_x, max_y, part); }
     if (cap) return 0;
     RT_TRY(ctx_timed_end(C, st));
     return ctx_mark_done(C, st);
@@ -963,6 +990,31 @@
 int rt_world_render_schedule_reuse(rt_world* W, uint64_t* reused, uint64_t* computed) {
     if (!W) return RT_EINVAL;
     return rt_render_ctx_schedule_reuse(&W->z->ctx, reused, computed);
+}
+int rt_render_ctx_schedule_feedback(rt_render_ctx* C, uint64_t* refined, uint32_t* out, int n) {
+    if (!C || !refined || n < 0 || (n > 0 && !out)) return RT_EINVAL;
+    *refined = C->keep.refinements;
+    uint32_t w[RT_FEEDBACK_WORDS] = {C->keep.valid && C->keep.has_counts ? 1u : 0u, C->keep.valid && C->keep.refined ? 1u : 0u, 0u, 0u};
+    if (w[1] && n > 2) {
+        if (C->has_done) RT_TRY(hipEventSynchronize(C->done));
+        RT_TRY(hipMemcpy(w + 2, C->d_kept + kSchedKeptWords, 2 * sizeof(uint32_t), hipMemcpyDeviceToHost));
+    }
+    for (int k = 0; k < n && k < RT_FEEDBACK_WORDS; ++k) out[k] = w[k];
+    return 0;
+}
+int rt_world_render_schedule_feedback(rt_world* W, uint64_t* refined, uint32_t* out, int n) {
+    if (!W) return RT_EINVAL;
+    return rt_render_ctx_schedule_feedback(&W->z->ctx, refined, out, n);
+}
+int rt_render_ctx_schedule_counts(rt_render_ctx* C, uint16_t* out, int64_t n) {
+    if (!C || !out || n < 0) return RT_EINVAL;
+    if (!C->keep.valid || !C->keep.has_counts || !C->d_iters || n != C->iters_n) return RT_EINVAL;
+    if (C->has_done) RT_TRY(hipEventSynchronize(C->done));
+    return (int)hipMemcpy(out, C->d_iters, sizeof(uint16_t) * (size_t)n, hipMemcpyDeviceToHost);
+}
+int rt_world_render_schedule_counts(rt_world* W, uint16_t* out, int64_t n) {
+    if (!W) return RT_EINVAL;
+    return rt_render_ctx_schedule_counts(&W->z->ctx, out, n);
 }
 int rt_world_render_times(rt_world* W, float* ms_out, int max, int* count) {
     if (!W || !ms_out || !count || max < 0) return RT_EINVAL;
@@ -1477,6 +1529,7 @@
 int rt_debug_wp_classes(unsigned long long* out96, int reset) { return (int)read_wp_classes(out96, reset); }
 int rt_debug_waves(unsigned long long* out) { return (int)read_wave_dbg(out); }
 int rt_debug_pilot(int* out, int n) { return (int)read_pilot_dbg(out, n); }
+int rt_debug_chains(unsigned int* out, int n_pixels) { return (int)read_chain_dbg(out, n_pixels); }
 #endif
 
 using rt::ppm_text;
diff --git a/dd2360-raytracing_amd/csrc/rt_device.h b/dd2360-raytracing_amd/csrc/rt_device.h
--- a/dd2360-raytracing_amd/csrc/rt_device.h
+++ b/dd2360-raytracing_amd/csrc/rt_device.h
@@ -165,6 +165,7 @@
     const unsigned int* ad_count;
     float* ad_sl;
     float* ad_q;
+    unsigned short* iters_out;
 };
 
 }
diff --git a/dd2360-raytracing_amd/csrc/rt_handles.h b/dd2360-raytracing_amd/csrc/rt_handles.h
--- a/dd2360-raytracing_amd/csrc/rt_handles.h
+++ b/dd2360-raytracing_amd/csrc/rt_handles.h
@@ -54,6 +54,7 @@
     int* d_cost = nullptr; unsigned int* d_order = nullptr; unsigned char* d_flags = nullptr; unsigned int* d_long = nullptr; int* d_work = nullptr; int64_t sched_tiles = 0;
     unsigned int* last_queue = nullptr;
     rt::SchedKeep keep; unsigned int* d_kept = nullptr;
+    unsigned short* d_iters = nullptr; int64_t iters_n = 0;
     int* p_cost = nullptr; unsigned int* p_order = nullptr; int64_t p_tiles = 0; bool p_valid = false; rt::SchedKey p_key;
     bool p_pinned = false;
     float* a_sl = nullptr; float* a_q = nullptr; unsigned int* a_list = nullptr; int64_t a_pixels = 0; unsigned int* a_count = nullptr; int64_t a_rounds = 0;
diff --git a/dd2360-raytracing_amd/csrc/rt_kernels.hip b/dd2360-raytracing_amd/csrc/rt_kernels.hip
--- a/dd2360-raytracing_amd/csrc/rt_kernels.hip
+++ b/dd2360-raytracing_amd/csrc/rt_kernels.hip
@@ -1115,7 +1115,7 @@
     int sample = 0, depth = 0;
     bool live = false;
     RT_STATS_ONLY(
-    unsigned int pix_iters = 0;
+    unsigned int pix_iters = 0, pix_alone = 0;
     unsigned long long pix_t0 = 0;
     )
 
@@ -1241,8 +1241,10 @@
             const float k = (float)(1.0 / (double)(float)A.ns);
             col.x *= k; col.y *= k; col.z *= k;
             fb[0] = sqrtf(col.x); fb[1] = sqrtf(col.y); fb[2] = sqrtf(col.z);
+            if constexpr (TREE && (COOPG == 4 || COOPG == 5)) { if (A.iters_out) A.iters_out[idx] = (unsigned short)(iters < 65535u ? iters : 65535u); }
             RT_STATS_ONLY(
             fb[0] = (float)pix_iters; fb[1] = (float)((__builtin_amdgcn_s_memrealtime() >> 4) & 0xffffffull); fb[2] = (float)((pix_t0 >> 4) & 0xffffffull);
+            if (idx < (1ll << 20)) { unsigned int* cd = g_chain_dbg + idx * 8 + 6; cd[0] = (unsigned int)pix_t0; cd[1] = pix_alone; }
             )
         } else {
             if (A.ns == 1) { fb[0] = col.x; fb[1] = col.y; fb[2] = col.z; }
@@ -1257,8 +1259,8 @@
     unsigned long long th[4] = {0, 0, 0, 0};
     unsigned long long dbg_thin_cyc = 0, dbg_thin_closest = 0, dbg_thin1_cyc = 0; unsigned int dbg_thin1_iters = 0; unsigned long long dbg_t_prev = TICK();
     )
-    constexpr bool kSolo = TREE && COOPG == 5;
-    if (kSolo && lane == 0 && begin_long_pixel(true)) solo = true;
+    constexpr bool kSolo = TREE && (COOPG == 5 || (COOPG == 4 && MODE != 1));
+    if (kSolo && n_solo != 0u && lane == 0 && begin_long_pixel(true)) solo = true;
     if (__ballot(live) == 0ull && lane < RT_LONG_PER_WAVE) begin_long_pixel(false);
     if (__ballot(live) != 0ull) { thin = true; __builtin_amdgcn_s_setprio(3); }
 
@@ -1324,7 +1326,7 @@
         RT_STATS_ONLY(
         const unsigned long long tC1 = TICK(); st.cyc[0] += tC1 - tC0; st.cyc[2] += tC0; if (thin) dbg_thin_closest += tC1 - tC0;
         if (TREE && thin12) { th[0] += (st.cyc[4] - c4_) - tC0; th[1] += st.cyc[5] - c5_; th[2] += (st.cyc[1] - c1_) - (st.cyc[5] - c5_); th[3] += st.cyc[3] - c3_; }
-        if (live) { ++pix_iters; }
+        if (live) { ++pix_iters; if (__popcll(__ballot(live)) <= 2) ++pix_alone; }
         )
         if (live && !(TREE && ts.pending)) {
             ++iters;
@@ -1345,6 +1347,12 @@
                 (void)lum;
                 ++sample; depth = 0; att = {1.0f, 1.0f, 1.0f};
                 if (sample < ns) {
+                    RT_STATS_ONLY(
+                    if (MODE == 0 && idx < (1ll << 20) && (sample == ns / 3 || sample == 2 * (ns / 3))) {
+                        unsigned int* cd = g_chain_dbg + idx * 8 + (sample == ns / 3 ? 0 : 3);
+                        cd[0] = (unsigned int)__builtin_amdgcn_s_memrealtime(); cd[1] = pix_iters; cd[2] = pix_alone;
+                    }
+                    )
                     { const RenderArgs& C = *cold_args(); r = primary_ray(C.scene.cam, i, j, C.max_x, C.max_y, s); }
                     bool now_long = false;
                     if ((sample & (RT_LONG_CHECK - 1)) == 0 && sample + 8 <= ns) {
@@ -1363,7 +1371,7 @@
                     WPASS(WP_ENDPIX);
                     end_pixel();
                     RT_STATS_ONLY(
-                    pix_iters = 0;
+                    pix_iters = 0; pix_alone = 0;
                     )
                     STAT(st, ST_SWITCHES, 1);
                     live = false; is_long = false; is_med = false;
@@ -1586,6 +1594,23 @@
 RT_DEV int cost_class(int w) { const int c = (w - 64) / 64; return c < 0 ? 0 : (c > 7 ? 7 : c); }
 
 #ifndef RT_TU_LIST
+RT_DEV int block_sum3x3(const RenderArgs& A, const unsigned char* __restrict__ pilot, long long g, int bx, int by) {
+    const int own = pilot[g];
+    int sum = 0;
+#pragma unroll
+    for (int dy = -1; dy <= 1; ++dy)
+#pragma unroll
+        for (int dx = -1; dx <= 1; ++dx) {
+            const int nx_ = bx + dx, ny_ = by + dy;
+            int v = own;
+            if (nx_ >= 0 && ny_ >= 0 && nx_ < A.tiles_x * 4 && ny_ < A.tiles_y * 4) {
+                long long nl;
+                if (part_has((long long)(ny_ >> 2) * A.tiles_x + (nx_ >> 2), A.part, A.nparts, A.tile_begin, A.tile_end, nl)) v = pilot[nl * 16 + (ny_ & 3) * 4 + (nx_ & 3)];
+            }
+            sum += v;
+        }
+    return sum;
+}
 __global__ __launch_bounds__(256) void k_long_select(RenderArgs A, const unsigned char* __restrict__ pilot, unsigned char* __restrict__ long_flag,
                                                     unsigned int* __restrict__ long_list, int long_sum, int solo_sum, unsigned char* __restrict__ sum8) {
     const long long g = (long long)blockIdx.x * 256 + threadIdx.x;
@@ -1595,20 +1620,7 @@
     const long long tile = part_tile(local_tile, A.part, A.nparts, A.tile_begin, A.tile_end);
     const int tx = (int)(tile % A.tiles_x), ty = (int)(tile / A.tiles_x);
     const int bx = tx * 4 + (sub & 3), by = ty * 4 + (sub >> 2);
-    const int own = pilot[g];
-    int sum = 0;
-#pragma unroll
-    for (int dy = -1; dy <= 1; ++dy)
-#pragma unroll
-        for (int dx = -1; dx <= 1; ++dx) {
-            const int nx_ = bx + dx, ny_ = by + dy;
-            int v = own;
-            if (nx_ >= 0 && ny_ >= 0 && nx_ < A.tiles_x * 4 && ny_ < A.tiles_y * 4) {
-                long long nl;
-                if (part_has((long long)(ny_ >> 2) * A.tiles_x + (nx_ >> 2), A.part, A.nparts, A.tile_begin, A.tile_end, nl)) v = pilot[nl * 16 + (ny_ & 3) * 4 + (nx_ & 3)];
-            }
-            sum += v;
-        }
+    const int sum = block_sum3x3(A, pilot, g, bx, by);
     if (sum8) sum8[g] = (unsigned char)(sum < 255 ? sum : 255);
     const int abs_sum = (int)A.queue[kQueueThr + 1];
     const bool is_long = sum >= (abs_sum > 0 && abs_sum < long_sum ? abs_sum : long_sum);
@@ -1622,6 +1634,61 @@
         if (is_long && in_img) {
             if (sum >= solo_sum) { const unsigned int pos = atomicAdd(A.queue + 4, 1u); long_list[A.n_local_tiles * 64 - 1 - pos] = (unsigned int)pid; }
             else { const unsigned int pos = atomicAdd(A.queue + 2, 1u); long_list[pos] = (unsigned int)pid; }
+        }
+    }
+}
+
+constexpr int kQueueMaxCount = 6, kQueueSoloAsked = 7;
+__global__ __launch_bounds__(256) void k_count_cost(RenderArgs A, const unsigned short* __restrict__ iters, int* __restrict__ cost, unsigned char* __restrict__ pilot) {
+    const int lane = threadIdx.x & 63;
+    const long long local_tile = (long long)blockIdx.x * 4 + (threadIdx.x >> 6);
+    if (local_tile >= A.n_local_tiles) return;
+    const long long tile = part_tile(local_tile, A.part, A.nparts, A.tile_begin, A.tile_end);
+    const int tx = (int)(tile % A.tiles_x), ty = (int)(tile / A.tiles_x);
+    const int px = lane & 7, py = lane >> 3;
+    const int i = tx * 8 + px, j = ty * 8 + py;
+    const bool in_img = (i < A.max_x) && (j < A.max_y);
+    const long long idx = part_whole(A.nparts, A.tile_begin, A.tile_end) ? (long long)j * A.max_x + i : local_tile * 64 + lane;
+    const unsigned int v = in_img ? (unsigned int)iters[idx] : 0u;
+    unsigned int b = v;
+    b += (unsigned int)__shfl_xor((int)b, 1); b += (unsigned int)__shfl_xor((int)b, 8);
+    unsigned int t = v, m = v;
+    for (int off = 32; off > 0; off >>= 1) { t += (unsigned int)__shfl_xor((int)t, off); const unsigned int o = (unsigned int)__shfl_xor((int)m, off); m = o > m ? o : m; }
+    const unsigned int ns = (unsigned int)(A.ns > 0 ? A.ns : 1);
+    if (lane == 0) { cost[local_tile] = (int)((2u * t) / ns); if (m != 0u) atomicMax(A.queue + kQueueMaxCount, m); }
+    if (((px | py) & 1) == 0) { const unsigned int c = b / (2u * ns); pilot[local_tile * 16 + (py >> 1) * 4 + (px >> 1)] = (unsigned char)(c < 255u ? c : 255u); }
+}
+__global__ __launch_bounds__(256) void k_count_select(RenderArgs A, const unsigned char* __restrict__ pilot, const unsigned short* __restrict__ iters, unsigned char* __restrict__ long_flag,
+                                                     unsigned int* __restrict__ long_list, unsigned char* __restrict__ sum8, float solo_frac, unsigned int solo_cap, unsigned int* __restrict__ extra) {
+    const long long g = (long long)blockIdx.x * 256 + threadIdx.x;
+    if (g >= A.n_local_tiles * 16) return;
+    const long long local_tile = g >> 4;
+    const int sub = (int)(g & 15);
+    const long long tile = part_tile(local_tile, A.part, A.nparts, A.tile_begin, A.tile_end);
+    const int tx = (int)(tile % A.tiles_x), ty = (int)(tile / A.tiles_x);
+    const int sum = block_sum3x3(A, pilot, g, tx * 4 + (sub & 3), ty * 4 + (sub >> 2));
+    if (sum8) sum8[g] = (unsigned char)(sum < 255 ? sum : 255);
+    const unsigned int thr = A.queue[kQueueThr], top = A.queue[kQueueMaxCount];
+    if (g == 0 && extra) { extra[0] = top; extra[1] = solo_cap; }
+    const float solo_from = solo_frac * (float)top;
+    const bool whole = part_whole(A.nparts, A.tile_begin, A.tile_end);
+    const int lx = 2 * (sub & 3), ly = 2 * (sub >> 2);
+#pragma unroll
+    for (int q = 0; q < 4; ++q) {
+        const int px = lx + (q & 1), py = ly + (q >> 1);
+        const int i = tx * 8 + px, j = ty * 8 + py;
+        const bool in_img = (i < A.max_x) && (j < A.max_y);
+        const long long pid = local_tile * 64 + py * 8 + px;
+        const unsigned int count = in_img ? (unsigned int)iters[whole ? (long long)j * A.max_x + i : pid] : 0u;
+        const bool is_long = in_img && thr != 0u && count >= thr;
+        long_flag[pid] = is_long ? 1 : 0;
+        if (is_long) {
+            bool alone = false;
+            if (solo_frac > 0.f && (float)count >= solo_from) {
+                const unsigned int asked = atomicAdd(A.queue + kQueueSoloAsked, 1u);
+                if (asked < solo_cap) { alone = true; atomicAdd(A.queue + 4, 1u); long_list[A.n_local_tiles * 64 - 1 - asked] = (unsigned int)pid; }
+            }
+            if (!alone) { const unsigned int pos = atomicAdd(A.queue + 2, 1u); long_list[pos] = (unsigned int)pid; }
         }
     }
 }
@@ -2020,14 +2087,20 @@
     }
 }
 
+struct CountedSelect { const unsigned short* iters; float solo_frac; unsigned int solo_cap; unsigned int* extra; };
+static hipError_t select_and_order(const RenderArgs& A, int* cost, unsigned int* order, unsigned char* flags, unsigned int* long_list, hipStream_t st, int long_sum, int solo_sum, const CountedSelect* counted);
 hipError_t launch_select_and_order(const RenderArgs& A, int* cost, unsigned int* order, unsigned char* flags, unsigned int* long_list, hipStream_t st, int long_sum, int solo_sum) {
+    return select_and_order(A, cost, order, flags, long_list, st, long_sum, solo_sum, nullptr);
+}
+static hipError_t select_and_order(const RenderArgs& A, int* cost, unsigned int* order, unsigned char* flags, unsigned int* long_list, hipStream_t st, int long_sum, int solo_sum, const CountedSelect* counted) {
     const bool tail = flags && A.tail_list && A.tail_ws && A.f_tail > 0.f;
     hipLaunchKernelGGL(k_tile_order, dim3(1), dim3(1024), 0, st, (const int*)cost, order, (long long)A.n_local_tiles, A.queue, (int)A.ns, (int)A.n_lanes, A.f_inflight, A.f_static,
                        tail ? A.f_tail : 0.f, (long long)A.n_local_tiles, tail ? A.tail_ws : (unsigned int*)nullptr, tail ? A.head_sum : 0, A.head_min_load);
     if (flags) {
         const unsigned char* pilot = flags + (size_t)A.n_local_tiles * 64;
         unsigned char* sum8 = flags + (size_t)A.n_local_tiles * 80;
-        hipLaunchKernelGGL(k_long_select, dim3((unsigned)((A.n_local_tiles * 16 + 255) / 256)), dim3(256), 0, st, A, pilot, flags, long_list, long_sum > 0 ? long_sum : RT_PILOT_LONG_SUM, solo_sum, sum8);
+        if (counted) hipLaunchKernelGGL(k_count_select, dim3((unsigned)((A.n_local_tiles * 16 + 255) / 256)), dim3(256), 0, st, A, pilot, counted->iters, flags, long_list, sum8, counted->solo_frac, counted->solo_cap, counted->extra);
+        else hipLaunchKernelGGL(k_long_select, dim3((unsigned)((A.n_local_tiles * 16 + 255) / 256)), dim3(256), 0, st, A, pilot, flags, long_list, long_sum > 0 ? long_sum : RT_PILOT_LONG_SUM, solo_sum, sum8);
         if (tail) {
             const unsigned nb = (unsigned)((A.n_local_tiles * 16 + kTailChunk - 1) / kTailChunk);
             hipLaunchKernelGGL(k_tail_hist, dim3(nb), dim3(256), 0, st, (const unsigned int*)order, (const unsigned char*)sum8, (long long)A.n_local_tiles, (const unsigned int*)A.queue, A.tail_ws);
@@ -2062,6 +2135,20 @@
     B.head_min_load = variant == 2 ? A.head_min_load : 0.f;
     { const hipError_t e = launch_pilot(A, tree, cost, pilot, nullptr, st); if (e != hipSuccess) return e; }
     return launch_select_and_order(B, cost, order, flags, long_list, st, 0, variant == 5 ? RT_PILOT_SOLO_SUM : 0x7fffffff);
+}
+
+int render_variant_of(bool tree, const DevAccel& acc) { return render_variant(tree, 0, acc); }
+hipError_t launch_count_order(const RenderArgs& A, const unsigned short* iters, int* cost, unsigned int* order, unsigned char* flags, unsigned int* long_list,
+                              float solo_frac, int solo_cap_den, unsigned int* extra, hipStream_t st) {
+    if (A.n_local_tiles <= 0) return hipSuccess;
+    const int variant = render_variant(true, 0, A.tree.acc);
+    if ((variant != 4 && variant != 5) || !iters || !flags || !long_list) return hipErrorInvalidValue;
+    RenderArgs B = A;
+    B.n_lanes = (int)render_grid_blocks(A, variant, 0) * 256;
+    B.head_sum = A.head_sum; B.head_min_load = 0.f;
+    hipLaunchKernelGGL(k_count_cost, dim3((unsigned)((A.n_local_tiles + 3) / 4)), dim3(256), 0, st, B, iters, cost, flags + (size_t)A.n_local_tiles * 64);
+    const CountedSelect cs{iters, solo_frac, solo_cap_den > 0 ? (unsigned int)(B.n_lanes / 64 / solo_cap_den) : 0u, extra};
+    return select_and_order(B, cost, order, flags, long_list, st, 0, 0x7fffffff, &cs);
 }
 
 template <int MODE, int COOPG>
diff --git a/dd2360-raytracing_amd/csrc/rt_sched_keep.h b/dd2360-raytracing_amd/csrc/rt_sched_keep.h
--- a/dd2360-raytracing_amd/csrc/rt_sched_keep.h
+++ b/dd2360-raytracing_amd/csrc/rt_sched_keep.h
@@ -32,19 +32,33 @@
     bool captured = false;
     SchedKey key;
     uint64_t reused = 0, computed = 0;
+    bool has_counts = false, refined = false;
+    uint64_t refinements = 0;
 };
+inline void sched_keep_forget(SchedKeep& K) { K.valid = false; K.has_counts = false; K.refined = false; }
 
 inline SchedAction sched_keep_decide(SchedKeep& K, const SchedKey& key, bool enabled, bool capturing) {
     if (capturing) K.captured = true;
-    if (capturing || K.captured || !enabled) { K.valid = false; ++K.computed; return kSchedBypass; }
+    if (capturing || K.captured || !enabled) { sched_keep_forget(K); ++K.computed; return kSchedBypass; }
     if (K.valid && sched_key_equal(K.key, key)) { ++K.reused; return kSchedReuse; }
-    K.valid = false; ++K.computed;
+    sched_keep_forget(K); ++K.computed;
     return kSchedCompute;
 }
 inline void sched_keep_commit(SchedKeep& K, const SchedKey& key) {
     if (K.captured) return;
     K.key = key; K.valid = true;
 }
-inline void sched_keep_drop(SchedKeep& K) { K.valid = false; }
+inline void sched_keep_drop(SchedKeep& K) { sched_keep_forget(K); }
+
+inline bool sched_feedback_gate(int ns, int min_ns, int render_variant, bool half) { return !half && ns >= min_ns && (render_variant == 4 || render_variant == 5); }
+inline void sched_keep_counts(SchedKeep& K) { if (K.valid && !K.captured) K.has_counts = true; }
+inline bool sched_keep_refine_due(const SchedKeep& K, bool enabled, bool gate) {
+    return K.valid && K.has_counts && !K.refined && !K.captured && enabled && gate;
+}
+inline void sched_keep_refine_begin(SchedKeep& K) { K.valid = false; }
+inline void sched_keep_refine_commit(SchedKeep& K) {
+    if (K.captured || !K.has_counts) return;
+    K.valid = true; K.refined = true; ++K.refinements;
+}
 
 }
diff --git a/dd2360-raytracing_amd/csrc/rt_stats.h b/dd2360-raytracing_amd/csrc/rt_stats.h
--- a/dd2360-raytracing_amd/csrc/rt_stats.h
+++ b/dd2360-raytracing_amd/csrc/rt_stats.h
@@ -16,6 +16,7 @@
 __device__ unsigned long long g_stats[ST_N];
 __device__ int g_pilot_dbg[1 << 20];
 __device__ unsigned long long g_wave_dbg[8192 * 4];
+__device__ unsigned int g_chain_dbg[(1 << 20) * 8];
 struct Stats { unsigned int c[ST_N]; unsigned long long cyc[8]; };
 #ifdef RT_STATS_LIGHT
 #define STAT(st, k, v) ((void)0)
@@ -42,6 +43,7 @@
 #define RT_STATS_ONLY(...) __VA_ARGS__
 #define RT_STATS_READERS \
 hipError_t read_pilot_dbg(int* out, int n) { return hipMemcpyFromSymbol(out, HIP_SYMBOL(g_pilot_dbg), sizeof(int) * (size_t)(n < (1 << 20) ? n : (1 << 20))); } \
+hipError_t read_chain_dbg(unsigned int* out, int n_pixels) { return hipMemcpyFromSymbol(out, HIP_SYMBOL(g_chain_dbg), sizeof(unsigned int) * 8 * (size_t)(n_pixels < (1 << 20) ? n_pixels : (1 << 20))); } \
 hipError_t read_wave_dbg(unsigned long long* out) { return hipMemcpyFromSymbol(out, HIP_SYMBOL(g_wave_dbg), sizeof(unsigned long long) * 8192 * 4); } \
 hipError_t read_wp_classes(unsigned long long* out, int reset) { \
     hipError_t e = hipMemcpyFromSymbol(out, HIP_SYMBOL(g_wp_cls), sizeof(unsigned long long) * 4 * kWpBlocks); \
diff --git a/dd2360-raytracing_amd/csrc/rt_tuning.h b/dd2360-raytracing_amd/csrc/rt_tuning.h
--- a/dd2360-raytracing_amd/csrc/rt_tuning.h
+++ b/dd2360-raytracing_amd/csrc/rt_tuning.h
@@ -76,6 +76,18 @@
 #endif
 #ifndef RT_SCHED_CACHE
 #define RT_SCHED_CACHE 1
+#endif
+#ifndef RT_SCHED_FEEDBACK
+#define RT_SCHED_FEEDBACK 1
+#endif
+#ifndef RT_FEEDBACK_MIN_NS
+#define RT_FEEDBACK_MIN_NS 32
+#endif
+#ifndef RT_FB_SOLO_FRAC
+#define RT_FB_SOLO_FRAC 0.75f
+#endif
+#ifndef RT_FB_SOLO_CAP_DEN
+#define RT_FB_SOLO_CAP_DEN 32
 #endif
 #ifndef RT_PROG_OWN
 #define RT_PROG_OWN 64
diff --git a/dd2360-raytracing_amd/rt_amd.py b/dd2360-raytracing_amd/rt_amd.py
--- a/dd2360-raytracing_amd/rt_amd.py
+++ b/dd2360-raytracing_amd/rt_amd.py
@@ -34,6 +34,7 @@
 WHOLE = Partition(0, 1)
 PART_RUN = 64
 SCHEDULE_FIELDS = ("inflight_thr", "static_thr", "tail_mark", "head", "head_thr", "from_end", "long_raw", "solo_raw")
+FEEDBACK_FIELDS = ("has_counts", "rebuilt", "max_count", "solo_cap")
 
 class Adaptive(C.Structure):
     _fields_ = [("min_spp", C.c_int32), ("max_spp", C.c_int32), ("batch", C.c_int32), ("rel_error", C.c_float), ("floor", C.c_float)]
@@ -187,6 +188,10 @@
     "rt_world_render_schedule": (_i, [_vp, _vp, _i]),
     "rt_render_ctx_schedule_reuse": (_i, [_vp, _vp, _vp]),
     "rt_world_render_schedule_reuse": (_i, [_vp, _vp, _vp]),
+    "rt_render_ctx_schedule_feedback": (_i, [_vp, _vp, _vp, _i]),
+    "rt_world_render_schedule_feedback": (_i, [_vp, _vp, _vp, _i]),
+    "rt_render_ctx_schedule_counts": (_i, [_vp, _vp, C.c_int64]),
+    "rt_world_render_schedule_counts": (_i, [_vp, _vp, C.c_int64]),
     "rt_render_kernel_name": (_i, [_vp, _vp, _i, _vp, _i]),
     "rt_multi_unique_id": (_i, [_vp]),
     "rt_multi_init": (_i, [_vp, _i, _i, _vp]),
@@ -382,6 +387,16 @@
         check(lib().rt_render_ctx_schedule_reuse(self.h, C.byref(a), C.byref(b)), "rt_render_ctx_schedule_reuse")
         return a.value, b.value
 
+    def schedule_feedback(self):
+        a, out = C.c_uint64(0), np.zeros(len(FEEDBACK_FIELDS), np.uint32)
+        check(lib().rt_render_ctx_schedule_feedback(self.h, C.byref(a), _np(out), len(out)), "rt_render_ctx_schedule_feedback")
+        return dict(zip(("refined",) + FEEDBACK_FIELDS, [a.value] + [int(v) for v in out]))
+
+    def schedule_counts(self, n):
+        out = np.zeros(int(n), np.uint16)
+        check(lib().rt_render_ctx_schedule_counts(self.h, _np(out), int(n)), "rt_render_ctx_schedule_counts")
+        return out
+
     def close(self):
         if getattr(self, "h", None):
             lib().rt_render_ctx_destroy(self.h)
@@ -595,6 +610,16 @@
         check(lib().rt_world_render_schedule_reuse(self.h, C.byref(a), C.byref(b)), "rt_world_render_schedule_reuse")
         return a.value, b.value
 
+    def schedule_feedback(self):
+        a, out = C.c_uint64(0), np.zeros(len(FEEDBACK_FIELDS), np.uint32)
+        check(lib().rt_world_render_schedule_feedback(self.h, C.byref(a), _np(out), len(out)), "rt_world_render_schedule_feedback")
+        return dict(zip(("refined",) + FEEDBACK_FIELDS, [a.value] + [int(v) for v in out]))
+
+    def schedule_counts(self, n):
+        out = np.zeros(int(n), np.uint16)
+        check(lib().rt_world_render_schedule_counts(self.h, _np(out), int(n)), "rt_world_render_schedule_counts")
+        return out
+
     def close(self):
         if getattr(self, "h", None):
             lib().rt_free_world(self.h)
diff --git a/include/rt_amd.h b/include/rt_amd.h
--- a/include/rt_amd.h
+++ b/include/rt_amd.h
@@ -188,6 +188,12 @@
 
 int rt_render_ctx_schedule_reuse(rt_render_ctx* ctx, uint64_t* reused, uint64_t* computed);
 int rt_world_render_schedule_reuse(rt_world* world, uint64_t* reused, uint64_t* computed);
+
+#define RT_FEEDBACK_WORDS 4
+int rt_render_ctx_schedule_feedback(rt_render_ctx* ctx, uint64_t* refined, uint32_t* out, int n);
+int rt_world_render_schedule_feedback(rt_world* world, uint64_t* refined, uint32_t* out, int n);
+int rt_render_ctx_schedule_counts(rt_render_ctx* ctx, uint16_t* out, int64_t n);
+int rt_world_render_schedule_counts(rt_world* world, uint16_t* out, int64_t n);
 
 int rt_assemble(void* fb_full, const void* fb_parts, int max_x, int max_y, int nparts, int precision, void* stream);
 
```

Result: faster. 5143, median of 6 (+6.3%).
